# projectchrono/DEM-Engine

Measured on AMD Instinct MI355X. Metric: clump*steps/s, higher is better.
Workload: dtype f32 physics / f64 geometry

## Files before the change

dem-engine_amd/abi.py:

```python
import ctypes as C
import os

import numpy as np

_HERE = os.path.dirname(os.path.abspath(__file__))

NULL_MAPPING_PARTNER = 0xFFFFFFFF
FAMILY_MASK_ENTRIES = 32896
NUM_FAMILIES = 256
FAMILY_FIXED = 1
FAMILY_GHOST = 2
FAMILY_PRESCRIBED = 4
INTEGRATOR_FORWARD_EULER, INTEGRATOR_CENTERED_DIFFERENCE, INTEGRATOR_EXTENDED_TAYLOR = 0, 1, 2
FORCE_HERTZIAN, FORCE_HERTZIAN_FRICTIONLESS, FORCE_CUSTOM = 0, 1, 2
GHOST_BYTES = 56


ARITH_FAST, ARITH_EXACT = 1, 0


class DemeParams(C.Structure):
    _fields_ = [
        ("nvXp2", C.c_uint32), ("nvYp2", C.c_uint32), ("nvZp2", C.c_uint32),
        ("nbX", C.c_uint32), ("nbY", C.c_uint32), ("nbZ", C.c_uint32),
# ... 691 lines not shown


def _owner_state_request(owner_ids, columns):
    ids = np.ascontiguousarray(owner_ids, dtype=np.uint32).ravel()
    st, out = DemeOwnerState(), {}
    for name in STATE_DTYPES:
        setattr(st, name, None)
    for name in columns:
        out[name] = np.zeros(max(ids.size, 1), STATE_DTYPES[name])
        setattr(st, name, out[name].ctypes.data)
    st._keep = out
    return ids, st, {k: v[:ids.size] for k, v in out.items()}


def _owner_state_rows(owner_ids, arrays):
    ids = None if owner_ids is None else np.ascontiguousarray(owner_ids, dtype=np.uint32).ravel()
    st, keep = DemeOwnerState(), {}
    for name in STATE_DTYPES:
        a = arrays.get(name)
        if a is None:
            setattr(st, name, None)
            continue
        keep[name] = np.ascontiguousarray(a, dtype=STATE_DTYPES[name]).ravel()
        if ids is not None and keep[name].size != ids.size:
            raise DemeError(f"scatter_owner_state: column {name} has {keep[name].size} rows for {ids.size} ids")
        if not keep[name].size:
            keep[name] = np.zeros(1, STATE_DTYPES[name])
        setattr(st, name, keep[name].ctypes.data)
    st._keep = keep
    return ids, st


def exported_symbols():
    import re
    hdr = os.path.join(_HERE, "..", "include", "deme_hip.h")
    txt = open(hdr).read()
    return sorted(set(re.findall(r"\b(deme_[a-z_0-9]+)\s*\(", txt)))


def _ptr(a):
    return None if a is None else a.ctypes.data


def sort_tile_keys():
    return int(load_library().deme_sort_tile_keys())


def tri_loads_block_rows():
    return int(load_library().deme_tri_loads_block_rows())


def _inspect_tri_loads(self, fn, name, force_threshold, first, count):
    if count is None:
        if getattr(self, "n_tri", None) is None:
            raise ValueError(f"{name}: count is needed (this object has not seen the scene's triangle count)")
        count = self.n_tri - int(first)
    force = np.zeros((max(int(count), 0), 3), np.float64)
    contacts = np.zeros(max(int(count), 0), np.uint32)
    self._ck(fn(self.h, float(force_threshold), int(first), int(count), _ptr(force), _ptr(contacts)), name)
    return force, contacts


def sort_pairs_u32(keys, vals, begin_bit, end_bit, force_own=True, device=0):
    keys, vals = np.ascontiguousarray(keys, np.uint32), np.ascontiguousarray(vals, np.uint32)
    assert keys.shape == vals.shape and keys.ndim == 1
    ko, vo = np.empty_like(keys), np.empty_like(vals)
    rc = load_library().deme_sort_pairs_u32(device, _ptr(keys), _ptr(vals), keys.size, begin_bit, end_bit, int(bool(force_own)), _ptr(ko),
                                            _ptr(vo))
    if rc:
        raise DemeError(f"deme_sort_pairs_u32 failed with code {rc}")
    return ko, vo


def sort_keys_u64(keys, begin_bit, end_bit, force_own=True, device=0):
    keys = np.ascontiguousarray(keys, np.uint64)
    assert keys.ndim == 1
    ko = np.empty_like(keys)
    rc = load_library().deme_sort_keys_u64(device, _ptr(keys), keys.size, begin_bit, end_bit, int(bool(force_own)), _ptr(ko))
    if rc:
        raise DemeError(f"deme_sort_keys_u64 failed with code {rc}")
    return ko


def jit_probe(src, wildcard_names=(), prerequisites="", owner_wildcards=(), geo_wildcards=()):
    lib = load_library()

    def arr(ns):
        return (C.c_char_p * max(1, len(ns)))(*[s.encode() for s in ns])
    log = C.create_string_buffer(8192)
    rc = lib.deme_jit_probe_ex(src.encode(), arr(wildcard_names), len(wildcard_names), arr(owner_wildcards), len(owner_wildcards),
                               arr(geo_wildcards), len(geo_wildcards), prerequisites.encode(), log, len(log))
    return rc == 0, log.value.decode(errors="replace")


class Context:

    def __init__(self, device=0):
        self.lib = load_library()
        h = _P()
        rc = self.lib.deme_ctx_create(int(device), C.byref(h))
        if rc != 0 or not h:
            raise DemeError(f"deme_ctx_create failed (status {rc}): is a HIP device visible?")
        self.h = h
        self.n_owners = 0
        self.n_spheres = 0
        self.n_wildcards = 0

    @classmethod
    def borrowed(cls, handle):
        self = cls.__new__(cls)
        self.lib = load_library()
        self.h = handle
        self._borrowed = True
        v = (C.c_uint32 * 4)()
        self.lib.deme_scene_sizes.argtypes = [_P, C.POINTER(C.c_uint32)]
        self._ck(self.lib.deme_scene_sizes(self.h, v), "deme_scene_sizes")
        self.n_owners, self.n_spheres, self.n_wildcards = int(v[0]), int(v[2]), int(v[3])
        return self

    def refresh_sizes(self):
        v = (C.c_uint32 * 4)()
        self.lib.deme_scene_sizes.argtypes = [_P, C.POINTER(C.c_uint32)]
        self._ck(self.lib.deme_scene_sizes(self.h, v), "deme_scene_sizes")
        self.n_owners, self.n_spheres = int(v[0]), int(v[2])

    def close(self):
        if getattr(self, "h", None):
            if not getattr(self, "_borrowed", False):
                self.lib.deme_ctx_destroy(self.h)
            self.h = None

    def __del__(self):
        try:
            self.close()
        except Exception:
            pass

    def _ck(self, rc, what):
        if rc != 0:
            msg = self.lib.deme_last_error(self.h)
            raise DemeError(f"{what} failed (status {rc}): {msg.decode() if msg else ''}")

    def set_stream(self, stream_ptr):
        self._ck(self.lib.deme_ctx_set_stream(self.h, stream_ptr), "deme_ctx_set_stream")

    def sync(self):
        self._ck(self.lib.deme_sync(self.h), "deme_sync")

    def set_arith_mode(self, mode):
        m = {"fast": ARITH_FAST, "exact": ARITH_EXACT}.get(mode, mode)
        self._ck(self.lib.deme_set_arith_mode(self.h, int(m)), "deme_set_arith_mode")

    def arith_mode(self):
        return "fast" if self.lib.deme_get_arith_mode(self.h) == ARITH_FAST else "exact"

    def set_params(self, p):
        self.n_wildcards = int(p.nContactWildcards)
        self._ck(self.lib.deme_set_params(self.h, C.byref(p)), "deme_set_params")

    def upload_scene(self, sc):
        self.n_owners, self.n_spheres = int(sc.nOwners), int(sc.nSpheres)
        self.n_tri = int(sc.nTri)
        self._ck(self.lib.deme_upload_scene(self.h, C.byref(sc)), "deme_upload_scene")

    def upload_state(self, arrays):
        st, _ = make_state_struct(self.n_owners, arrays)
# ... 359 lines not shown
```

dem-engine_amd/csrc/deme_hip.hip:

```cpp
#include <algorithm>
#include <cmath>
#include <cstdarg>
#include <cstdio>
#include <cstdlib>
#include <chrono>
#include <cstring>
#include <condition_variable>
#include <functional>
#include <memory>
#include <mutex>
#include <dlfcn.h>
#include <map>
#include <string>
#include <thread>
#include <vector>

#include <hip/hip_runtime.h>
#include <rocprim/rocprim.hpp>
template <unsigned RB, unsigned IPT = 8>
using DemeRadixCfg = rocprim::radix_sort_config<rocprim::default_config, rocprim::default_config,
                                                rocprim::radix_sort_onesweep_config<rocprim::kernel_config<1024, IPT>, rocprim::kernel_config<1024, IPT>, RB,
                                                                                    rocprim::block_radix_rank_algorithm::match>,
                                                1024 * 1024>;
#include <array>
#include <iterator>
#include <limits>

#include "../../include/deme_hip.h"
#include "deme_device.h"
#include "deme_force.h"
#include "deme_force_fast.h"
#include "deme_jit.h"
#include "deme_kernels.h"
#include "deme_tile.h"
#include "deme_tile_step.h"
#include "deme_migrate.h"
#include "deme_mesh_kernels.h"
#include "deme_resize.h"
#include "deme_query.h"
#include "deme_contact_inspect.h"
#include "deme_tri_loads.h"
#include "deme_sort.h"

using namespace deme_dev;

namespace {

struct DevBuf {
    void* p = nullptr;
    size_t bytes = 0;
    template <typename T>
    T* as() const {
        return reinterpret_cast<T*>(p);
    }
};

struct ContactList {
    DevBuf mapping, ownerA, ownerB[2], bIdx[2], info, tInfo, rIdx, lPos, remVal, rankC, remKey[2], cDefer, blockMode, smFlag, smList;
    DevBuf aStart, bStart, heavy, fixedFlag, heavyList, rangeCtr, hList, hCount, tileMode, tileOrg, rStart, lOff, lCount, tileRem, tileBase,
        tileBig, bigList;
    uint64_t nListed = 0;
    int listKeys = 0;
    bool legacyLists = false;
    bool tileActive = false;
    bool fusedList = false;
    bool fusedChecked = false;
    bool hrPending = false, heavyOverflow = false;
    uint32_t nHeavy = 0, nHeavyFree = 0, nSA = 0, nSM = 0;
    uint32_t nBigTiles = 0, tileMaxHalo = 0, tileMaxList = 0, tileMaxHaloIn = 0;

    void invalidate() {
        nListed = 0, listKeys = 0;
        legacyLists = tileActive = fusedList = fusedChecked = hrPending = heavyOverflow = false;
        nHeavy = nHeavyFree = nSA = nSM = 0;
        nBigTiles = tileMaxHalo = tileMaxList = tileMaxHaloIn = 0;
    }
    std::array<DevBuf*, 35> buffers() {
        return {&mapping, &ownerA, &ownerB[0], &ownerB[1], &bIdx[0], &bIdx[1], &info, &tInfo, &rIdx, &lPos, &remVal, &rankC, &remKey[0],
                &remKey[1], &cDefer, &blockMode, &smFlag, &smList, &aStart, &bStart, &heavy, &fixedFlag, &heavyList, &rangeCtr, &hList,
                &hCount, &tileMode, &tileOrg, &rStart, &lOff, &lCount, &tileRem, &tileBase, &tileBig, &bigList};
    }
};

struct TimerSlot {
    std::vector<std::pair<hipEvent_t, hipEvent_t>> pending;
    double total_ms = 0;
    uint64_t launches = 0;
    uint64_t seen = 0;
};

}

struct deme_ctx {
    int device = 0;
    hipStream_t stream = nullptr;
    bool ownStream = true;
    std::string err;
    DemeParams hp{};
    bool haveParams = false, haveScene = false;
    DevParams dp{};
    uint32_t nOwners = 0, nOwnerClumps = 0, nSpheres = 0, nAnal = 0, nMat = 0, nComp = 0, nMassProps = 0;
    DevBuf owners, spheres, acc, comp, massProps, anal, matPair, E, nu, CoR, mu, Crr, famMasks, famExtra, famFlags;
    std::vector<uint8_t> hObjType;
    std::vector<float4> hComp;
    uint32_t nTemplateComps = 0;
    DevBuf rsMark, rsKeys[2], rsRuns, rsUKeys, rsIdx, rsOldR, rsUses, rsRemap;
    DevBuf qMark, qHits, qRecs, qCtr, qState;
    uint64_t qHostBytes = 0;
    DevBuf ciMask, ciCounts, ciPartial, ciOut;
    DevBuf tlTri[2], tlRow[2], tlTmp, tlPartial, tlForce, tlCount;
    std::map<std::string, int> regionBySource;
    DevBuf sphFam;
    DevBuf geo, binLo, binN, binPartial, incKeys[2], incVals[2], keysRaw, keysMid, keysSorted[2], wc[2], ctr,
        scanTmp, sortTmp, rec[4], stage;
    ContactList list[2];
    int cur = 0;
    DevBuf conA4, conA2, conB4, conB2, aSum, rec32;
    RangeCounters* hrPinned = nullptr;
    hipEvent_t hrEvent = nullptr;
    bool ctrFresh = false;
    bool conTile = false;
#define DEME_FUSED_AUTO_MAX_OWNERS 100000u
    int fusedEnable = 0;
    bool fusedPrevValid = false;
    uint64_t nFusedSteps = 0;
    DevBuf ownersNext, recContact, inCnt, inStart, tInfoIn, inContact, hCountIn;
    uint32_t tileMinContactsCustom = 320;
    uint64_t lastSegMax = 0;
    size_t keySegMin = (size_t)1 << 20;
    DevBuf persistKeys, binStat;
    DevBuf nextAcc;
    std::vector<AccRec> hNextAcc;
    bool nextAccPending = false;
    std::vector<uint64_t> hPersist;
    uint32_t nTri = 0;
    DevBuf tris, triWorld, triLo, triHi, triCounts, triOffsets, triKeys[2], triVals[2];
    size_t triCap = 0;
    uint64_t nTriInc = 0;
    deme_jit::MaterialTables mt;
    hipModule_t customMod = nullptr;
    hipFunction_t customFn[3] = {nullptr, nullptr, nullptr};
    hipFunction_t customTileFn[4] = {nullptr, nullptr, nullptr, nullptr};
    std::map<size_t, std::vector<char>> jitCache;
    bool conValid = false;
    int keysCur = 0, wcCur = 0;
    size_t incCap = 0, cntCap = 0;
    uint64_t nInc = 0, nContacts = 0, nPrev = 0, nWcStored = 0;
    uint64_t nActiveBins = 0;
    uint32_t maxInBin = 0;
    bool haveList = false, mapFresh = false;
    bool seeded = false;
    hipModule_t prescMod = nullptr;
    hipFunction_t prescFn = nullptr;
    DevBuf prescList, prescSlot, prescRec;
    DevBuf userWc[4][8];
    uint32_t nOwnerWc = 0, nGeoWc = 0;
    bool hasGhosts = false;
    uint32_t asyncLead = 0;
    DevBuf revSlot;
    const void* revAcc = nullptr;
    bool pairsOnce = false;
    PrescArgs laterPa{nullptr, nullptr};
    bool crossStale = false;
    char* pin = nullptr;
    int spinSync = 1;
    bool snapPending = false;
    DevBuf ownersSnap;
    hipStream_t detStream = nullptr;
    hipEvent_t evSnap = nullptr, evP1 = nullptr;
    uint64_t nAsyncDetections = 0;
    std::vector<uint32_t> hShared;
    DevBuf sharedIds, sharedBuf;
    bool tailFused = true;
    bool inGroupStep = false;
    hipStream_t haloStream = nullptr;
    hipEvent_t evStepDone = nullptr, evHaloDone = nullptr;
    bool overlapDetect = false;
    hipModule_t rulesMod = nullptr;
    DemeAdaptive ad{};
    hipEvent_t evDet0 = nullptr, evDet1 = nullptr, evWin0 = nullptr, evWin1 = nullptr;
    double binAccMs = 0, binPrevMs = -1, freqPrevMs = -1;
    float binRate = 0.f;
    uint32_t binObs = 0, freqObs = 0, nBinChanges = 0, nFreqChanges = 0;
    uint64_t winStartStep = 0;
    int freqDir = 1, binFlip = 1;
    bool winOpen = false;
    std::vector<hipModule_t> regionMod;
    std::vector<hipFunction_t> regionFn;
    DevBuf volumes;
    bool haveVolumes = false;
    hipFunction_t rulesFn = nullptr;
    bool rulesNeedAcc = false;
    uint32_t nPresc = 0;
    uint8_t hostFamFlags[DEME_NUM_FAMILIES] = {0};
    bool prescDirty = true;
    bool record = false;
    uint64_t nSteps = 0, nDetections = 0;
    uint32_t stepsSinceCD = 0;
    bool listStale = false;
    uint32_t lastStatus = 0;
    double timeElapsed = 0;
    int arith = DEME_ARITH_FAST;
    uint32_t xcdGroup = 0;
    bool permuted = false;
    int reorderEnable = 1;
    std::vector<uint32_t> hO2E, hE2O, hS2E, hE2S;
    DevBuf dO2E, dS2E;
    double orderSpread[2] = {0, 0};
    bool orderEligible = false;
    bool orderStructOK = false;
    bool geoStale = false;
    bool orderRenewDue = false;
    uint32_t orderBaseHalo = 0;
    uint64_t orderDetAt = 0, nOrderRenewals = 0;
    uint64_t listSerial = 0, viewSerial = ~0ull;
    std::vector<uint64_t> viewKeys;
    std::vector<uint32_t> viewPerm;
    int timing = 0;
    std::map<std::string, TimerSlot> timers;
    std::vector<hipEvent_t> eventPool;
};

namespace {

int fail(deme_ctx* c, int code, const char* fmt, ...) {
    char buf[1024];
    va_list ap;
    va_start(ap, fmt);
    vsnprintf(buf, sizeof(buf), fmt, ap);
    va_end(ap);
    if (c) {
        c->err = buf;
        c->lastStatus = (uint32_t)code;
    }
    return code;
}

inline uint64_t key_class_of_type(uint8_t type) {
    return type == DEME_SPHERE_SPHERE_CONTACT ? DEME_KEY_CLASS_SS : type == DEME_SPHERE_MESH_CONTACT ? DEME_KEY_CLASS_SM : DEME_KEY_CLASS_SA;
}

int records_refused(deme_ctx* c) {
    if (!c->record)
        return fail(c, DEME_ERR_INVALID, "contact recording is off (deme_set_record_contacts)");
    if (c->seeded)
        return fail(c, DEME_ERR_INVALID, "the list is a seed (deme_seed_contacts, or the engine's order was just renewed): its contacts have not been evaluated yet -- step or detect first");
    return DEME_OK;
}

#define HIPCK(call)                                                                                   \
    do {                                                                                              \
        hipError_t _e = (call);                                                                       \
        if (_e != hipSuccess)                                                                         \
            return fail(c, DEME_ERR_HIP, "%s failed: %s (%s:%d)", #call, hipGetErrorString(_e), __FILE__, __LINE__); \
    } while (0)

template <typename T>
static inline T* pin_at(deme_ctx* c, size_t off) {
    return reinterpret_cast<T*>(c->pin + off);
}
static hipError_t sync_readback(deme_ctx* c, hipStream_t st, bool spin) {
    if (c->spinSync && spin) {
        const auto t0 = std::chrono::steady_clock::now();
        for (int it = 0;; it++) {
            const hipError_t q = hipStreamQuery(st);
            if (q != hipErrorNotReady)
                return q;
            if ((it & 255) == 255 && std::chrono::steady_clock::now() - t0 > std::chrono::milliseconds(5))
                break;
        }
    }
    return hipStreamSynchronize(st);
}

int ensure(deme_ctx* c, DevBuf& b, size_t bytes, bool keep = false) {
    if (bytes <= b.bytes && b.p)
        return DEME_OK;
    size_t want = std::max<size_t>(bytes, 256);
    if (b.p)
        want = std::max(want, b.bytes + b.bytes / 4);
    void* np = nullptr;
    HIPCK(hipMalloc(&np, want));
    if (keep && b.p && b.bytes)
        HIPCK(hipMemcpyAsync(np, b.p, b.bytes, hipMemcpyDeviceToDevice, c->stream));
    if (b.p) {
        HIPCK(hipStreamSynchronize(c->stream));
        HIPCK(hipFree(b.p));
    }
    b.p = np;
    b.bytes = want;
    return DEME_OK;
}

template <typename T>
int upload(deme_ctx* c, DevBuf& b, const T* src, size_t n) {
    int rc = ensure(c, b, std::max<size_t>(n, 1) * sizeof(T));
    if (rc)
        return rc;
    if (n && src)
        HIPCK(hipMemcpyAsync(b.p, src, n * sizeof(T), hipMemcpyHostToDevice, c->stream));
    else if (n)
        HIPCK(hipMemsetAsync(b.p, 0, n * sizeof(T), c->stream));
    return DEME_OK;
}

template <class Call>
int with_temp(deme_ctx* c, DevBuf& tmp, Call&& call) {
    size_t bytes = 0;
    HIPCK(call(nullptr, bytes));
    if (int rc = ensure(c, tmp, bytes))
        return rc;
    bytes = tmp.bytes;
    HIPCK(call(tmp.p, bytes));
    return DEME_OK;
}

#ifndef DEME_SORT_ROCPRIM
#define DEME_SORT_ROCPRIM 0
#endif
constexpr size_t DEME_SORT_OWN_FROM_INCIDENCES = 82000;
constexpr size_t DEME_SORT_OWN_FROM_KEYS64 = 430000;
constexpr size_t DEME_SORT_OWN_FROM_RECORDS = 180000;
inline bool sort_takes_own(size_t n, size_t cap, size_t ownFrom) {
    return !DEME_SORT_ROCPRIM && n >= ownFrom && std::max(n, cap) <= deme_sort::MAX_N;
}
template <class RocCfg, bool HAS_V, typename K>
hipError_t deme_radix_sort(void* tmp, size_t& bytes, const K* keysIn, K* keysOut, const uint32_t* valsIn, uint32_t* valsOut, size_t n, size_t cap,
                           unsigned beginBit, unsigned endBit, size_t ownFrom, hipStream_t st) {
    if (sort_takes_own(n, cap, ownFrom))
        return deme_sort::radix_sort<K, HAS_V>(tmp, bytes, keysIn, keysOut, valsIn, valsOut, n, cap, beginBit, endBit, st);
    if constexpr (HAS_V)
        return rocprim::radix_sort_pairs<RocCfg>(tmp, bytes, keysIn, keysOut, valsIn, valsOut, n, beginBit, endBit, st);
    else
        return rocprim::radix_sort_keys<RocCfg>(tmp, bytes, keysIn, keysOut, n, beginBit, endBit, st);
}

inline unsigned grid_for(size_t n, unsigned block = 256) { return (unsigned)((n + block - 1) / block); }
inline unsigned bits_for(uint64_t n, unsigned cap) {
    unsigned b = 1;
    while (b < cap && (1ull << b) < n)
        b++;
    return b;
}

hipEvent_t get_event(deme_ctx* c) {
    if (!c->eventPool.empty()) {
        hipEvent_t e = c->eventPool.back();
        c->eventPool.pop_back();
        return e;
    }
    hipEvent_t e;
    hipEventCreate(&e);
    return e;
}
struct ScopedTimer {
    deme_ctx* c;
    TimerSlot* slot = nullptr;
    hipEvent_t a = nullptr, b = nullptr;
    hipStream_t st = nullptr;
    ScopedTimer(deme_ctx* ctx, const char* name, bool always = false, hipStream_t stream = nullptr) : c(ctx), st(stream ? stream : ctx->stream) {
        if (!c->timing)
            return;
        slot = &c->timers[name];
        if (!always && (slot->seen++ % (uint64_t)c->timing) != 0) {
            slot = nullptr;
            return;
        }
        if (slot->pending.size() >= 8192) {
            slot = nullptr;
            return;
        }
        a = get_event(c);
        b = get_event(c);
        hipEventRecord(a, st);
    }
    ~ScopedTimer() {
        if (slot) {
            hipEventRecord(b, st);
            slot->pending.emplace_back(a, b);
        }
    }
};
void drain_timers(deme_ctx* c) {
    for (auto& kv : c->timers) {
        for (auto& pr : kv.second.pending) {
            hipEventSynchronize(pr.second);
            float ms = 0;
            hipEventElapsedTime(&ms, pr.first, pr.second);
            kv.second.total_ms += ms;
            kv.second.launches++;
            c->eventPool.push_back(pr.first);
            c->eventPool.push_back(pr.second);
        }
        kv.second.pending.clear();
    }
}

void refresh_dev_params(deme_ctx* c) {
    DevParams& d = c->dp;
    const DemeParams& h = c->hp;
    d.nvXp2 = h.nvXp2, d.nvYp2 = h.nvYp2;
    d.nbX = h.nbX, d.nbY = h.nbY, d.nbZ = h.nbZ;
    d.mNbX = fast_div_magic(h.nbX), d.mNbXY = fast_div_magic(h.nbX * h.nbY);
    d.l = h.l, d.voxelSize = h.voxelSize, d.binSize = h.binSize;
    d.LBFX = h.LBFX, d.LBFY = h.LBFY, d.LBFZ = h.LBFZ;
    d.Gx = h.Gx, d.Gy = h.Gy, d.Gz = h.Gz;
    d.h = h.h;
    d.approxMaxVel = h.approxMaxVel, d.expSafetyMulti = h.expSafetyMulti, d.expSafetyAdder = h.expSafetyAdder;
    d.errOutVel = h.errOutVel;
    d.integrator = h.integrator, d.forceModel = h.forceModel, d.nW = h.nContactWildcards;
    d.nOwners = c->nOwners, d.nSpheres = c->nSpheres, d.nAnal = c->nAnal, d.nMat = c->nMat;
    d.errOutBinSphNum = h.errOutBinSphNum ? h.errOutBinSphNum : 32768u;
    d.comp = c->comp.as<float4>();
    d.massProps = c->massProps.as<float4>();
    d.anal = c->anal.as<AnalObj>();
    d.matPair = c->matPair.as<MatPair>();
    d.E = c->E.as<float>(), d.nu = c->nu.as<float>(), d.CoR = c->CoR.as<float>(), d.mu = c->mu.as<float>(),
    d.Crr = c->Crr.as<float>();
    d.familyMasks = c->famMasks.as<uint8_t>();
    d.familyExtra = c->famExtra.as<float>();
    d.familyFlags = c->famFlags.as<uint8_t>();
    d.tris = c->tris.p;
    d.nTri = c->nTri;
    d.s2e = c->permuted ? c->dS2E.as<uint32_t>() : nullptr;
    d.o2e = c->permuted ? c->dO2E.as<uint32_t>() : nullptr;
}

int check_ready(deme_ctx* c) {
    if (!c)
        return DEME_ERR_INVALID;
    if (!c->haveParams || !c->haveScene)
        return fail(c, DEME_ERR_INVALID, "deme_set_params and deme_upload_scene must be called first");
    if (hipSetDevice(c->device) != hipSuccess)
        return fail(c, DEME_ERR_HIP, "device %d cannot be selected", c->device);
    return DEME_OK;
}

void build_mat_pairs(const DemeScene* s, std::vector<MatPair>& out) {
    const uint32_t n = s->nMat;
    out.resize((size_t)n * n);
    for (uint32_t a = 0; a < n; a++)
        for (uint32_t b = 0; b < n; b++) {
            MatPair m{};
            const float Y1 = s->E[a], nu1 = s->nu[a], Y2 = s->E[b], nu2 = s->nu[b];
            const float invE = (1.0f - nu1 * nu1) / Y1 + (1.0f - nu2 * nu2) / Y2;
            m.E_cnt = 1.0f / invE;
            const float invG = 2.0f * (2.0f - nu1) * (1.0f + nu1) / Y1 + 2.0f * (2.0f - nu2) * (1.0f + nu2) / Y2;
            m.G_cnt = 1.0f / invG;
            m.CoR = s->CoR ? s->CoR[a * n + b] : 0.f;
            m.mu = s->mu ? s->mu[a * n + b] : 0.f;
            m.Crr = s->Crr ? s->Crr[a * n + b] : 0.f;
            const float loge = (float)((m.CoR < 1e-12) ? log(1e-12) : logf(m.CoR));
            m.beta = (float)(loge / sqrt(loge * loge + 9.869604401089358));
            out[(size_t)a * n + b] = m;
        }
}

int size_list_per_contact(deme_ctx* c, ContactList& L, size_t cap, bool hasGhosts, uint32_t nTri) {
    int rc = 0;
    rc |= ensure(c, L.mapping, cap * 4, true);
    rc |= ensure(c, L.ownerA, cap * 4);
    for (int k = 0; k < 2; k++) {
        rc |= ensure(c, L.ownerB[k], cap * 4);
        rc |= ensure(c, L.bIdx[k], cap * 4);
    }
    rc |= ensure(c, L.info, cap * 16);
    rc |= ensure(c, L.tInfo, cap * 8);
    rc |= ensure(c, L.rIdx, cap * 4);
    rc |= ensure(c, L.lPos, cap * 2);
    rc |= ensure(c, L.remVal, (cap + 1) * 4);
    rc |= ensure(c, L.rankC, (cap + 1) * 4);
    rc |= ensure(c, L.remKey[0], (cap + 1) * 4);
    rc |= ensure(c, L.remKey[1], (cap + 1) * 4);
    if (hasGhosts) {
        rc |= ensure(c, L.cDefer, cap);
        rc |= ensure(c, L.blockMode, (cap / DEME_FORCE_BLOCK + 2) * 4);
    }
    if (nTri) {
        rc |= ensure(c, L.smFlag, cap);
        rc |= ensure(c, L.smList, cap * 4);
    }
    return rc;
}
int size_list_per_owner(deme_ctx* c, ContactList& L, size_t nO) {
    if (ensure(c, L.aStart, (nO + 1) * 4) || ensure(c, L.bStart, (nO + 1) * 4) || ensure(c, L.heavy, nO + 1) || ensure(c, L.fixedFlag, nO + 1) ||
        ensure(c, L.heavyList, 4096 * 4) || ensure(c, L.rangeCtr, sizeof(RangeCounters)))
        return c->lastStatus;
    const size_t nTiles = (nO + DEME_TILE_NB - 1) / DEME_TILE_NB + 1;
    if (ensure(c, L.hList, nTiles * DEME_TILE_HMAX * 4) || ensure(c, L.hCount, nTiles * 4) || ensure(c, L.tileMode, nTiles * 4) ||
        ensure(c, L.tileOrg, nTiles * 24) || ensure(c, L.rStart, (nO + 1) * 4) || ensure(c, L.lOff, nTiles * (DEME_TILE_NB + 1) * 2) ||
        ensure(c, L.lCount, nTiles * 4) || ensure(c, L.tileRem, (nTiles + 1) * 4) || ensure(c, L.tileBase, (nTiles + 1) * 4) ||
        ensure(c, L.tileBig, nTiles * 4) || ensure(c, L.bigList, nTiles * 4))
        return c->lastStatus;
    return DEME_OK;
}

int grow_contact_arena(deme_ctx* c, size_t cap) {
    const uint32_t nW = std::max<uint32_t>(c->hp.nContactWildcards, 1);
    int rc = 0;
    rc |= ensure(c, c->keysRaw, cap * 8);
    rc |= ensure(c, c->keysSorted[0], cap * 8, true);
    rc |= ensure(c, c->keysSorted[1], cap * 8, true);
    rc |= ensure(c, c->wc[0], cap * 4 * nW, true);
    rc |= ensure(c, c->wc[1], cap * 4 * nW, true);
    if (c->record)
        for (int k = 0; k < 4; k++)
            rc |= ensure(c, c->rec[k], cap * 12);
    rc |= ensure(c, c->conA4, cap * 16);
    rc |= ensure(c, c->conA2, cap * 8);
    rc |= ensure(c, c->conB4, cap * 16);
    rc |= ensure(c, c->conB2, cap * 8);
    rc |= size_list_per_contact(c, c->list[c->cur], cap, c->hasGhosts, c->nTri);
    rc |= ensure(c, c->recContact, (cap + 1) * 4);
    rc |= ensure(c, c->tInfoIn, cap * 8);
    rc |= ensure(c, c->inContact, cap * 4);
    rc |= ensure(c, c->rec32, cap * 32);
    if (rc)
        return rc;
    c->cntCap = cap;
    return DEME_OK;
}

int grow_incidence_arena(deme_ctx* c, size_t cap) {
    int rc = 0;
    for (int k = 0; k < 2; k++) {
        rc |= ensure(c, c->incKeys[k], cap * 4);
        rc |= ensure(c, c->incVals[k], cap * 4);
    }
    if (rc)
        return rc;
    c->incCap = cap;
    return DEME_OK;
}

int status_to_error(deme_ctx* c, uint32_t st) {
    if (st & DEME_ST_NONFINITE)
        return fail(c, DEME_ERR_VELOCITY, "a non-finite owner velocity was found at time %.9g", c->timeElapsed);
    if (st & DEME_ST_VELOCITY)
        return fail(c, DEME_ERR_VELOCITY,
                    "system max velocity exceeded the error-out velocity %.7g at time %.9g (SetErrorOutVelocity)",
                    (double)c->hp.errOutVel, c->timeElapsed);
    return DEME_OK;
}

int do_margins(deme_ctx* c, uint32_t drift) {
    HIPCK(hipMemsetAsync(c->ctr.p, 0, sizeof(DetectBlock), c->stream));
    c->ctrFresh = true;
    if (c->nOwners)
    hipLaunchKernelGGL(k_margins, dim3(grid_for(c->nOwners)), dim3(256), 0, c->stream, c->dp, c->owners.as<OwnerRec>(),
                       drift, c->ctr.as<DetectCounters>());
    return DEME_OK;
}

int do_migrate(deme_ctx* c);
int detect_part1(deme_ctx* c, hipStream_t st, OwnerRec* ow, bool async, uint64_t* nCout) {
    const uint32_t nS = c->nSpheres;
    DetectCounters hc{};
    const bool countersFresh = c->ctrFresh;
    c->ctrFresh = false;
    bool statusSeen = false;

    DetectBlock* blk = c->ctr.as<DetectBlock>();
    for (int attempt = 0; attempt < 4; attempt++) {
        if (attempt > 0 || !countersFresh)
            HIPCK(hipMemsetAsync(c->ctr.p, 0, sizeof(DetectBlock), st));
        const bool segmented = c->keySegMin && c->cntCap >= c->keySegMin && c->cntCap >= DEME_KEY_SEGS * 64u;
        KeyArena ar;
        ar.keys = c->keysRaw.as<uint64_t>();
        ar.segMask = segmented ? DEME_KEY_SEGS - 1u : 0u;
        ar.segCap = segmented ? (uint64_t)c->cntCap / DEME_KEY_SEGS : (uint64_t)c->cntCap;
        ar.ctr = segmented ? blk->segCtr : &blk->c.nContactsRaw;
        if (nS) {
            c->geoStale = false;
            hipLaunchKernelGGL(k_sphere_prep, dim3(grid_for(nS)), dim3(256), 0, st, c->dp,
                               ow, c->spheres.as<SphereRec>(), c->geo.as<GeoRec>(),
                               c->binLo.as<uint4>(), c->binN.as<uint2>(), c->binPartial.as<uint32_t>(),
                               ar, c->ctr.as<DetectCounters>(), c->sphFam.as<uint16_t>());
            hipLaunchKernelGGL(k_scan_small, dim3(1), dim3(DEME_SCAN_T), 0, st, c->binPartial.as<uint32_t>(), c->binPartial.as<uint32_t>(),
                               grid_for(nS), &blk->c.nIncidence);
        }
        uint32_t P = 0;
        bool filled = false;
        auto fill_incidence = [&]() {
            hipLaunchKernelGGL(k_fill_incidence, dim3(grid_for(nS)), dim3(256), 0, st, c->dp,
                               c->binLo.as<uint4>(), c->binN.as<uint2>(), c->binPartial.as<uint32_t>(),
                               c->incKeys[0].as<uint32_t>(), c->incVals[0].as<uint32_t>(), (uint64_t)c->incCap);
            filled = true;
        };
        if (nS && c->incCap)
            fill_incidence();
        if (nS) {
            HIPCK(hipMemcpyAsync(pin_at<DetectCounters>(c, 1024), c->ctr.p, sizeof(hc), hipMemcpyDeviceToHost, st));
            HIPCK(sync_readback(c, st, !async));
            hc = *pin_at<DetectCounters>(c, 1024);
            if (!statusSeen) {
                statusSeen = true;
                if (int rc = status_to_error(c, hc.status & ~DEME_ST_INCIDENCE))
                    return rc;
            }
            if (hc.status & DEME_ST_INCIDENCE)
                return fail(c, DEME_ERR_OVERFLOW,
                            "a sphere touches more than %u bins (margin far larger than the bin size): the incidence list cannot be built",
                            DEME_MAX_BINS_PER_SPHERE);
            if (hc.nIncidence > 0xFFFFFFFFull)
                return fail(c, DEME_ERR_OVERFLOW, "%llu bin-sphere incidences do not fit the 32-bit list offsets (use larger bins)",
                            hc.nIncidence);
            P = (uint32_t)hc.nIncidence;
        }
        if (P > c->incCap) {
            if (int rc = grow_incidence_arena(c, (size_t)P + P / 4 + 1024))
                return rc;
            filled = false;
        }
        c->nInc = P;
        uint32_t nStats = 0;
        const unsigned bits = bits_for((uint64_t)c->hp.nbX * c->hp.nbY * c->hp.nbZ, 32);
        if (P) {
            if (!filled)
                fill_incidence();
            const bool twoPass = bits > 16 && bits <= 22;
            if (int rc = with_temp(c, c->sortTmp, [&](void* tmp, size_t& bytes) {
                    return twoPass ? deme_radix_sort<DemeRadixCfg<11, 16>, true>(tmp, bytes, c->incKeys[0].as<uint32_t>(), c->incKeys[1].as<uint32_t>(),
                                                                                 c->incVals[0].as<uint32_t>(), c->incVals[1].as<uint32_t>(), (size_t)P,
                                                                                 (size_t)c->incCap, 0, bits, DEME_SORT_OWN_FROM_INCIDENCES, st)
                                   : deme_radix_sort<DemeRadixCfg<8>, true>(tmp, bytes, c->incKeys[0].as<uint32_t>(), c->incKeys[1].as<uint32_t>(),
                                                                            c->incVals[0].as<uint32_t>(), c->incVals[1].as<uint32_t>(), (size_t)P,
                                                                            (size_t)c->incCap, 0, bits, DEME_SORT_OWN_FROM_INCIDENCES, st);
                }))
                return rc;
            const uint32_t nWin = (uint32_t)grid_for(P, SW_T);
            if (int rc = ensure(c, c->binStat, (size_t)nWin * sizeof(uint2)))
                return rc;
            static_assert(SW_WPB == 1, "k_sweep writes one statistics record per window");
            hipLaunchKernelGGL(k_sweep, dim3(nWin), dim3(SW_T), 0, st, c->dp,
                               c->incKeys[1].as<uint32_t>(), c->incVals[1].as<uint32_t>(), P, c->geo.as<GeoRec>(),
                               c->sphFam.as<uint16_t>(), ar, c->binStat.as<uint2>());
            if (segmented)
                nStats = nWin;
            else
                hipLaunchKernelGGL(k_bin_stats_final, dim3((nWin + 2047u) / 2048u), dim3(256), 0, st, c->binStat.as<uint2>(), nWin,
                                   c->ctr.as<DetectCounters>());
        }
        c->nTriInc = 0;
        if (c->nTri && P) {
            const uint32_t nT = c->nTri;
            hipLaunchKernelGGL(k_tri_prep, dim3(grid_for(nT)), dim3(256), 0, st, c->dp, nT, c->tris.as<TriRec>(),
                               ow, c->triWorld.as<TriWorld>(), c->triLo.as<int4>(),
                               c->triHi.as<int4>(), c->triCounts.as<uint32_t>());
            size_t tmp = c->scanTmp.bytes;
            HIPCK(rocprim::exclusive_scan(c->scanTmp.p, tmp, c->triCounts.as<uint32_t>(), c->triOffsets.as<uint32_t>(), 0u,
                                          (size_t)nT + 1, rocprim::plus<uint32_t>(), st));
            uint32_t TP = 0;
            HIPCK(hipMemcpyAsync(&TP, c->triOffsets.as<uint32_t>() + nT, 4, hipMemcpyDeviceToHost, st));
            HIPCK(hipStreamSynchronize(st));
            if (TP > c->triCap) {
                const size_t cap = (size_t)TP + TP / 4 + 1024;
                for (int k = 0; k < 2; k++)
                    if (ensure(c, c->triKeys[k], cap * 4) || ensure(c, c->triVals[k], cap * 4))
                        return c->lastStatus;
                c->triCap = cap;
            }
            c->nTriInc = TP;
            if (TP) {
                hipLaunchKernelGGL(k_tri_fill, dim3(grid_for(nT)), dim3(256), 0, st, c->dp, nT,
                                   c->triWorld.as<TriWorld>(), c->triLo.as<int4>(), c->triHi.as<int4>(),
                                   c->triOffsets.as<uint32_t>(), c->triKeys[0].as<uint32_t>(), c->triVals[0].as<uint32_t>(),
                                   (uint64_t)c->triCap);
                if (int rc = with_temp(c, c->sortTmp, [&](void* tmp, size_t& bytes) {
                        return rocprim::radix_sort_pairs(tmp, bytes, c->triKeys[0].as<uint32_t>(), c->triKeys[1].as<uint32_t>(),
                                                         c->triVals[0].as<uint32_t>(), c->triVals[1].as<uint32_t>(), (size_t)TP, 0, bits, st);
                    }))
                    return rc;
                hipLaunchKernelGGL(k_tri_sweep, dim3(grid_for(TP)), dim3(256), 0, st, c->dp, TP,
                                   c->triKeys[1].as<uint32_t>(), c->triVals[1].as<uint32_t>(), c->triWorld.as<TriWorld>(), P,
                                   c->incKeys[1].as<uint32_t>(), c->incVals[1].as<uint32_t>(), c->geo.as<GeoRec>(),
                                   c->sphFam.as<uint16_t>(), ar);
            }
        }
        const int nextEarly = c->keysCur ^ 1;
        uint32_t compactBlocks = 0;
        if (segmented) {
            compactBlocks = (uint32_t)std::min<uint64_t>(grid_for(std::max<uint64_t>(c->lastSegMax + c->lastSegMax / 8 + 1024, 1)), grid_for(ar.segCap));
            hipLaunchKernelGGL(k_compact_keys, dim3(compactBlocks, DEME_KEY_SEGS), dim3(256), 0, st, c->keysRaw.as<uint64_t>(), ar.segCap,
                               blk, 0u, c->keysSorted[nextEarly].as<uint64_t>(), c->binStat.as<uint2>(), nStats);
        }
        const DetectHead* hh = pin_at<DetectHead>(c, 1024);
        HIPCK(hipMemcpyAsync(pin_at<DetectHead>(c, 1024), c->ctr.p, segmented ? sizeof(DetectHead) : sizeof(DetectCounters), hipMemcpyDeviceToHost, st));
        HIPCK(sync_readback(c, st, !async));
        hc = hh->c;
        if (!statusSeen) {
            statusSeen = true;
            if (int rc = status_to_error(c, hc.status & ~DEME_ST_INCIDENCE))
                return rc;
        }
        unsigned long long segMax = 0;
        if (segmented) {
            hc.nContactsRaw = 0;
            for (uint32_t g = 0; g < DEME_KEY_SEGS; g++) {
                hc.nContactsRaw += hh->segCount[g];
                segMax = std::max(segMax, hh->segCount[g]);
            }
        }
        if (hc.nContactsRaw > c->cntCap || segMax > ar.segCap) {
            if (async)
                HIPCK(hipStreamSynchronize(c->stream));
            const size_t want = std::max<size_t>(hc.nContactsRaw, (size_t)segMax * DEME_KEY_SEGS);
            if (int rc = grow_contact_arena(c, want + want / 4 + 1024))
                return rc;
            continue;
        }
        c->nActiveBins = hc.nActiveBins;
        c->maxInBin = hc.maxInBin ? hc.maxInBin : (P ? 1u : 0u);
        if (c->maxInBin > c->dp.errOutBinSphNum)
            return fail(c, DEME_ERR_BIN_TOO_FULL,
                        "a bin contains %u sphere components, exceeding the allowance %u (SetMaxSphereInBin)", c->maxInBin,
                        c->dp.errOutBinSphNum);
        uint64_t nC = hc.nContactsRaw;
        const size_t nPersist = c->hPersist.size();
        if (nPersist) {
            if (nC + nPersist > c->cntCap) {
                if (async)
                HIPCK(hipStreamSynchronize(c->stream));
            if (int rc = grow_contact_arena(c, (size_t)nC + nPersist + nC / 4 + 1024))
                    return rc;
                continue;
            }
            nC += nPersist;
        }
        const int next = c->keysCur ^ 1;
        uint64_t* rawKeys = c->keysRaw.as<uint64_t>();
        if (segmented) {
            c->lastSegMax = segMax;
            if (grid_for(segMax) > compactBlocks)
                hipLaunchKernelGGL(k_compact_keys, dim3((unsigned)grid_for(segMax) - compactBlocks, DEME_KEY_SEGS), dim3(256), 0, st,
                                   c->keysRaw.as<uint64_t>(), ar.segCap, blk, compactBlocks, c->keysSorted[next].as<uint64_t>(),
                                   (const uint2*)nullptr, 0u);
            if (hc.nContactsRaw)
                rawKeys = c->keysSorted[next].as<uint64_t>();
        }
        if (nPersist)
            HIPCK(hipMemcpyAsync(rawKeys + hc.nContactsRaw, c->persistKeys.p, nPersist * 8, hipMemcpyDeviceToDevice, st));
        if (nC) {
            const unsigned bitsA = bits_for(c->dp.nSpheres, 31);
            if (int rc = ensure(c, c->keysMid, (size_t)c->cntCap * 8))
                return rc;
            uint64_t* mid = c->keysMid.as<uint64_t>();
            if (int rc = with_temp(c, c->sortTmp, [&](void* tmp, size_t& bytes) {
                    return deme_radix_sort<DemeRadixCfg<8>, false>(tmp, bytes, rawKeys, mid, nullptr, nullptr, (size_t)nC, (size_t)c->cntCap, 31,
                                                                   33 + bitsA, DEME_SORT_OWN_FROM_KEYS64, st);
                }))
                return rc;
            hipLaunchKernelGGL(k_segment_rank_sort, dim3(grid_for(nC)), dim3(256), 0, st, (uint32_t)nC, mid,
                               c->keysSorted[next].as<uint64_t>());
            if (nPersist) {
                unsigned long long* cnt = &blk->c.nContactsRaw;
                if (int rc = with_temp(c, c->scanTmp, [&](void* tmp, size_t& bytes) {
                        return rocprim::unique(tmp, bytes, c->keysSorted[next].as<uint64_t>(), c->keysRaw.as<uint64_t>(), cnt, (size_t)nC,
                                               rocprim::equal_to<uint64_t>(), st);
                    }))
                    return rc;
                unsigned long long nU = 0;
                HIPCK(hipMemcpyAsync(&nU, cnt, 8, hipMemcpyDeviceToHost, st));
                HIPCK(hipStreamSynchronize(st));
                nC = nU;
                HIPCK(hipMemcpyAsync(c->keysSorted[next].p, c->keysRaw.p, (size_t)nC * 8, hipMemcpyDeviceToDevice, st));
            }
        }
        *nCout = nC;
        return DEME_OK;
    }
    return fail(c, DEME_ERR_OVERFLOW, "contact arena kept overflowing");
}

int build_legacy_lists(deme_ctx* c, ContactList& L, const OwnerRec* ow, hipStream_t st) {
    const uint64_t nC = L.nListed;
    if (nC) {
        const unsigned obits = bits_for(c->nOwners, 32);
        if (int rc = with_temp(c, c->sortTmp, [&](void* tmp, size_t& bytes) {
                return rocprim::radix_sort_pairs(tmp, bytes, L.ownerB[0].as<uint32_t>(), L.ownerB[1].as<uint32_t>(), L.bIdx[0].as<uint32_t>(),
                                                 L.bIdx[1].as<uint32_t>(), (size_t)nC, 0, obits, st);
            }))
            return rc;
    }
    if (c->hasGhosts) {
        if (int rc = size_list_per_contact(c, L, c->cntCap, true, c->nTri))
            return rc;
        HIPCK(hipMemsetAsync(L.blockMode.p, 0, L.blockMode.bytes, st));
    }
    if (nC)
        hipLaunchKernelGGL(k_run_starts, dim3(grid_for(nC)), dim3(256), 0, st, (uint32_t)nC, L.ownerB[1].as<uint32_t>(),
                           c->nOwners, L.bStart.as<uint32_t>());
    else
        HIPCK(hipMemsetAsync(L.bStart.p, 0, ((size_t)c->nOwners + 1) * 4, st));
    HIPCK(hipMemsetAsync(&L.rangeCtr.as<RangeCounters>()->nHeavy, 0, 2 * sizeof(unsigned int), st));
    hipLaunchKernelGGL(k_owner_ranges, dim3(grid_for((size_t)c->nOwners + 1)), dim3(256), 0, st, c->dp, (uint32_t)nC,
                       L.ownerA.as<uint32_t>(), L.ownerB[1].as<uint32_t>(), ow, L.aStart.as<uint32_t>(),
                       L.bStart.as<uint32_t>(), L.heavy.as<uint8_t>(), L.fixedFlag.as<uint8_t>(), L.heavyList.as<uint32_t>(),
                       (uint32_t)(L.heavyList.bytes / 4), L.rangeCtr.as<RangeCounters>(), L.info.as<uint4>(),
                       c->hasGhosts ? L.cDefer.as<uint8_t>() : (uint8_t*)nullptr, L.blockMode.as<uint32_t>());
    L.legacyLists = true;
    return DEME_OK;
}
int read_legacy_counts(deme_ctx* c, ContactList& L, hipStream_t st, RangeCounters& hr) {
    HIPCK(hipMemcpyAsync(&hr, L.rangeCtr.p, sizeof(hr), hipMemcpyDeviceToHost, st));
    HIPCK(hipStreamSynchronize(st));
    if (hr.nHeavy > L.heavyList.bytes / 4)
        return fail(c, DEME_ERR_OVERFLOW, "%u owners exceed the heavy-owner list", hr.nHeavy);
    L.nHeavy = hr.nHeavy, L.nHeavyFree = hr.nHeavyFree;
    return DEME_OK;
}

void resolve_heavy_counts(deme_ctx* c, ContactList& L);
int ensure_legacy_lists(deme_ctx* c) {
    ContactList& L = c->list[c->cur];
    if (L.legacyLists || !c->haveList)
        return DEME_OK;
    resolve_heavy_counts(c, L);
    if (int rc = build_legacy_lists(c, L, c->owners.as<OwnerRec>(), c->stream))
        return rc;
    RangeCounters hr{};
    return read_legacy_counts(c, L, c->stream, hr);
}

bool tile_eligible(const deme_ctx* c, uint64_t nC) {
    const uint32_t nTiles = (c->nOwners + DEME_TILE_NB - 1) / DEME_TILE_NB;
    if (!nC || c->arith != DEME_ARITH_FAST || !c->hShared.empty())
        return false;
    if (c->hp.forceModel == DEME_FORCE_CUSTOM && !(c->customTileFn[0] && nC >= (uint64_t)c->tileMinContactsCustom * nTiles))
        return false;
    static_assert(DEME_TILE_T < 2 * 17 * 17, "a tile's tables may hold more than 16 materials: tInfo has 4-bit material fields");
    const uint64_t pieces = (uint64_t)c->nComp + 2ull * c->nMat * c->nMat + 4ull * c->nAnal;
    return pieces <= DEME_TILE_T && c->nMassProps <= DEME_TILE_T && c->nAnal <= 65535 && c->nComp <= 65535 &&
           tile_table_bytes(c->nComp, c->nMat, c->nAnal, c->nMassProps, c->dp.familyTrivial) <= DEME_TILE_TABLE_MAX;
}

int detect_part2(deme_ctx* c, ContactList& L, const OwnerRec* ow, hipStream_t st, uint64_t nC) {
    const int next = c->keysCur ^ 1;
    L.invalidate();
    const bool tileEligible = tile_eligible(c, nC);
    const uint32_t nTiles = (c->nOwners + DEME_TILE_NB - 1) / DEME_TILE_NB;
    if (nC) {
        const uint64_t nPrev = c->haveList ? c->nContacts : 0;
        hipLaunchKernelGGL(k_history, dim3(grid_for(nC)), dim3(256), 0, st, (uint32_t)nC, c->keysSorted[next].as<uint64_t>(),
                           (uint32_t)nPrev, c->keysSorted[c->keysCur].as<uint64_t>(), L.mapping.as<uint32_t>(),
                           L.rangeCtr.as<uint32_t>(), (uint32_t)(sizeof(RangeCounters) / 4), L.tileRem.as<uint32_t>(),
                           tileEligible ? nTiles + 1 : 0u);
    } else {
        HIPCK(hipMemsetAsync(L.rangeCtr.p, 0, sizeof(RangeCounters), st));
    }
    if (nC) {
        hipLaunchKernelGGL(k_contact_owners, dim3(grid_for(nC)), dim3(256), 0, st, c->dp, (uint32_t)nC,
                           c->keysSorted[next].as<uint64_t>(), c->spheres.as<SphereRec>(), L.ownerA.as<uint32_t>(),
                           L.ownerB[0].as<uint32_t>(), L.bIdx[0].as<uint32_t>(), L.info.as<uint4>(),
                           c->nTri ? L.smFlag.as<uint8_t>() : (uint8_t*)nullptr,
                           tileEligible ? L.tileRem.as<uint32_t>() : (uint32_t*)nullptr, (uint32_t)DEME_TILE_NB);
        if (c->nTri) {
            unsigned int* cnt = &L.rangeCtr.as<RangeCounters>()->nSM;
            if (int rc = with_temp(c, c->scanTmp, [&](void* tmp, size_t& bytes) {
                    return rocprim::select(tmp, bytes, rocprim::counting_iterator<uint32_t>(0), L.smFlag.as<uint8_t>(), L.smList.as<uint32_t>(), cnt,
                                           (size_t)nC, st);
                }))
                return rc;
        }
        hipLaunchKernelGGL(k_run_starts, dim3(grid_for(nC)), dim3(256), 0, st, (uint32_t)nC, L.ownerA.as<uint32_t>(), c->nOwners,
                           L.aStart.as<uint32_t>());
    } else {
        HIPCK(hipMemsetAsync(L.aStart.p, 0, ((size_t)c->nOwners + 1) * 4, st));
    }
    L.nListed = nC, L.listKeys = next;
    bool tiled = false;
    RangeCounters hr{};
    if (tileEligible) {
        hipLaunchKernelGGL(k_scan_small, dim3(1), dim3(DEME_SCAN_T), 0, st, L.tileRem.as<uint32_t>(), L.tileBase.as<uint32_t>(), nTiles + 1,
                           &L.rangeCtr.as<RangeCounters>()->nRemote);
        hipLaunchKernelGGL(k_tile_build, dim3(nTiles), dim3(256), 0, st, c->dp, c->nOwners, L.info.as<uint4>(),
                           L.ownerB[0].as<uint32_t>(), L.aStart.as<uint32_t>(), ow, L.tileBase.as<uint32_t>(), L.tInfo.as<uint2>(),
                           L.hList.as<uint32_t>(), L.hCount.as<uint32_t>(),
                           c->hasGhosts ? L.tileMode.as<uint32_t>() : (uint32_t*)nullptr, L.lOff.as<uint16_t>(),
                           L.lPos.as<uint16_t>(), L.lCount.as<uint32_t>(), L.rankC.as<uint32_t>(), L.remKey[0].as<uint32_t>(),
                           L.remVal.as<uint32_t>(), L.tileOrg.as<int64_t>(), L.rangeCtr.as<RangeCounters>(), nTiles,
                           L.tileBig.as<uint32_t>(), L.bigList.as<uint32_t>(), c->recContact.as<uint32_t>());
        hipLaunchKernelGGL(k_tile_stats, dim3((nTiles + 1023u) / 1024u), dim3(256), 0, st, nTiles, L.hCount.as<uint32_t>(),
                           L.lCount.as<uint32_t>(), L.rangeCtr.as<RangeCounters>());
        uint32_t nR = 0;
        HIPCK(hipMemcpyAsync(pin_at<RangeCounters>(c, 128), L.rangeCtr.p, sizeof(hr), hipMemcpyDeviceToHost, st));
        HIPCK(sync_readback(c, st, true));
        hr = *pin_at<RangeCounters>(c, 128);
        nR = (uint32_t)hr.nRemote + hr.nExtra;
        L.nBigTiles = hr.nBig;
        const unsigned obits = bits_for(c->nOwners, 32);
        if (nR) {
            if (int rc = with_temp(c, c->sortTmp, [&](void* tmp, size_t& bytes) {
                    return deme_radix_sort<DemeRadixCfg<10>, true>(tmp, bytes, L.remKey[0].as<uint32_t>(), L.remKey[1].as<uint32_t>(),
                                                                   L.remVal.as<uint32_t>(), L.rIdx.as<uint32_t>(), (size_t)nR, (size_t)c->cntCap, 0, obits,
                                                                   DEME_SORT_OWN_FROM_RECORDS, st);
                }))
                return rc;
            hipLaunchKernelGGL(k_run_starts, dim3(grid_for(nR)), dim3(256), 0, st, nR, L.remKey[1].as<uint32_t>(), c->nOwners,
                               L.rStart.as<uint32_t>());
        } else {
            HIPCK(hipMemsetAsync(L.rStart.p, 0, ((size_t)c->nOwners + 1) * 4, st));
        }
        hipLaunchKernelGGL(k_owner_ranges_tile, dim3(grid_for(c->nOwners)), dim3(256), 0, st, c->dp, ow, L.aStart.as<uint32_t>(),
                           L.lOff.as<uint16_t>(), L.rStart.as<uint32_t>(), L.heavy.as<uint8_t>(), L.fixedFlag.as<uint8_t>(),
                           L.heavyList.as<uint32_t>(), (uint32_t)(L.heavyList.bytes / 4), L.rangeCtr.as<RangeCounters>());
        tiled = true;
        static const int fusedEnv = getenv("DEME_FUSED") ? atoi(getenv("DEME_FUSED")) : -1;
        const int fusedMode = fusedEnv < 0 ? c->fusedEnable : fusedEnv;
        if ((fusedMode == 2 ? c->nOwners <= DEME_FUSED_AUTO_MAX_OWNERS : fusedMode != 0) && hr.nBig == 0 && c->hp.forceModel != DEME_FORCE_CUSTOM && !c->record && c->nTri == 0 &&
            !c->hasGhosts && !c->prescFn && !c->rulesFn && c->hShared.empty() && c->asyncLead == 0 &&
            !c->ad.autoBinSize && !c->ad.autoUpdateFreq) {
            hipLaunchKernelGGL(k_in_count, dim3(grid_for((size_t)c->nOwners + 1)), dim3(256), 0, st, c->dp, ow,
                               L.rStart.as<uint32_t>(), c->inCnt.as<uint32_t>());
            if (int rc = with_temp(c, c->scanTmp, [&](void* tmp, size_t& bytes) {
                    return rocprim::exclusive_scan(tmp, bytes, c->inCnt.as<uint32_t>(), c->inStart.as<uint32_t>(), 0u, (size_t)c->nOwners + 1,
                                                   rocprim::plus<uint32_t>(), st);
                }))
                return rc;
            hipLaunchKernelGGL(k_tile_incoming, dim3(nTiles), dim3(256), 0, st, c->dp, c->nOwners, L.info.as<uint4>(),
                               L.rStart.as<uint32_t>(), L.rIdx.as<uint32_t>(), c->recContact.as<uint32_t>(), c->inStart.as<uint32_t>(),
                               L.hList.as<uint32_t>(), L.hCount.as<uint32_t>(), c->hCountIn.as<uint32_t>(), c->tInfoIn.as<uint2>(),
                               c->inContact.as<uint32_t>(), L.rangeCtr.as<RangeCounters>());
            L.fusedList = true;
        }
    }
    if (tiled) {
        if (!c->hrPinned) {
            HIPCK(hipHostMalloc((void**)&c->hrPinned, sizeof(RangeCounters), hipHostMallocDefault));
            HIPCK(hipEventCreateWithFlags(&c->hrEvent, hipEventDisableTiming));
        }
        HIPCK(hipMemcpyAsync(c->hrPinned, L.rangeCtr.p, sizeof(RangeCounters), hipMemcpyDeviceToHost, st));
        HIPCK(hipEventRecord(c->hrEvent, st));
        L.hrPending = true;
    } else {
        if (int rc = build_legacy_lists(c, L, ow, st))
            return rc;
        if (int rc = read_legacy_counts(c, L, st, hr))
            return rc;
    }
    L.tileActive = tiled;
    L.tileMaxHalo = hr.tileMaxHalo, L.tileMaxList = hr.tileMaxList;
    L.nSA = hr.nSA;
    L.nSM = hr.nSM;
    c->fusedPrevValid = false;
    if (tiled && c->orderEligible) {
        const uint32_t fit = std::max(1u, nTiles - std::min(nTiles, hr.nBig));
        const uint32_t mean16 = (uint32_t)(16ull * hr.tileHaloSum / fit);
        if (!c->orderBaseHalo) {
            c->orderBaseHalo = std::max(mean16, 16u);
            c->orderDetAt = c->nDetections;
        } else if (c->nDetections - c->orderDetAt >= 20 && nTiles > 4 &&
                   (hr.nBig > std::max(4u, nTiles / 64u) || mean16 > c->orderBaseHalo + c->orderBaseHalo / 2)) {
            c->orderRenewDue = true;
        }
    }
    c->conValid = false;
    c->nPrev = c->haveList ? c->nContacts : 0;
    c->nContacts = nC;
    c->keysCur = next;
    c->listSerial++;
    c->haveList = true;
    c->seeded = false;
    c->mapFresh = true;
    c->nDetections++;
    return DEME_OK;
}


int do_detect(deme_ctx* c) {
    if (c->mapFresh)
        if (int rc = do_migrate(c))
            return rc;
    ScopedTimer tm(c, "detect", true);
    uint64_t nC = 0;
    if (int rc = detect_part1(c, c->stream, c->owners.as<OwnerRec>(), false, &nC))
        return rc;
    return detect_part2(c, c->list[c->cur], c->owners.as<OwnerRec>(), c->stream, nC);
}

int do_migrate(deme_ctx* c) {
    ContactList& L = c->list[c->cur];
    const uint32_t nW = c->hp.nContactWildcards;
// ... 364 lines not shown
            PrescRec* rec = c->prescRec.as<PrescRec>();
            uint32_t n = c->nPresc;
            float t = (float)c->timeElapsed;
            void* args[] = {&c->dp, &ow, &list, &n, &rec, &t};
            HIPCK(hipModuleLaunchKernel(c->prescFn, grid_for(n), 1, 1, 256, 1, 1, 0, c->stream, args, nullptr));
            pa.rec = rec;
            pa.slot = c->prescSlot.as<uint32_t>();
        }
    }
    if (from == AccFrom::Contributions) {
        if (L.heavyOverflow)
            return c->lastStatus;
        GatherArgs ga = gather_args(c);
        ga.revPhase = who == Owners::NotWaiting ? 1u : 0u;
        if (c->nOwners)
        hipLaunchKernelGGL(k_integrate<true>, dim3(grid_for(c->nOwners)), dim3(256), 0, c->stream, c->dp,
                           c->owners.as<OwnerRec>(), c->acc.as<AccRec>(), ga, pa);
    } else {
        if (c->nOwners)
        hipLaunchKernelGGL(k_integrate<false>, dim3(grid_for(c->nOwners)), dim3(256), 0, c->stream, c->dp,
                           c->owners.as<OwnerRec>(), c->acc.as<AccRec>(), gather_args(c), pa);
    }
    c->laterPa = pa;
    if (who == Owners::NotWaiting)
        return DEME_OK;
    return clear_next_acc(c);
}
int launch_integrate_later(deme_ctx* c, const uint32_t* ids, uint32_t n) {
    if (n) {
        ScopedTimer tm(c, "integrate_later");
        hipLaunchKernelGGL(k_integrate_list, dim3(grid_for(n)), dim3(256), 0, c->stream, c->dp, c->owners.as<OwnerRec>(),
                           c->acc.as<AccRec>(), gather_args(c), c->laterPa, ids, n);
    }
    return clear_next_acc(c);
}

void launch_full_reduction(deme_ctx* c) {
    if (c->nOwners)
    hipLaunchKernelGGL(k_gather_acc, dim3(grid_for(c->nOwners)), dim3(256), 0, c->stream, c->dp, gather_args(c),
                       c->owners.as<OwnerRec>(), c->acc.as<AccRec>());
    launch_reduce_heavy(c, false);
}

}

#include "deme_order.inc"

extern "C" {

const char* deme_version(void) { return "deme_hip 0.1 (gfx950)"; }

int deme_ctx_create(int device, deme_ctx** out) {
    if (!out)
        return DEME_ERR_INVALID;
    *out = nullptr;
    int n = 0;
    if (hipGetDeviceCount(&n) != hipSuccess || n <= 0 || device >= n)
        return DEME_ERR_HIP;
    if (hipSetDevice(device) != hipSuccess)
        return DEME_ERR_HIP;
    deme_ctx* c = new deme_ctx();
    c->device = device;
    if (hipStreamCreateWithFlags(&c->stream, hipStreamNonBlocking) != hipSuccess) {
        delete c;
        return DEME_ERR_HIP;
    }
    if (ensure(c, c->ctr, sizeof(DetectBlock)) || ensure(c, c->scanTmp, 1 << 20)) {
        delete c;
        return DEME_ERR_HIP;
    }
    hipMemsetAsync(c->ctr.p, 0, sizeof(DetectBlock), c->stream);
    if (hipHostMalloc((void**)&c->pin, 16384, hipHostMallocDefault) != hipSuccess) {
        deme_ctx_destroy(c);
        return DEME_ERR_HIP;
    }
    if (const char* e = getenv("DEME_ARITH"))
        c->arith = (strcmp(e, "exact") == 0) ? DEME_ARITH_EXACT : DEME_ARITH_FAST;
    if (const char* e = getenv("DEME_XCD_GROUP"))
        c->xcdGroup = (uint32_t)std::max(0, atoi(e));
    if (const char* e = getenv("DEME_SPIN_SYNC"))
        c->spinSync = atoi(e);
    if (const char* e = getenv("DEME_KEY_SEG_MIN"))
        c->keySegMin = (size_t)std::max(0ll, atoll(e));
    *out = c;
    return DEME_OK;
}

void deme_ctx_destroy(deme_ctx* c) {
    if (!c)
        return;
    hipSetDevice(c->device);
    hipStreamSynchronize(c->stream);
    drain_timers(c);
    for (auto e : c->eventPool)
        hipEventDestroy(e);
    for (hipModule_t m : {c->customMod, c->prescMod, c->rulesMod})
        if (m)
            (void)hipModuleUnload(m);
    for (hipModule_t m : c->regionMod)
        if (m)
            (void)hipModuleUnload(m);
    for (hipEvent_t e : {c->evDet0, c->evDet1, c->evWin0, c->evWin1})
        if (e)
            hipEventDestroy(e);
    if (c->haloStream) {
        hipStreamSynchronize(c->haloStream);
        hipEventDestroy(c->evStepDone);
        hipEventDestroy(c->evHaloDone);
        hipStreamDestroy(c->haloStream);
    }
    if (c->pin)
        hipHostFree(c->pin);
    for (ContactList& l : c->list)
        for (DevBuf* b : l.buffers())
            if (b->p)
                hipFree(b->p);
    if (c->hrPinned) {
        hipHostFree(c->hrPinned);
        hipEventDestroy(c->hrEvent);
    }
    if (c->detStream) {
        hipStreamSynchronize(c->detStream);
        hipEventDestroy(c->evSnap);
        hipEventDestroy(c->evP1);
        hipStreamDestroy(c->detStream);
    }
    DevBuf* all[] = {&c->hCountIn, &c->ownersNext, &c->recContact, &c->inCnt, &c->inStart, &c->tInfoIn, &c->inContact,
                     &c->sphFam, &c->dO2E, &c->dS2E, &c->rec32, &c->revSlot, &c->nextAcc, &c->binStat, &c->volumes,
                     &c->persistKeys, &c->owners, &c->spheres, &c->acc, &c->conA4, &c->conA2, &c->conB4, &c->conB2, &c->aSum,
                     &c->prescList, &c->prescSlot, &c->prescRec, &c->tris, &c->triWorld, &c->triLo, &c->triHi, &c->triCounts,
                     &c->triOffsets, &c->triKeys[0], &c->triKeys[1], &c->triVals[0], &c->triVals[1], &c->comp, &c->massProps,
                     &c->anal, &c->matPair, &c->E, &c->nu, &c->CoR, &c->mu, &c->Crr, &c->famMasks, &c->famExtra, &c->famFlags,
                     &c->geo, &c->binLo, &c->binN, &c->binPartial, &c->incKeys[0], &c->incKeys[1], &c->incVals[0],
                     &c->incVals[1], &c->keysRaw, &c->keysSorted[0], &c->keysSorted[1], &c->wc[0], &c->wc[1], &c->ctr,
                     &c->scanTmp, &c->sortTmp, &c->rec[0], &c->rec[1], &c->rec[2], &c->rec[3], &c->stage, &c->sharedIds,
                     &c->sharedBuf, &c->keysMid, &c->ownersSnap, &c->rsMark, &c->rsKeys[0], &c->rsKeys[1], &c->rsRuns,
                     &c->rsUKeys, &c->rsIdx, &c->rsOldR, &c->rsUses, &c->rsRemap, &c->qMark, &c->qHits, &c->qRecs, &c->qCtr, &c->qState,
                     &c->ciMask, &c->ciCounts, &c->ciPartial, &c->ciOut, &c->tlTri[0], &c->tlTri[1], &c->tlRow[0], &c->tlRow[1],
                     &c->tlTmp, &c->tlPartial, &c->tlForce, &c->tlCount};
    for (DevBuf* b : all)
        if (b->p)
            hipFree(b->p);
    for (auto& kind : c->userWc)
        for (auto& b : kind)
            if (b.p)
                hipFree(b.p);
    if (c->ownStream && c->stream)
        hipStreamDestroy(c->stream);
    delete c;
}

const char* deme_last_error(const deme_ctx* c) { return c ? c->err.c_str() : "null context"; }

int deme_ctx_set_stream(deme_ctx* c, void* s) {
    if (!c)
        return DEME_ERR_INVALID;
    hipSetDevice(c->device);
    HIPCK(hipStreamSynchronize(c->stream));
    if (s) {
        if (c->ownStream)
            hipStreamDestroy(c->stream);
        c->stream = (hipStream_t)s;
        c->ownStream = false;
    } else if (!c->ownStream) {
        HIPCK(hipStreamCreateWithFlags(&c->stream, hipStreamNonBlocking));
        c->ownStream = true;
    }
    return DEME_OK;
}

int deme_set_arith_mode(deme_ctx* c, int mode) {
    if (!c || (mode != DEME_ARITH_FAST && mode != DEME_ARITH_EXACT))
        return DEME_ERR_INVALID;
    hipSetDevice(c->device);
    if (mode != c->arith) {
        HIPCK(hipStreamSynchronize(c->stream));
        c->arith = mode;
        c->conValid = false;
        if (mode == DEME_ARITH_EXACT) {
            c->orderEligible = false, c->orderRenewDue = false;
            if (c->permuted && c->haveScene)
                if (int rc = order_restore(c))
                    return rc;
        } else if (c->haveScene && c->orderStructOK) {
            c->orderEligible = true;
            c->orderRenewDue = true;
        }
    }
    return DEME_OK;
}
int deme_get_arith_mode(const deme_ctx* c) { return c ? c->arith : -1; }

int deme_force_kernel_name(const deme_ctx* c, char* name, size_t cap, uint32_t* tileMaxHalo, uint32_t* tileMaxList) {
    if (!c || !name || !cap)
        return DEME_ERR_INVALID;
// ... 2913 lines not shown
    if (int rc = check_ready(c))
        return rc;
    if (int rc = contact_inspect_refused(c, "deme_inspect_contacts", out, region, thr))
        return rc;
    ContactSums* res = nullptr;
    if (int rc = contact_inspect_launch(c, region, thr, false, &res))
        return rc;
    DemeContactSums h;
    HIPCK(hipMemcpyAsync(&h, res, sizeof h, hipMemcpyDeviceToHost, c->stream));
    HIPCK(hipStreamSynchronize(c->stream));
    c->qHostBytes += sizeof h;
    *out = h;
    return DEME_OK;
}

int deme_inspect_contact_counts(deme_ctx* c, int region, float thr, uint32_t* perOwner, size_t cap) {
    if (int rc = check_ready(c))
        return rc;
    if (int rc = contact_inspect_refused(c, "deme_inspect_contact_counts", perOwner, region, thr))
        return rc;
    const size_t nO = c->nOwners;
    if (cap < nO)
        return fail(c, DEME_ERR_INVALID, "buffer too small: need %zu", nO);
    if (!nO)
        return DEME_OK;
    if (ensure(c, c->ciOut, nO * 4))
        return c->lastStatus;
    if (int rc = contact_inspect_launch(c, region, thr, true, nullptr))
        return rc;
    if (nO)
    hipLaunchKernelGGL(k_contact_counts_out, dim3(grid_for(nO)), dim3(256), 0, c->stream, (uint32_t)nO, c->ciCounts.as<uint32_t>(), c->dp.o2e,
                       (const uint32_t*)nullptr, c->ciOut.as<uint32_t>(), (uint32_t)nO);
    std::vector<uint32_t> h(nO);
    HIPCK(hipMemcpyAsync(h.data(), c->ciOut.p, nO * 4, hipMemcpyDeviceToHost, c->stream));
    HIPCK(hipStreamSynchronize(c->stream));
    c->qHostBytes += 4ull * nO;
    memcpy(perOwner, h.data(), nO * 4);
    return DEME_OK;
}

namespace {
int tri_loads_args_refused(char (&msg)[320], const char* who, float thr, uint32_t firstTri, uint32_t nTris, uint32_t nTri, const void* force,
                           const void* contacts) {
    msg[0] = 0;
    if (!std::isfinite(thr) || thr < 0.f)
        snprintf(msg, sizeof msg, "%s: the force threshold is %g; it must be finite and >= 0", who, (double)thr);
    else if ((uint64_t)firstTri + nTris > nTri)
        snprintf(msg, sizeof msg, "%s: triangles [%u, %llu) were asked for; the scene has %u", who, firstTri,
                 (unsigned long long)firstTri + nTris, nTri);
    else if (nTris && !force && !contacts)
        snprintf(msg, sizeof msg, "%s: null output (force and contacts)", who);
    return msg[0] ? DEME_ERR_INVALID : DEME_OK;
}
int tri_loads_launch(deme_ctx* c, float thr) {
    const size_t n = c->haveList ? (size_t)c->nContacts : 0, nT = c->nTri;
    const unsigned grid = grid_for(std::max<size_t>(n, 1), TRI_LOADS_BLOCK_ROWS);
    if (ensure(c, c->tlForce, nT * 24) || ensure(c, c->tlCount, nT * 4))
        return c->lastStatus;
    HIPCK(hipMemsetAsync(c->tlForce.p, 0, nT * 24, c->stream));
    HIPCK(hipMemsetAsync(c->tlCount.p, 0, nT * 4, c->stream));
    if (!n)
        return DEME_OK;
    for (int k = 0; k < 2; k++)
        if (ensure(c, c->tlTri[k], n * 4) || ensure(c, c->tlRow[k], n * 4))
            return c->lastStatus;
    if (ensure(c, c->tlPartial, (size_t)grid * 2 * sizeof(TriPartial)))
        return c->lastStatus;
    TriSelectArgs a{};
    a.n = (uint32_t)n, a.keys = c->keysSorted[c->keysCur].as<uint64_t>();
    a.spheres = c->spheres.as<SphereRec>(), a.owners = c->owners.as<OwnerRec>();
    a.nSpheres = c->nSpheres, a.nOwners = c->nOwners, a.nTri = c->nTri;
    a.force = c->rec[0].as<float>(), a.thr2 = (double)thr * (double)thr;
    a.tri = c->tlTri[0].as<uint32_t>(), a.row = c->tlRow[0].as<uint32_t>();
    {
        ScopedTimer t(c, "tri_loads_select", true);
        hipLaunchKernelGGL(k_tri_select, dim3(grid_for(n)), dim3(256), 0, c->stream, a);
    }
    const unsigned bits = bits_for((uint64_t)nT + 1, 32);
    {
        ScopedTimer t(c, "tri_loads_sort", true);
        if (int rc = with_temp(c, c->tlTmp, [&](void* tmp, size_t& bytes) {
                return deme_radix_sort<DemeRadixCfg<8>, true>(tmp, bytes, c->tlTri[0].as<uint32_t>(), c->tlTri[1].as<uint32_t>(),
                                                              c->tlRow[0].as<uint32_t>(), c->tlRow[1].as<uint32_t>(), n, n, 0, bits,
                                                              DEME_SORT_OWN_FROM_RECORDS, c->stream);
            }))
            return rc;
    }
    ScopedTimer t(c, "tri_loads_sums", true);
    hipLaunchKernelGGL(k_tri_seg_sums, dim3(grid), dim3(256), 0, c->stream, (uint32_t)n, (uint32_t)nT, c->tlTri[1].as<uint32_t>(),
                       c->tlRow[1].as<uint32_t>(), c->rec[0].as<float>(), c->tlForce.as<double>(), c->tlCount.as<uint32_t>(),
                       c->tlPartial.as<TriPartial>());
    hipLaunchKernelGGL(k_tri_seg_final, dim3(1), dim3(256), 0, c->stream, 2u * grid, (uint32_t)nT, c->tlPartial.as<TriPartial>(),
                       c->tlForce.as<double>(), c->tlCount.as<uint32_t>());
    HIPCK(hipGetLastError());
    return DEME_OK;
}
int tri_loads_fetch(deme_ctx* c, uint32_t firstTri, uint32_t nTris, double* force, uint32_t* contacts) {
    if (force)
        HIPCK(hipMemcpyAsync(force, c->tlForce.as<double>() + 3 * (size_t)firstTri, (size_t)nTris * 24, hipMemcpyDeviceToHost, c->stream));
    if (contacts)
        HIPCK(hipMemcpyAsync(contacts, c->tlCount.as<uint32_t>() + firstTri, (size_t)nTris * 4, hipMemcpyDeviceToHost, c->stream));
    HIPCK(hipStreamSynchronize(c->stream));
    return DEME_OK;
}
}

unsigned deme_tri_loads_block_rows(void) { return TRI_LOADS_BLOCK_ROWS; }

int deme_inspect_tri_loads(deme_ctx* c, float thr, uint32_t firstTri, uint32_t nTris, double* force, uint32_t* contacts) {
    if (int rc = check_ready(c))
        return rc;
    char msg[320];
    if (int rc = tri_loads_args_refused(msg, "deme_inspect_tri_loads", thr, firstTri, nTris, c->nTri, force, contacts))
        return fail(c, rc, "%s", msg);
    if (!nTris)
        return DEME_OK;
    if (records_refused(c))
        return fail(c, DEME_ERR_INVALID, "deme_inspect_tri_loads: %s", std::string(c->err).c_str());
    if (int rc = tri_loads_launch(c, thr))
        return rc;
    std::vector<double> hf(force ? (size_t)nTris * 3 : 0);
    std::vector<uint32_t> hn(contacts ? nTris : 0);
    if (int rc = tri_loads_fetch(c, firstTri, nTris, force ? hf.data() : nullptr, contacts ? hn.data() : nullptr))
        return rc;
    c->qHostBytes += (uint64_t)nTris * ((force ? 24 : 0) + (contacts ? 4 : 0));
    if (force)
        memcpy(force, hf.data(), hf.size() * 8);
    if (contacts)
        memcpy(contacts, hn.data(), hn.size() * 4);
    return DEME_OK;
}

namespace {
inline void owner_state_row(const DemeOwnerState* out, size_t at, const OwnerRec& r) {
#define DEME_COL(abi, T, Rec, f) if (out->abi) out->abi[at] = r.f;
    DEME_OWNER_COLS(DEME_COL, DEME_COL_NONE, DEME_COL_NONE)
#undef DEME_COL
    if (out->familyID) out->familyID[at] = (uint8_t)r.family;
}
}

int deme_query_owner_state(deme_ctx* c, const uint32_t* ownerIds, size_t n, DemeOwnerState* out) {
    if (int rc = check_ready(c))
        return rc;
    char msg[320];
    if (int rc = owner_ids_refused(msg, "deme_query_owner_state", out, "state", ownerIds, n, c->nOwners, out,
                                   "need the reduction a full download launches (deme_download_owner_state)", true))
        return fail(c, rc, "%s", msg);
    if (!n)
        return DEME_OK;
    std::vector<uint32_t> slots(n);
    for (size_t i = 0; i < n; i++)
        slots[i] = c->permuted ? c->hE2O[ownerIds[i]] : ownerIds[i];
    if (ensure(c, c->stage, n * 4) || ensure(c, c->qState, n * sizeof(OwnerRec)))
        return c->lastStatus;
    HIPCK(hipMemcpyAsync(c->stage.p, slots.data(), n * 4, hipMemcpyHostToDevice, c->stream));
    hipLaunchKernelGGL(k_query_owner_state, dim3(grid_for(n)), dim3(256), 0, c->stream, (uint32_t)n, c->owners.as<OwnerRec>(),
                       c->stage.as<uint32_t>(), (const uint32_t*)nullptr, SlabBooksDev{}, 0u, 0u, (const uint8_t*)nullptr,
                       c->qState.as<OwnerRec>(), (uint32_t)n, (uint32_t*)nullptr);
    std::vector<OwnerRec> h(n);
    HIPCK(hipMemcpyAsync(h.data(), c->qState.p, n * sizeof(OwnerRec), hipMemcpyDeviceToHost, c->stream));
    HIPCK(hipStreamSynchronize(c->stream));
    c->qHostBytes += (uint64_t)n * sizeof(OwnerRec);
    for (size_t i = 0; i < n; i++)
        owner_state_row(out, i, h[i]);
    return DEME_OK;
}
// ... 20 lines not shown
    HIPCK(hipMemcpyAsync(c->stage.p, keys.data(), n * 4, hipMemcpyHostToDevice, c->stream));
    HIPCK(hipMemcpyAsync(c->qState.p, patch.data(), n * sizeof(OwnerRec), hipMemcpyHostToDevice, c->stream));
    const uint32_t threads = byGid ? c->nOwners : (uint32_t)n;
    if (threads)
        hipLaunchKernelGGL(k_scatter_owner_state, dim3(grid_for(threads)), dim3(256), 0, c->stream, threads, c->owners.as<OwnerRec>(), c->nOwners,
                           c->stage.as<uint32_t>(), (uint32_t)n, c->qState.as<OwnerRec>(), mask, byGid ? c->dp.o2e : (const uint32_t*)nullptr,
                           byGid ? ownerGid : (const uint32_t*)nullptr);
    HIPCK(hipStreamSynchronize(c->stream));
    return DEME_OK;
}
}

int deme_scatter_owner_state(deme_ctx* c, const uint32_t* ownerIds, size_t n, const DemeOwnerState* in) {
    if (int rc = check_ready(c))
        return rc;
    char msg[320];
    std::vector<std::pair<uint32_t, uint32_t>> sorted;
    if (int rc = owner_ids_refused(msg, "deme_scatter_owner_state", in, "state", ownerIds, n, c->nOwners, in,
                                   "columns are not written by owner id (deme_upload_owner_state hands the accumulators to the caller)", true, &sorted))
        return fail(c, rc, "%s", msg);
    const uint32_t mask = owner_state_mask(in);
    if (!n || !mask)
        return DEME_OK;
    std::vector<uint32_t> slots(n);
    std::vector<OwnerRec> patch(n);
    for (size_t i = 0; i < n; i++) {
        slots[i] = c->permuted ? c->hE2O[ownerIds[i]] : ownerIds[i];
        patch[i] = owner_state_patch(in, i);
    }
    if (int rc = launch_owner_scatter(c, in, slots, patch, mask, false, nullptr))
        return rc;
    c->qHostBytes += (uint64_t)n * (4 + sizeof(OwnerRec));
    return DEME_OK;
}

namespace {
struct SortScratch {
    std::vector<void*> held;
    ~SortScratch() {
        for (void* p : held)
            (void)hipFree(p);
    }
    template <typename T>
    T* room(size_t n) {
        void* p = nullptr;
        if (hipMalloc(&p, std::max<size_t>(n, 1) * sizeof(T)) != hipSuccess)
            return nullptr;
        held.push_back(p);
        return reinterpret_cast<T*>(p);
    }
};
template <class RocCfg, bool HAS_V, typename K>
int sort_host_arrays(int device, const K* keys, const uint32_t* vals, size_t n, unsigned beginBit, unsigned endBit, size_t ownFrom, K* keysOut,
                     uint32_t* valsOut) {
    if (endBit < beginBit || endBit > 8 * sizeof(K) || (n && (!keys || !keysOut || (HAS_V && (!vals || !valsOut)))))
        return DEME_ERR_INVALID;
    if (!ownFrom && (DEME_SORT_ROCPRIM || n > deme_sort::MAX_N))
        return DEME_ERR_INVALID;
    if (!n)
        return DEME_OK;
    if (hipSetDevice(device) != hipSuccess)
        return DEME_ERR_HIP;
    SortScratch s;
    K *dIn = s.room<K>(n), *dOut = s.room<K>(n);
    uint32_t *vIn = HAS_V ? s.room<uint32_t>(n) : nullptr, *vOut = HAS_V ? s.room<uint32_t>(n) : nullptr;
    if (!dIn || !dOut || (HAS_V && (!vIn || !vOut)))
        return DEME_ERR_HIP;
    size_t bytes = 0;
    if (deme_radix_sort<RocCfg, HAS_V>(nullptr, bytes, dIn, dOut, vIn, vOut, n, n, beginBit, endBit, ownFrom, nullptr) != hipSuccess)
        return DEME_ERR_HIP;
    void* tmp = s.room<char>(bytes);
    if (!tmp)
        return DEME_ERR_HIP;
    bool ok = hipMemcpy(dIn, keys, n * sizeof(K), hipMemcpyHostToDevice) == hipSuccess;
    if (HAS_V)
        ok = ok && hipMemcpy(vIn, vals, n * 4, hipMemcpyHostToDevice) == hipSuccess;
    ok = ok && deme_radix_sort<RocCfg, HAS_V>(tmp, bytes, dIn, dOut, vIn, vOut, n, n, beginBit, endBit, ownFrom, nullptr) == hipSuccess;
    ok = ok && hipDeviceSynchronize() == hipSuccess;
    ok = ok && hipMemcpy(keysOut, dOut, n * sizeof(K), hipMemcpyDeviceToHost) == hipSuccess;
    if (HAS_V)
        ok = ok && hipMemcpy(valsOut, vOut, n * 4, hipMemcpyDeviceToHost) == hipSuccess;
    return ok ? DEME_OK : DEME_ERR_HIP;
}
}

unsigned deme_sort_tile_keys(void) { return deme_sort::TILE; }

int deme_sort_pairs_u32(int device, const uint32_t* keys, const uint32_t* vals, size_t n, unsigned beginBit, unsigned endBit, int forceOwn,
                        uint32_t* keysOut, uint32_t* valsOut) {
    const unsigned bits = endBit >= beginBit ? endBit - beginBit : 0;
    if (bits <= 20)
        return sort_host_arrays<DemeRadixCfg<10>, true>(device, keys, vals, n, beginBit, endBit, forceOwn ? 0 : DEME_SORT_OWN_FROM_RECORDS, keysOut,
                                                        valsOut);
    if (bits <= 22)
        return sort_host_arrays<DemeRadixCfg<11, 16>, true>(device, keys, vals, n, beginBit, endBit, forceOwn ? 0 : DEME_SORT_OWN_FROM_INCIDENCES,
                                                            keysOut, valsOut);
    return sort_host_arrays<DemeRadixCfg<8>, true>(device, keys, vals, n, beginBit, endBit, forceOwn ? 0 : DEME_SORT_OWN_FROM_INCIDENCES, keysOut,
                                                   valsOut);
}

int deme_sort_keys_u64(int device, const uint64_t* keys, size_t n, unsigned beginBit, unsigned endBit, int forceOwn, uint64_t* keysOut) {
    return sort_host_arrays<DemeRadixCfg<8>, false>(device, keys, nullptr, n, beginBit, endBit, forceOwn ? 0 : DEME_SORT_OWN_FROM_KEYS64, keysOut,
                                                    nullptr);
}

#include "deme_decomp.inc"
```

dem-engine_amd/csrc/deme_kernels.h:

```cpp
#pragma once
#include "deme_device.h"
#include "deme_owner_cols.h"

namespace deme_dev {

#define DEME_NULL_BINID_DEV 0xFFFFFFFFu
#define DEME_ST_VELOCITY 1u
#define DEME_ST_NONFINITE 2u
#define DEME_ST_INCIDENCE 4u
#define DEME_MAX_BINS_PER_SPHERE 0xFFFFFFu

struct DetectCounters {
    unsigned long long nContactsRaw;
    unsigned int nActiveBins;
    unsigned int maxInBin;
    unsigned int status;
    unsigned int pad0;
    unsigned long long nIncidence;
    unsigned int pad[8];
};

#define DEME_KEY_SEGS 64u
#define DEME_KEY_SEG_STRIDE 16u
struct DetectBlock {
    DetectCounters c;
    unsigned long long segCount[DEME_KEY_SEGS];
    unsigned long long segCtr[DEME_KEY_SEGS * DEME_KEY_SEG_STRIDE];
};
struct DetectHead {
    DetectCounters c;
    unsigned long long segCount[DEME_KEY_SEGS];
};
struct KeyArena {
    uint64_t* keys;
    unsigned long long* ctr;
    uint64_t segCap;
    uint32_t segMask;
};
__device__ inline uint32_t arena_seg(const KeyArena& a) {
    return blockIdx.x & a.segMask;
}
__device__ inline unsigned long long arena_reserve(const KeyArena& a, uint32_t seg, unsigned long long n) {
    return atomicAdd(&a.ctr[seg * DEME_KEY_SEG_STRIDE], n);
}
__device__ inline void arena_store(const KeyArena& a, uint32_t seg, unsigned long long slot, uint64_t key) {
    if (slot < a.segCap)
        a.keys[(uint64_t)seg * a.segCap + slot] = key;
}
__device__ void bin_stats_block(const uint2* __restrict__ perBlock, uint32_t nBlocks, uint32_t block, DetectCounters* ctr);
__global__ __launch_bounds__(256) void k_compact_keys(const uint64_t* __restrict__ in, uint64_t segCap, DetectBlock* blk, uint32_t xOff,
                                                      uint64_t* __restrict__ out, const uint2* __restrict__ stats, uint32_t nStats) {
    __shared__ unsigned long long sStart, sCount;
    const uint32_t seg = blockIdx.y;
    if (threadIdx.x < 64) {
        static_assert(DEME_KEY_SEGS == 64, "one lane per segment");
        const unsigned long long raw = blk->segCtr[threadIdx.x * DEME_KEY_SEG_STRIDE];
        if (stats && seg == 0 && blockIdx.x == 0)
            blk->segCount[threadIdx.x] = raw;
        const unsigned long long cnt = min(raw, (unsigned long long)segCap);
        unsigned long long inc = cnt;
        for (int d = 1; d < 64; d <<= 1) {
            const unsigned long long u = __shfl_up(inc, d);
            if ((int)threadIdx.x >= d)
                inc += u;
        }
        if (threadIdx.x == seg)
            sStart = inc - cnt, sCount = cnt;
    }
    __syncthreads();
    const uint64_t i = ((uint64_t)xOff + blockIdx.x) * blockDim.x + threadIdx.x;
    if (i < sCount)
        out[sStart + i] = in[(uint64_t)seg * segCap + i];
    if (stats && seg == 0)
        for (uint32_t b = blockIdx.x; b * 2048u < nStats; b += gridDim.x)
            bin_stats_block(stats, nStats, b, &blk->c);
}

__global__ __launch_bounds__(256) void k_margins(const DevParams p, OwnerRec* owners, uint32_t drift,
                                                 DetectCounters* ctr) {
    const uint32_t o = blockIdx.x * blockDim.x + threadIdx.x;
    if (o >= p.nOwners)
        return;
    OwnerRec* r = owners + o;
    const double vx = r->vx, vy = r->vy, vz = r->vz;
    float absv = (float)sqrt(vx * vx + vy * vy + vz * vz);
    if (!isfinite(absv))
        atomicOr(&ctr->status, DEME_ST_NONFINITE);
    else if (absv > p.errOutVel)
        atomicOr(&ctr->status, DEME_ST_VELOCITY);
    if (absv > p.approxMaxVel)
        absv = p.approxMaxVel;
    const float extra = p.familyTrivial ? 0.f : p.familyExtra[fam_of(r->family)];
    r->margin = (float)((double)(absv * p.expSafetyMulti + p.expSafetyAdder) * (double)p.h * (double)drift + (double)extra);
}

__global__ __launch_bounds__(256) void k_set_margins(uint32_t n, OwnerRec* owners, const float* m, const uint32_t* __restrict__ o2e) {
    const uint32_t o = blockIdx.x * blockDim.x + threadIdx.x;
    if (o < n)
        owners[o].margin = m[o2e ? o2e[o] : o];
}

struct ObjWorld {
    double x, y, z;
    float dx, dy, dz;
    float size1, nsign, margin;
    uint32_t type, family;
};

__global__ __launch_bounds__(256) void k_sphere_prep(const DevParams p, const OwnerRec* __restrict__ owners,
                                                     const SphereRec* __restrict__ spheres, GeoRec* __restrict__ geo,
                                                     uint4* __restrict__ binLo, uint2* __restrict__ binN,
                                                     uint32_t* __restrict__ partial, const KeyArena ar, DetectCounters* ctr,
                                                     uint16_t* __restrict__ sphFam) {
    __shared__ ObjWorld sObj[64];
    __shared__ uint32_t sWaveSum[4];
    const uint32_t s = blockIdx.x * blockDim.x + threadIdx.x;
    const bool valid = s < p.nSpheres;
    d3 pos{0, 0, 0};
    double rBin = 0;
    uint32_t fam = 0, myCount = 0;
    bool ghostOnce = false;
    if (valid) {
        const SphereRec sr = load_sphere(spheres, s);
        const OwnerRec o = load_owner(owners, sr.owner);
        const float4 c = p.comp[sr.comp];
        const d3 op = decode_pos(o.voxelID, o.locX, o.locY, o.locZ, p);
        const f3 rel = rot_apply(rot_coeffs(o.qw, o.qx, o.qy, o.qz), mk3(c.x, c.y, c.z));
        pos = {op.x + (double)rel.x, op.y + (double)rel.y, op.z + (double)rel.z};
        rBin = (double)c.w;
        rBin += o.margin;
        float rSweep = c.w;
        rSweep += o.margin;
        fam = fam_of(o.family);
        ghostOnce = ghost_of(o.family) && (p.hasGhosts & 2u);
        GeoRec g;
        g.x = pos.x, g.y = pos.y, g.z = pos.z, g.r = rSweep, g.owner = p.o2e ? p.o2e[sr.owner] : sr.owner;
        geo[s] = g;
        if (!(p.familyTrivial && !p.hasGhosts))
            sphFam[s] = (uint16_t)o.family;
        uint32_t lx, hx, ly, hy, lz, hz;
        bin_range(pos.x, rBin, p.binSize, p.nbX, lx, hx);
        bin_range(pos.y, rBin, p.binSize, p.nbY, ly, hy);
        bin_range(pos.z, rBin, p.binSize, p.nbZ, lz, hz);
        const uint32_t nx = hx - lx + 1, ny = hy - ly + 1, nz = hz - lz + 1;
        binLo[s] = make_uint4(lx, ly, lz, nx);
        binN[s] = make_uint2(ny, nz);
        const uint64_t n64 = (uint64_t)nx * ny * nz;
        if (n64 > DEME_MAX_BINS_PER_SPHERE)
            atomicOr(&ctr->status, DEME_ST_INCIDENCE);
        myCount = (n64 > DEME_MAX_BINS_PER_SPHERE) ? 0u : (uint32_t)n64;
    }
    {
        uint32_t sum = myCount;
        for (int off = 32; off > 0; off >>= 1)
            sum += (uint32_t)__shfl_xor((int)sum, off);
        if ((threadIdx.x & 63u) == 0)
            sWaveSum[threadIdx.x >> 6] = sum;
        __syncthreads();
        if (threadIdx.x == 0)
            partial[blockIdx.x] = sWaveSum[0] + sWaveSum[1] + sWaveSum[2] + sWaveSum[3];
    }

    for (uint32_t ob0 = 0; ob0 < p.nAnal; ob0 += 64) {
        __syncthreads();
        if (threadIdx.x < 64 && ob0 + threadIdx.x < p.nAnal) {
            const AnalObj ob = p.anal[ob0 + threadIdx.x];
            const OwnerRec o = load_owner(owners, ob.owner);
            const d3 op = decode_pos(o.voxelID, o.locX, o.locY, o.locZ, p);
            const RotM m = rot_coeffs(o.qw, o.qx, o.qy, o.qz);
            const f3 rp = rot_apply(m, mk3(ob.relx, ob.rely, ob.relz));
            const f3 rd = rot_apply(m, mk3(ob.rotx, ob.roty, ob.rotz));
            ObjWorld w;
            w.x = op.x + (double)rp.x, w.y = op.y + (double)rp.y, w.z = op.z + (double)rp.z;
            w.dx = rd.x, w.dy = rd.y, w.dz = rd.z;
            w.size1 = ob.size1, w.nsign = ob.normal, w.margin = o.margin;
            w.type = ob.type, w.family = fam_of(o.family);
            sObj[threadIdx.x] = w;
        }
        __syncthreads();
        {
            const uint32_t nHere = min(64u, p.nAnal - ob0);
            const uint32_t lane = threadIdx.x & 63u;
            for (uint32_t k = 0; k < nHere; k++) {
                const ObjWorld w = sObj[k];
                bool hit = valid && !ghostOnce;
                float thres = 0.f;
                if (hit && !p.familyTrivial) {
                    if (p.familyMasks[mask_pair(fam, w.family)] != 0)
                        hit = false;
                    const float ea = p.familyExtra[fam], eb = p.familyExtra[w.family];
                    thres = (ea < eb) ? ea : eb;
                }
                if (hit) {
                    d3 cp;
                    f3 nr;
                    double depth;
                    const uint32_t t = sphere_entity(pos, (float)rBin, w.type, {w.x, w.y, w.z}, mk3(w.dx, w.dy, w.dz),
                                                     w.size1, w.nsign, w.margin, cp, nr, depth);
                    hit = t && depth > (double)thres;
                }
                const unsigned long long m = __ballot(hit);
                if (m) {
                    const int leader = __ffsll((long long)m) - 1;
                    unsigned long long slot0 = 0;
                    if ((int)lane == leader)
                        slot0 = arena_reserve(ar, arena_seg(ar), (unsigned long long)__popcll(m));
                    slot0 = __shfl(slot0, leader);
                    const unsigned long long slot = slot0 + (unsigned long long)__popcll(m & ((1ull << lane) - 1ull));
                    if (hit)
                        arena_store(ar, arena_seg(ar), slot, make_key(DEME_KEY_CLASS_SA, s, ob0 + k));
                }
            }
        }
    }
}

#define DEME_SCAN_T 1024u
#define DEME_SCAN_IPT 4u
__global__ __launch_bounds__(DEME_SCAN_T) void k_scan_small(const uint32_t* in, uint32_t* out, uint32_t n, unsigned long long* totalOut) {
    __shared__ unsigned long long sWave[DEME_SCAN_T / 64];
    __shared__ unsigned long long sCarry;
    const uint32_t lane = threadIdx.x & 63u, w = threadIdx.x >> 6;
    if (threadIdx.x == 0)
        sCarry = 0;
    __syncthreads();
    for (uint32_t base = 0; base < n; base += DEME_SCAN_T * DEME_SCAN_IPT) {
        const uint32_t first = base + threadIdx.x * DEME_SCAN_IPT;
        uint32_t v[DEME_SCAN_IPT];
        unsigned long long sum = 0;
#pragma unroll
        for (uint32_t i = 0; i < DEME_SCAN_IPT; i++) {
            v[i] = first + i < n ? in[first + i] : 0u;
            sum += v[i];
        }
        unsigned long long inc = sum;
        for (int d = 1; d < 64; d <<= 1) {
            const unsigned long long u = __shfl_up(inc, d);
            if ((int)lane >= d)
                inc += u;
        }
        if (lane == 63)
            sWave[w] = inc;
        __syncthreads();
        unsigned long long run = sCarry + inc - sum, total = 0;
        for (uint32_t j = 0; j < DEME_SCAN_T / 64; j++) {
            const unsigned long long t = sWave[j];
            run += j < w ? t : 0ull;
            total += t;
        }
#pragma unroll
        for (uint32_t i = 0; i < DEME_SCAN_IPT; i++) {
            if (first + i < n)
                out[first + i] = (uint32_t)run;
            run += v[i];
        }
        __syncthreads();
        if (threadIdx.x == 0)
            sCarry += total;
        __syncthreads();
    }
    if (threadIdx.x == 0)
        *totalOut = sCarry;
}

__global__ __launch_bounds__(256) void k_fill_incidence(const DevParams p, const uint4* __restrict__ binLo,
                                                        const uint2* __restrict__ binN,
                                                        const uint32_t* __restrict__ partialPrefix,
                                                        uint32_t* __restrict__ keys, uint32_t* __restrict__ vals,
                                                        uint64_t cap) {
    __shared__ uint32_t sWaveSum[4];
    const uint32_t s = blockIdx.x * blockDim.x + threadIdx.x;
    const bool valid = s < p.nSpheres;
    const uint4 lo = valid ? binLo[s] : make_uint4(0u, 0u, 0u, 0u);
    const uint2 n = valid ? binN[s] : make_uint2(0u, 0u);
    const uint64_t n64 = (uint64_t)lo.w * n.x * n.y;
    const uint32_t cnt = n64 > DEME_MAX_BINS_PER_SPHERE ? 0u : (uint32_t)n64;
    const uint32_t lane = threadIdx.x & 63u, w = threadIdx.x >> 6;
    uint32_t inc = cnt;
    for (int d = 1; d < 64; d <<= 1) {
        const uint32_t u = (uint32_t)__shfl_up((int)inc, d);
        if ((int)lane >= d)
            inc += u;
    }
    if (lane == 63)
        sWaveSum[w] = inc;
    __syncthreads();
    uint32_t before = partialPrefix[blockIdx.x] + inc - cnt;
    for (uint32_t j = 0; j < 3; j++)
        before += j < w ? sWaveSum[j] : 0u;
    if (!cnt)
        return;
    uint64_t off = before;
    for (uint32_t k = lo.z; k < lo.z + n.y; k++)
        for (uint32_t j = lo.y; j < lo.y + n.x; j++)
            for (uint32_t i = lo.x; i < lo.x + lo.w; i++) {
                if (off < cap) {
                    keys[off] = i + j * p.nbX + k * p.nbX * p.nbY;
                    vals[off] = s;
                }
                off++;
            }
}

#ifndef SW_T
#define SW_T 256
#endif
#ifndef SW_WPB
#define SW_WPB 1
#endif
#define SW_W (2 * SW_T)
#define SW_OUT 256
#define SW_FLUSH 128

struct SweepLDS {
    float4 f[SW_W];
    uint32_t owner[SW_W], sph[SW_W], bin[SW_W];
    uint16_t fam[SW_W];
    uint32_t queue[SW_T / 64][128];
    uint64_t out[SW_OUT];
    unsigned long long gBase;
    unsigned long long headMask[SW_W / 64];
    uint32_t nOut;
    uint32_t start, endIdx, giant;
    uint32_t pop;
    uint32_t nBins, nextBin;
    uint16_t binStart[SW_W + 2];
};

__device__ inline bool pair_near(double ax, double ay, double az, float ar, uint32_t ao, double bx, double by, double bz, float br,
                                 uint32_t bo) {
    if (ao == bo)
        return false;
    const double rA = (double)ar, rB = (double)br;
    const double d2 = (ax - bx) * (ax - bx) + (ay - by) * (ay - by) + (az - bz) * (az - bz);
    return !(d2 > (rA + rB) * (rA + rB));
}

__device__ inline float sweep_radius(float x, float y, float z, float r) {
    const float mag = fabsf(x) + fabsf(y) + fabsf(z) + r;
    return (r + 0.5e-6f + 4e-7f * mag) * 1.00001f;
}
__device__ inline bool pair_near_f(float4 a, uint32_t ao, float4 b, uint32_t bo) {
    const float dx = a.x - b.x, dy = a.y - b.y, dz = a.z - b.z;
    const float rs = a.w + b.w;
    return (ao != bo) & (dx * dx + dy * dy + dz * dz <= rs * rs);
// ... 278 lines not shown
                    float mr = 0;
                    uint32_t mo = 0, mf = 0, ms = 0;
                    if (valid) {
                        ms = sphIds[jb];
                        const GeoRec g = geo[ms];
                        mx = g.x, my = g.y, mz = g.z, mr = g.r, mo = g.owner;
                        mf = (p.familyTrivial && !p.hasGhosts) ? 0u : sphFam[ms];
                    }
                    for (uint32_t i = 0; i < na; i++) {
                        const bool act = valid && (ta + i < jb);
                        bool hit = false;
                        uint64_t key = 0;
                        if (act) {
                            const GeoRec ga = geo[L.sph[i]];
                            const bool entryFirst = L.owner[i] <= mo;
                            const double ax = entryFirst ? ga.x : mx, ay = entryFirst ? ga.y : my, az = entryFirst ? ga.z : mz;
                            const double bx = entryFirst ? mx : ga.x, by = entryFirst ? my : ga.y, bz = entryFirst ? mz : ga.z;
                            const float ar_ = entryFirst ? ga.r : mr, br_ = entryFirst ? mr : ga.r;
                            const uint32_t ao = entryFirst ? L.owner[i] : mo, bo = entryFirst ? mo : L.owner[i];
                            const uint32_t af = entryFirst ? (uint32_t)L.fam[i] : mf, bf = entryFirst ? mf : (uint32_t)L.fam[i];
                            hit = pair_test(p, ax, ay, az, ar_, ao, af, bx, by, bz, br_, bo, bf, gbin);
                            if (hit)
                                key = entryFirst ? make_key(DEME_KEY_CLASS_SS, L.sph[i], ms) : make_key(DEME_KEY_CLASS_SS, ms, L.sph[i]);
                        }
                        sweep_emit(L, hit, key, lane, ar);
                    }
                    __syncthreads();
                    if (L.nOut >= SW_FLUSH)
                        sweep_flush(L, t, ar);
                }
            }
        }
        __syncthreads();
        if (t == 0) {
            uint32_t heads = (giantStart < SW_W) ? 1u : 0u;
            for (uint32_t ch = 0; ch < SW_W / 64; ch++)
                heads += (uint32_t)__popcll(L.headMask[ch]);
            winStats[win] = make_uint2(heads, max(L.pop, giantPop));
        }
        if (L.nOut >= SW_FLUSH)
            sweep_flush(L, t, ar);
    }
    __syncthreads();
    sweep_flush(L, t, ar);
}

__device__ void bin_stats_block(const uint2* __restrict__ perBlock, uint32_t nBlocks, uint32_t block, DetectCounters* ctr) {
    __shared__ uint32_t sHeads[4], sPop[4];
    uint32_t heads = 0, pop = 0;
    {
        const uint32_t i0 = block * 2048u;
        uint2 v[8];
#pragma unroll
        for (uint32_t k = 0; k < 8; k++) {
            const uint32_t i = i0 + k * 256u + threadIdx.x;
            v[k] = (i < nBlocks) ? perBlock[i] : make_uint2(0u, 0u);
        }
#pragma unroll
        for (uint32_t k = 0; k < 8; k++) {
            heads += v[k].x;
            pop = max(pop, v[k].y);
        }
    }
    for (int off = 32; off > 0; off >>= 1) {
        heads += (uint32_t)__shfl_xor((int)heads, off);
        pop = max(pop, (uint32_t)__shfl_xor((int)pop, off));
    }
    if ((threadIdx.x & 63u) == 0) {
        sHeads[threadIdx.x >> 6] = heads;
        sPop[threadIdx.x >> 6] = pop;
    }
    __syncthreads();
    if (threadIdx.x == 0) {
        atomicAdd(&ctr->nActiveBins, sHeads[0] + sHeads[1] + sHeads[2] + sHeads[3]);
        const uint32_t m = max(max(sPop[0], sPop[1]), max(sPop[2], sPop[3]));
        if (m > 1)
            atomicMax(&ctr->maxInBin, m);
    }
    __syncthreads();
}
__global__ __launch_bounds__(256) void k_bin_stats_final(const uint2* __restrict__ perBlock, uint32_t nBlocks, DetectCounters* ctr) {
    bin_stats_block(perBlock, nBlocks, blockIdx.x, ctr);
}

__global__ __launch_bounds__(256) void k_segment_rank_sort(uint32_t n, const uint64_t* __restrict__ in, uint64_t* __restrict__ out) {
    const uint32_t i = blockIdx.x * blockDim.x + threadIdx.x;
    if (i >= n)
        return;
    const uint64_t k = in[i], seg = k >> 31;
    uint32_t s = i, rank = 0;
    while (s > 0) {
        const uint64_t q = in[s - 1];
        if ((q >> 31) != seg)
            break;
        rank += (q <= k) ? 1u : 0u;
        s--;
    }
    for (uint32_t j = i + 1; j < n; j++) {
        const uint64_t q = in[j];
        if ((q >> 31) != seg)
            break;
        rank += (q < k) ? 1u : 0u;
    }
    out[s + rank] = k;
}

__global__ __launch_bounds__(256) void k_history(uint32_t nNew, const uint64_t* __restrict__ newKeys, uint32_t nPrev,
                                                 const uint64_t* __restrict__ prevKeys, uint32_t* __restrict__ mapping,
                                                 uint32_t* __restrict__ zeroA, uint32_t nZeroA, uint32_t* __restrict__ zeroB,
                                                 uint32_t nZeroB) {
    const uint32_t c = blockIdx.x * blockDim.x + threadIdx.x;
    for (uint32_t i = c; i < nZeroA; i += gridDim.x * blockDim.x)
        zeroA[i] = 0u;
    for (uint32_t i = c; i < nZeroB; i += gridDim.x * blockDim.x)
        zeroB[i] = 0u;
    if (c >= nNew)
        return;
    const uint64_t k = newKeys[c];
    uint32_t lo = 0, hi = nPrev;
    if (nPrev) {
        uint32_t g = (uint32_t)(((uint64_t)c * nPrev) / nNew);
        g = min(g, nPrev - 1);
        if (prevKeys[g] < k) {
            lo = g + 1;
            uint32_t step = 8;
            while (lo < nPrev) {
                const uint32_t j = (lo + step < nPrev) ? lo + step : nPrev - 1;
                if (prevKeys[j] < k) {
                    lo = j + 1;
                    step <<= 2;
                } else {
                    hi = j;
                    break;
                }
            }
        } else {
            hi = g;
            uint32_t step = 8;
            while (hi > 0) {
                const uint32_t j = (hi > step) ? hi - step : 0;
                if (prevKeys[j] < k) {
                    lo = j + 1;
                    break;
                }
                hi = j;
                step <<= 2;
            }
        }
    }
    while (lo < hi) {
        const uint32_t mid = lo + ((hi - lo) >> 1);
        if (prevKeys[mid] < k)
            lo = mid + 1;
        else
            hi = mid;
    }
    mapping[c] = (lo < nPrev && prevKeys[lo] == k) ? lo : 0xFFFFFFFFu;
}

__global__ __launch_bounds__(256) void k_migrate(uint32_t nNew, uint32_t nW, const uint32_t* __restrict__ mapping,
                                                 uint32_t nPrevStored, const float* __restrict__ oldW,
                                                 float* __restrict__ newW) {
    const uint32_t c = blockIdx.x * blockDim.x + threadIdx.x;
    if (c >= nNew)
        return;
    const uint32_t m = mapping[c];
    const bool have = (m != 0xFFFFFFFFu) && (m < nPrevStored);
    if (nW == 4) {
// ... 272 lines not shown
        const SphereRec sa = load_sphere(spheres, key_a(k));
        const uint32_t cls = key_class(k);
        uint32_t ob = 0, w = key_b(k);
        if (cls == DEME_KEY_CLASS_SS) {
            const SphereRec sb = load_sphere(spheres, key_b(k));
            ob = sb.owner;
            w = (uint32_t)sb.comp | ((uint32_t)sb.mat << 16);
        } else if (cls == DEME_KEY_CLASS_SA) {
            ob = p.anal[key_b(k)].owner;
        } else {
            ob = reinterpret_cast<const uint32_t*>(p.tris)[12 * (size_t)key_b(k) + 9];
        }
        ownerA[c] = sa.owner;
        ownerB[c] = ob;
        idx[c] = c;
        info[c] = make_uint4(sa.owner | (cls << 30), ob, (uint32_t)sa.comp | ((uint32_t)sa.mat << 16), w);
        if (smFlag)
            smFlag[c] = (cls == DEME_KEY_CLASS_SM) ? 1 : 0;
        if (tileRem) {
            tA = sa.owner / tileNB;
            remote = tA != ob / tileNB;
        }
    }
    if (tileRem) {
        unsigned long long todo = __ballot(remote);
        while (todo) {
            const int first = __ffsll((long long)todo) - 1;
            const uint32_t t0 = (uint32_t)__shfl((int)tA, first);
            const unsigned long long m = __ballot(remote && tA == t0);
            if ((int)(threadIdx.x & 63u) == first)
                atomicAdd(&tileRem[t0], (uint32_t)__popcll(m));
            todo &= ~m;
        }
    }
}

__global__ __launch_bounds__(256) void k_persist_flags(const DevParams p, uint32_t nC, const uint64_t* __restrict__ keys,
                                                       const SphereRec* __restrict__ spheres,
                                                       const OwnerRec* __restrict__ owners, int mode, uint32_t N1, uint32_t N2,
                                                       uint8_t* __restrict__ flag) {
    const uint32_t c = blockIdx.x * blockDim.x + threadIdx.x;
    if (c >= nC)
        return;
    const uint64_t k = keys[c];
    const uint32_t oa = load_sphere(spheres, key_a(k)).owner, cls = key_class(k);
    uint32_t ob;
    if (cls == DEME_KEY_CLASS_SS)
        ob = load_sphere(spheres, key_b(k)).owner;
    else if (cls == DEME_KEY_CLASS_SA)
        ob = p.anal[key_b(k)].owner;
    else
        ob = reinterpret_cast<const uint32_t*>(p.tris)[12 * (size_t)key_b(k) + 9];
    const uint32_t fA = fam_of(owners[oa].family), fB = fam_of(owners[ob].family);
    const bool q = mode == 0 || (mode == 1 && (fA == N1 || fB == N1)) || (mode == 2 && fA == N1 && fB == N1) ||
                   (mode == 3 && ((fA == N1 && fB == N2) || (fA == N2 && fB == N1)));
    flag[c] = q ? 1 : 0;
}

__device__ inline uint32_t lower_bound_u32(const uint32_t* a, uint32_t n, uint32_t v) {
    uint32_t lo = 0, hi = n;
    while (lo < hi) {
        const uint32_t mid = lo + ((hi - lo) >> 1);
        if (a[mid] < v)
            lo = mid + 1;
        else
            hi = mid;
    }
    return lo;
}

#define DEME_HEAVY_THRESHOLD 256u
struct RangeCounters {
    unsigned int nHeavy;
    unsigned int nHeavyFree;
    unsigned int nSA, nSM;
    unsigned int tileOverflow;
    unsigned int tileMaxHalo, tileMaxList;
    unsigned int nBig;
    unsigned int nExtra;
    unsigned int tileHaloSum;
    unsigned int nBigIn;
    unsigned int tileMaxHaloIn;
    unsigned long long nRemote;
    unsigned int pad[2];
};

__global__ __launch_bounds__(256) void k_run_starts(uint32_t n, const uint32_t* __restrict__ owner, uint32_t nOwners,
                                                    uint32_t* __restrict__ start) {
    const uint32_t i = blockIdx.x * blockDim.x + threadIdx.x;
    if (i >= n)
        return;
    const uint32_t cur = owner[i];
    const uint32_t first = (i == 0) ? 0u : owner[i - 1] + 1u;
    for (uint32_t o = first; o <= cur && o <= nOwners; o++)
        start[o] = i;
    if (i == n - 1)
        for (uint32_t o = cur + 1; o <= nOwners; o++)
            start[o] = n;
}

__global__ __launch_bounds__(256) void k_owner_ranges(const DevParams p, uint32_t nC, const uint32_t* __restrict__ ownerA,
                                                      const uint32_t* __restrict__ ownerBSorted,
                                                      const OwnerRec* __restrict__ owners, uint32_t* __restrict__ aStart,
                                                      uint32_t* __restrict__ bStart, uint8_t* __restrict__ heavy,
                                                      uint8_t* __restrict__ fixedFlag, uint32_t* __restrict__ heavyList,
                                                      uint32_t heavyCap, RangeCounters* rc,
                                                      const uint4* __restrict__ info, uint8_t* __restrict__ cDefer,
                                                      uint32_t* __restrict__ blockMode) {
    const uint32_t o = blockIdx.x * blockDim.x + threadIdx.x;
    if (o > p.nOwners)
        return;
    if (o == p.nOwners)
        return;
    const uint32_t a0 = aStart[o], a1 = aStart[o + 1];
    const uint32_t b0 = bStart[o], b1 = bStart[o + 1];
    const uint32_t fw = owners[o].family;
    const bool isFixed = (p.familyFlags[fam_of(fw)] & 1u) != 0 || ghost_of(fw);
    fixedFlag[o] = isFixed ? 1 : 0;
    if (cDefer) {
        bool d = ghost_of(fw);
        for (uint32_t c = a0; c < a1 && !d; c++)
            d = ghost_of(owners[info[c].y].family);
        for (uint32_t c = a0; c < a1; c++) {
            cDefer[c] = d ? 1 : 0;
            if (c == a0 || (c % DEME_FORCE_BLOCK) == 0)
                atomicOr(&blockMode[c / DEME_FORCE_BLOCK], d ? 2u : 1u);
        }
    }
    const bool hv = (a1 - a0) + (b1 - b0) > DEME_HEAVY_THRESHOLD || shared_of(fw);
    heavy[o] = hv ? 1 : 0;
    if (hv) {
        const unsigned int slot = atomicAdd(&rc->nHeavy, 1u);
        if (slot < heavyCap)
            heavyList[slot] = o;
        if (!isFixed)
            atomicAdd(&rc->nHeavyFree, 1u);
    }
}

struct PrescArgs {
    const PrescRec* rec;
    const uint32_t* slot;
};

#define DEME_INT_STAGE (64 * 5)
__device__ inline void lds_wave_fence() {
    __builtin_amdgcn_fence(__ATOMIC_RELEASE, "wavefront");
    __builtin_amdgcn_wave_barrier();
    __builtin_amdgcn_fence(__ATOMIC_ACQUIRE, "wavefront");
}
__device__ inline OwnerRec coop_load_owner(const OwnerRec* owners, uint32_t nOwners, uint32_t waveBase, uint4* stage) {
    const uint32_t lane = threadIdx.x & 63u;
    const uint4* src = reinterpret_cast<const uint4*>(owners) + (size_t)waveBase * 4;
    const uint32_t lim = (nOwners > waveBase ? min(64u, nOwners - waveBase) : 0u) * 4u;
    uint4 v[4];
#pragma unroll
    for (uint32_t k = 0; k < 4; k++) {
        const uint32_t e = k * 64u + lane;
        v[k] = (e < lim) ? src[e] : make_uint4(0, 0, 0, 0);
    }
#pragma unroll
    for (uint32_t k = 0; k < 4; k++) {
        const uint32_t e = k * 64u + lane;
        stage[(e >> 2) * 5u + (e & 3u)] = v[k];
    }
    lds_wave_fence();
    OwnerRec r;
    uint4* q = reinterpret_cast<uint4*>(&r);
    const uint4* mine = stage + lane * 5u;
    q[0] = mine[0], q[1] = mine[1], q[2] = mine[2], q[3] = mine[3];
    return r;
}
// ... 390 lines not shown
```

dem-engine_amd/csrc/deme_sort.h:

```cpp
#pragma once
#include <cstdint>
#include <hip/hip_runtime.h>
#include <rocprim/block/block_scan.hpp>

namespace deme_sort {

#ifndef DEME_SORT_THREADS
#define DEME_SORT_THREADS 512
#endif
#ifndef DEME_SORT_KPT
#define DEME_SORT_KPT 8
#endif
constexpr unsigned THREADS = DEME_SORT_THREADS, WAVE = 64, WAVES = THREADS / WAVE;
constexpr unsigned SCAN_THREADS = 256;
constexpr unsigned RB = 8, RADIX = 1u << RB;
constexpr unsigned KPT = DEME_SORT_KPT;
constexpr unsigned TILE = THREADS * KPT;
constexpr unsigned SCAN_IPT = 16;
constexpr size_t MAX_N = (size_t)1 << 31;
static_assert(THREADS >= RADIX && THREADS % WAVE == 0, "one thread per digit in the histogram steps");
static_assert(WAVE == 64, "ballots are 64 lanes wide");

using BlockScan = rocprim::block_scan<uint32_t, THREADS>;
using RowScan = rocprim::block_scan<uint32_t, SCAN_THREADS>;

template <typename K>
__device__ inline unsigned digit_of(K k, unsigned shift, unsigned mask) {
    return (unsigned)(k >> shift) & mask;
}

template <typename K>
__global__ __launch_bounds__(THREADS) void k_count(const K* __restrict__ keys, uint32_t n, uint32_t nTiles, unsigned shift, unsigned nbits,
                                                   uint32_t* __restrict__ table) {
    constexpr unsigned COPIES = 4;
    __shared__ uint32_t hist[COPIES * RADIX];
    const unsigned tid = threadIdx.x, tile = blockIdx.x, mask = (1u << nbits) - 1u;
    for (unsigned d = tid; d < COPIES * RADIX; d += THREADS)
        hist[d] = 0;
    __syncthreads();
    const uint32_t base = tile * TILE + tid;
    K k[KPT];
#pragma unroll
    for (unsigned i = 0; i < KPT; i++)
        k[i] = base + i * THREADS < n ? keys[base + i * THREADS] : K(0);
#pragma unroll
    for (unsigned i = 0; i < KPT; i++)
        if (base + i * THREADS < n)
            atomicAdd(&hist[digit_of(k[i], shift, mask) * COPIES + tid % COPIES], 1u);
    __syncthreads();
    if (tid <= mask) {
        uint32_t c = 0;
#pragma unroll
        for (unsigned j = 0; j < COPIES; j++)
            c += hist[tid * COPIES + j];
        table[(size_t)tid * nTiles + tile] = c;
    }
}

__global__ __launch_bounds__(SCAN_THREADS) void k_scan_rows(uint32_t* __restrict__ table, uint32_t nTiles, uint32_t* __restrict__ totals) {
    __shared__ typename RowScan::storage_type scanSt;
    uint32_t* row = table + (size_t)blockIdx.x * nTiles;
    uint32_t carry = 0;
    for (uint32_t base = 0; base < nTiles; base += SCAN_THREADS * SCAN_IPT) {
        const uint32_t first = base + threadIdx.x * SCAN_IPT;
        uint32_t v[SCAN_IPT], sum = 0;
#pragma unroll
        for (unsigned i = 0; i < SCAN_IPT; i++) {
            v[i] = first + i < nTiles ? row[first + i] : 0u;
            sum += v[i];
        }
        uint32_t excl, total;
        RowScan().exclusive_scan(sum, excl, 0u, total, scanSt);
        __syncthreads();
        uint32_t run = carry + excl;
#pragma unroll
        for (unsigned i = 0; i < SCAN_IPT; i++) {
            if (first + i < nTiles)
                row[first + i] = run;
            run += v[i];
        }
        carry += total;
    }
    if (threadIdx.x == 0)
        totals[blockIdx.x] = carry;
}

template <typename K, bool HAS_V>
__global__ __launch_bounds__(THREADS) void k_scatter(const K* __restrict__ keys, const uint32_t* __restrict__ vals, uint32_t n, uint32_t nTiles,
                                                     unsigned shift, unsigned nbits, const uint32_t* __restrict__ table,
                                                     const uint32_t* __restrict__ totals, K* __restrict__ keysOut, uint32_t* __restrict__ valsOut) {
    __shared__ typename BlockScan::storage_type scanSt;
    __shared__ K sKeys[TILE];
    __shared__ uint32_t sVals[HAS_V ? TILE : 1];
    __shared__ uint32_t wcnt[WAVES * RADIX];
    __shared__ uint32_t gbase[RADIX];
    const unsigned tid = threadIdx.x, lane = tid % WAVE, w = tid / WAVE, tile = blockIdx.x, mask = (1u << nbits) - 1u;
    const uint32_t tile0 = tile * TILE, nValid = n - tile0 < TILE ? n - tile0 : TILE;
    for (unsigned d = tid; d < WAVES * RADIX; d += THREADS)
        wcnt[d] = 0;
    K k[KPT];
    uint32_t v[KPT], rank[KPT];
#pragma unroll
    for (unsigned i = 0; i < KPT; i++) {
        const uint32_t at = w * (WAVE * KPT) + i * WAVE + lane;
        k[i] = at < nValid ? keys[tile0 + at] : ~K(0);
        if (HAS_V)
            v[i] = at < nValid ? vals[tile0 + at] : 0u;
    }
    __syncthreads();
    uint32_t* wc = wcnt + w * RADIX;
#pragma unroll
    for (unsigned i = 0; i < KPT; i++) {
        const unsigned d = digit_of(k[i], shift, mask);
        unsigned long long same = ~0ull;
#pragma unroll
        for (unsigned b = 0; b < RB; b++) {
            const bool bit = (d >> b) & 1u;
            const unsigned long long bal = __ballot(bit);
            same &= bit ? bal : ~bal;
        }
        const uint32_t before = __hip_atomic_load(wc + d, __ATOMIC_RELAXED, __HIP_MEMORY_SCOPE_WAVEFRONT);
        if ((same >> lane) == 1ull)
            __hip_atomic_fetch_add(wc + d, (uint32_t)__popcll(same), __ATOMIC_RELAXED, __HIP_MEMORY_SCOPE_WAVEFRONT);
        rank[i] = before + (uint32_t)__popcll(same & ((1ull << lane) - 1ull));
    }
    __syncthreads();
    const unsigned dt = tid % RADIX;
    uint32_t pre[WAVES], c = 0;
#pragma unroll
    for (unsigned j = 0; j < WAVES; j++) {
        pre[j] = c;
        c += tid < RADIX ? wcnt[j * RADIX + dt] : 0u;
    }
    uint32_t dstart, dbase;
    BlockScan().exclusive_scan(c, dstart, 0u, scanSt);
    __syncthreads();
    BlockScan().exclusive_scan(tid <= mask ? totals[tid] : 0u, dbase, 0u, scanSt);
    if (tid < RADIX) {
#pragma unroll
        for (unsigned j = 0; j < WAVES; j++)
            wcnt[j * RADIX + dt] = dstart + pre[j];
    }
    if (tid <= mask)
        gbase[tid] = dbase + table[(size_t)tid * nTiles + tile] - dstart;
    __syncthreads();
#pragma unroll
    for (unsigned i = 0; i < KPT; i++) {
        const uint32_t p = wcnt[w * RADIX + digit_of(k[i], shift, mask)] + rank[i];
        sKeys[p] = k[i];
        if (HAS_V)
            sVals[p] = v[i];
    }
    __syncthreads();
#pragma unroll
    for (unsigned i = 0; i < KPT; i++) {
        const uint32_t p = i * THREADS + tid;
        if (p < nValid) {
            const K key = sKeys[p];
            const uint32_t o = gbase[digit_of(key, shift, mask)] + p;
            if (o < n) {
                keysOut[o] = key;
                if (HAS_V)
                    valsOut[o] = sVals[p];
            }
        }
    }
}

inline size_t align256(size_t b) { return (b + 255) & ~(size_t)255; }
inline unsigned passes_for(unsigned beginBit, unsigned endBit) { return (endBit - beginBit + RB - 1) / RB; }

template <typename K, bool HAS_V>
hipError_t radix_sort(void* tmp, size_t& bytes, const K* keysIn, K* keysOut, const uint32_t* valsIn, uint32_t* valsOut, size_t n, size_t cap,
                      unsigned beginBit, unsigned endBit, hipStream_t st) {
    const size_t room = n > cap ? n : cap, tilesRoom = (room + TILE - 1) / TILE;
    const size_t tableB = align256((tilesRoom + 1) * RADIX * 4), keysB = align256(room * sizeof(K)), valsB = HAS_V ? align256(room * 4) : 0;
    if (!tmp) {
        bytes = tableB + keysB + valsB;
        return hipSuccess;
    }
    if (bytes < tableB + keysB + valsB || room > MAX_N || endBit < beginBit || endBit > 8 * sizeof(K))
        return hipErrorInvalidValue;
    if (!n)
        return hipSuccess;
    const unsigned passes = passes_for(beginBit, endBit);
    if (!passes) {
        hipError_t e = hipMemcpyAsync(keysOut, keysIn, n * sizeof(K), hipMemcpyDeviceToDevice, st);
        if (e == hipSuccess && HAS_V)
            e = hipMemcpyAsync(valsOut, valsIn, n * 4, hipMemcpyDeviceToDevice, st);
        return e;
    }
    uint32_t* table = reinterpret_cast<uint32_t*>(tmp);
    uint32_t* totals = table + tilesRoom * RADIX;
    K* keysAlt = reinterpret_cast<K*>(reinterpret_cast<char*>(tmp) + tableB);
    uint32_t* valsAlt = reinterpret_cast<uint32_t*>(reinterpret_cast<char*>(tmp) + tableB + keysB);
    const uint32_t nTiles = (uint32_t)((n + TILE - 1) / TILE);
    const K* kSrc = keysIn;
    const uint32_t* vSrc = valsIn;
    for (unsigned p = 0; p < passes; p++) {
        const unsigned shift = beginBit + p * RB, nbits = endBit - shift < RB ? endBit - shift : RB;
        const bool toOut = (passes - 1 - p) % 2 == 0;
        K* kDst = toOut ? keysOut : keysAlt;
        uint32_t* vDst = toOut ? valsOut : valsAlt;
        hipLaunchKernelGGL(k_count<K>, dim3(nTiles), dim3(THREADS), 0, st, kSrc, (uint32_t)n, nTiles, shift, nbits, table);
        hipLaunchKernelGGL(k_scan_rows, dim3(1u << nbits), dim3(SCAN_THREADS), 0, st, table, nTiles, totals);
        hipLaunchKernelGGL((k_scatter<K, HAS_V>), dim3(nTiles), dim3(THREADS), 0, st, kSrc, vSrc, (uint32_t)n, nTiles, shift, nbits, table,
                           totals, kDst, vDst);
        kSrc = kDst, vSrc = vDst;
    }
    return hipGetLastError();
}

}
```

dem-engine_amd/csrc/deme_tile.h:

```cpp
#pragma once
#include "deme_force_fast.h"

#ifndef DEME_TILE_NB
#define DEME_TILE_NB 128
#endif
#ifndef DEME_TILE_HMAX
#define DEME_TILE_HMAX 192
#endif
#ifndef DEME_TILE_T
#define DEME_TILE_T 256
#endif
#define DEME_TILE_HP2 256
#define DEME_TILE_LREG 4
#define DEME_TILE_LMAX (DEME_TILE_LREG * DEME_TILE_T)
static_assert(DEME_TILE_T >= 2 * DEME_TILE_NB, "one pulling thread per owner and side");
static_assert(DEME_TILE_NB + DEME_TILE_HMAX <= 2 * DEME_TILE_T, "a thread stages at most two owner records");
static_assert(DEME_TILE_LMAX == DEME_TILE_LREG * DEME_TILE_T, "list entries per thread");
#define DEME_TILE_HASH 1024u
#ifndef DEME_TILE_REC
#define DEME_TILE_REC 6
#endif
#define DEME_TILE_REC_USER 5
#ifndef DEME_JIT_NW
#define DEME_JIT_NW 1
// ... 647 lines not shown
                __attribute__((aligned(16))) uint4 sa[DEME_TILE_REC], sb[DEME_TILE_REC];
                const OwnerRec ra = load_owner(a.owners, oa), rb = load_owner(a.owners, ob);
                tile_stage<MODEL>(p, p.massProps[ra.inertiaOff].x, ra, u0x, u0y, u0z, sa);
                tile_stage<MODEL>(p, p.massProps[rb.inertiaOff].x, rb, u0x, u0y, u0z, sb);
                const TileOwner A = tile_read<MODEL>(sa, 0u, 0u), B = tile_read<MODEL>(sb, 0u, 0u);
                if (MODEL == 2) {
                    constexpr int NWU = DEME_JIT_NW;
                    float uw[NWU];
#pragma unroll
                    for (int k = 0; k < NWU; k++)
                        uw[k] = DEME_JIT_HAS_WC ? a.wc[(size_t)c * NWU + k] : 0.f;
                    TileUser U;
                    U.ox = (double)u0x * p.l + (double)p.LBFX, U.oy = (double)u0y * p.l + (double)p.LBFY, U.oz = (double)u0z * p.l + (double)p.LBFZ;
                    U.ownerA = oa, U.ownerB = ob;
                    U.c = c, U.keys = a.keys, U.ownerWc = a.ownerWc, U.geoWcSph = a.geoWcSph, U.geoWcAnal = a.geoWcAnal, U.time = a.timeElapsed;
                    tile_contact<MODEL>(p, T, ci, A, B, h, force, tA, tB, uw, &U);
                    if (DEME_JIT_HAS_WC) {
#pragma unroll
                        for (int k = 0; k < NWU; k++)
                            a.wc[(size_t)c * NWU + k] = uw[k];
                    }
                } else if (REC) {
                    TileRecOut ro;
                    tile_contact<MODEL>(p, T, ci, A, B, h, force, tA, tB, nullptr, nullptr, &ro);
                    float* r = a.rec[0] + 3ull * c;
                    r[0] = force.x, r[1] = force.y, r[2] = force.z;
                    r = a.rec[1] + 3ull * c;
                    r[0] = ro.torqueOnly.x, r[1] = ro.torqueOnly.y, r[2] = ro.torqueOnly.z;
                    r = a.rec[2] + 3ull * c;
                    r[0] = ro.locA.x, r[1] = ro.locA.y, r[2] = ro.locA.z;
                    r = a.rec[3] + 3ull * c;
                    r[0] = ro.locB.x, r[1] = ro.locB.y, r[2] = ro.locB.z;
                } else {
                    tile_contact<MODEL>(p, T, ci, A, B, h, force, tA, tB);
                }
                if (MODEL == 0)
                    stream_store(wc4 + c, h);
            }
            recA4[tid] = make_float4(force.x, force.y, force.z, tA.x);
            recA2[tid] = make_float2(tA.y, tA.z);
            const uint32_t k = a.rankC[c];
            float2* const r24 = reinterpret_cast<float2*>(a.rec32) + 3 * (size_t)k;
            stream_store(r24, make_float2(-force.x, -force.y));
            stream_store(r24 + 1, make_float2(-force.z, tB.x));
            stream_store(r24 + 2, make_float2(tB.y, tB.z));
        }
        __syncthreads();
        if (sideA) {
            const uint32_t e = min(phi, rlo + DEME_TILE_T);
            while (plo < e) {
                float4 v4[4];
                float2 v2[4];
#pragma unroll
                for (int k = 0; k < 4; k++) {
                    const uint32_t i = (plo + k < e) ? plo + k - rlo : (uint32_t)DEME_TILE_T;
                    v4[k] = recA4[i], v2[k] = recA2[i];
                }
#pragma unroll
                for (int k = 0; k < 4; k++) {
                    s01 += v2f{v4[k].x, v4[k].y};
                    s23 += v2f{v4[k].z, v4[k].w};
                    s45 += v2f{v2[k].x, v2[k].y};
                }
                plo = min(plo + 4u, e);
            }
        }
        __syncthreads();
    }
    if (sideA) {
        float2* const t24 = reinterpret_cast<float2*>(a.tSum) + 3 * (size_t)(o0 + tid);
        t24[0] = make_float2(s01.x, s01.y), t24[1] = make_float2(s23.x, s23.y), t24[2] = make_float2(s45.x, s45.y);
    }
}

#ifndef DEME_JIT
__global__ __launch_bounds__(256) void k_tile_build(const DevParams p, uint32_t nOwners, const uint4* __restrict__ info,
                                                    const uint32_t* __restrict__ ownerBList,
                                                    const uint32_t* __restrict__ aStart, const OwnerRec* __restrict__ owners,
                                                    const uint32_t* __restrict__ tileBase, uint2* __restrict__ tInfo,
                                                    uint32_t* __restrict__ hList, uint32_t* __restrict__ hCount,
                                                    uint32_t* __restrict__ tileMode, uint16_t* __restrict__ lOff,
                                                    uint16_t* __restrict__ lPos, uint32_t* __restrict__ lCount,
                                                    uint32_t* __restrict__ rankC, uint32_t* __restrict__ remKey,
                                                    uint32_t* __restrict__ remVal, int64_t* __restrict__ org, RangeCounters* rc,
                                                    uint32_t nTiles, uint32_t* __restrict__ tileBig, uint32_t* __restrict__ bigList,
                                                    uint32_t* __restrict__ recContact) {
    __shared__ uint32_t table[DEME_TILE_HASH];
    __shared__ uint16_t slotTab[DEME_TILE_HASH];
    __shared__ uint32_t list[DEME_TILE_HP2];
    __shared__ uint32_t cnt[DEME_TILE_NB], off[DEME_TILE_NB + 1], wsum[4];
    __shared__ uint16_t lp[DEME_TILE_LMAX];
    __shared__ uint32_t nU, nL, anyGhost;
    const uint32_t t = blockIdx.x, tid = threadIdx.x, lane = tid & 63u, wave = tid >> 6;
    const uint32_t o0 = t * DEME_TILE_NB, o1 = min(o0 + (uint32_t)DEME_TILE_NB, nOwners);
    const uint32_t c0 = aStart[o0], c1 = aStart[o1];
    for (uint32_t i = tid; i < DEME_TILE_HASH; i += 256)
        table[i] = 0xFFFFFFFFu;
    for (uint32_t i = tid; i < DEME_TILE_HP2; i += 256)
        list[i] = 0xFFFFFFFFu;
    if (tid < DEME_TILE_NB)
        cnt[tid] = 0;
    if (tid == 0)
        nU = 0, nL = 0, anyGhost = 0;
    __syncthreads();
    for (uint32_t c = c0 + tid; c < c1; c += 256) {
        const uint32_t ob = ownerBList[c];
        if (ob >= o0 && ob < o1) {
            atomicAdd(&cnt[ob - o0], 1u);
            continue;
        }
        uint32_t h = (ob * 2654435761u) >> 22;
        while (*(volatile uint32_t*)&nU <= DEME_TILE_HMAX) {
            const uint32_t old = atomicCAS(&table[h], 0xFFFFFFFFu, ob);
            if (old == 0xFFFFFFFFu) {
                const uint32_t slot = atomicAdd(&nU, 1u);
                slotTab[h] = (uint16_t)slot;
                if (slot < DEME_TILE_HP2)
                    list[slot] = ob;
                break;
            }
            if (old == ob)
                break;
            h = (h + 1u) & (DEME_TILE_HASH - 1u);
        }
    }
    __syncthreads();
    {
        static_assert(DEME_TILE_NB <= 256, "the builder has one thread per owner of the tile");
        uint32_t v = (tid < DEME_TILE_NB) ? cnt[tid] : 0u, inc = v;
        for (int d = 1; d < 64; d <<= 1) {
            const uint32_t u = (uint32_t)__shfl_up((int)inc, d);
            if ((int)lane >= d)
                inc += u;
        }
        if (lane == 63u)
            wsum[wave] = inc;
        __syncthreads();
        if (tid < DEME_TILE_NB) {
            uint32_t base = 0;
            for (uint32_t w = 0; w < wave; w++)
                base += wsum[w];
            off[tid] = base + inc - v;
            if (tid == DEME_TILE_NB - 1u)
                off[DEME_TILE_NB] = base + inc;
        }
        __syncthreads();
    }
    const uint32_t n = nU, nLoc = off[DEME_TILE_NB];
    if (n > DEME_TILE_HMAX || c1 - c0 > DEME_TILE_CMAX || nLoc > DEME_TILE_LMAX) {
        __shared__ uint32_t extraBase, bigGhost;
        if (tid == 0) {
            tileBig[t] = 1u;
            bigList[atomicAdd(&rc->nBig, 1u)] = t;
            extraBase = tileBase[nTiles] + atomicAdd(&rc->nExtra, nLoc);
            bigGhost = 0;
            hCount[t] = 0;
            lCount[t] = 0;
            int64_t ux, uy, uz;
            pos_units(load_owner(owners, o0), p, ux, uy, uz);
            org[3 * (size_t)t] = ux, org[3 * (size_t)t + 1] = uy, org[3 * (size_t)t + 2] = uz;
        }
        for (uint32_t i = tid; i <= DEME_TILE_NB; i += 256)
            lOff[(size_t)t * (DEME_TILE_NB + 1) + i] = 0;
        __syncthreads();
        uint32_t runR = tileBase[t], runL = extraBase;
        bool g = false;
        for (uint32_t cb = c0; cb < c1; cb += 256) {
            const uint32_t c = cb + tid;
            bool remote = false, local = false;
            uint32_t ob = 0;
            if (c < c1) {
                ob = ownerBList[c];
                local = ob >= o0 && ob < o1;
                remote = !local;
                if (tileMode)
                    g = g || ghost_of(owners[ob].family) || ghost_of(owners[info[c].x & 0x3FFFFFFFu].family);
            }
            const unsigned long long mr = __ballot(remote), ml = __ballot(local);
            if (lane == 0)
                wsum[wave] = (uint32_t)__popcll(mr) | ((uint32_t)__popcll(ml) << 16);
            __syncthreads();
            uint32_t beforeR = 0, beforeL = 0, totR = 0, totL = 0;
            for (uint32_t w = 0; w < 4; w++) {
                const uint32_t v = wsum[w];
                beforeR += (w < wave) ? (v & 0xFFFFu) : 0u, beforeL += (w < wave) ? (v >> 16) : 0u;
                totR += v & 0xFFFFu, totL += v >> 16;
            }
            if (c < c1) {
                const unsigned long long below = (1ull << lane) - 1ull;
                const uint32_t r = remote ? runR + beforeR + (uint32_t)__popcll(mr & below) : runL + beforeL + (uint32_t)__popcll(ml & below);
                rankC[c] = r;
                remKey[r] = ob, remVal[r] = r, recContact[r] = c;
            }
            runR += totR, runL += totL;
            __syncthreads();
        }
        if (tileMode) {
            if (g)
                bigGhost = 1;
            __syncthreads();
            if (tid == 0)
                tileMode[t] = bigGhost ? 2u : 1u;
        }
        return;
    }
    if (tid == 0)
        tileBig[t] = 0u;
    if (tid < DEME_TILE_NB)
        cnt[tid] = 0;
    __syncthreads();
    for (uint32_t i = tid; i < n; i += 256)
        hList[(size_t)t * DEME_TILE_HMAX + i] = list[i];
    if (tid == 0) {
        hCount[t] = n;
        lCount[t] = nLoc;
        int64_t ux, uy, uz;
        pos_units(load_owner(owners, o0), p, ux, uy, uz);
        org[3 * (size_t)t] = ux, org[3 * (size_t)t + 1] = uy, org[3 * (size_t)t + 2] = uz;
    }
    if (tileMode) {
        bool g = false;
        for (uint32_t i = tid; i < (o1 - o0) + n; i += 256)
            g = g || ghost_of(owners[i < o1 - o0 ? o0 + i : list[i - (o1 - o0)]].family);
        if (g)
            anyGhost = 1;
        __syncthreads();
        if (tid == 0)
            tileMode[t] = anyGhost ? 2u : 1u;
    }
    uint32_t run = tileBase[t];
    for (uint32_t cb = c0; cb < c1; cb += 256) {
        const uint32_t c = cb + tid;
        bool remote = false;
        uint32_t ob = 0;
        if (c < c1) {
            const uint4 ci = info[c];
            const uint32_t oa = ci.x & 0x3FFFFFFFu, cls = ci.x >> 30;
            ob = ci.y;
            uint32_t slotB;
            if (ob >= o0 && ob < o1) {
                slotB = ob - o0;
                lp[off[slotB] + atomicAdd(&cnt[slotB], 1u)] = (uint16_t)(c - c0);
            } else {
                uint32_t h = (ob * 2654435761u) >> 22;
                while (table[h] != ob)
                    h = (h + 1u) & (DEME_TILE_HASH - 1u);
                slotB = DEME_TILE_NB + slotTab[h];
                remote = true;
            }
            const uint32_t matA = ci.z >> 16, compA = ci.z & 0xFFFFu;
            const uint32_t matB = (cls == DEME_KEY_CLASS_SS) ? (ci.w >> 16) : 0u;
            const uint32_t wB = (cls == DEME_KEY_CLASS_SS) ? (ci.w & 0xFFFFu) : ci.w;
            tInfo[c] = make_uint2(tile_info_x(oa - o0, slotB, cls, remote ? 1u : 0u, matA, matB), compA | (wB << 16));
        }
        const unsigned long long m = __ballot(remote);
        if (lane == 0)
            wsum[wave] = (uint32_t)__popcll(m);
        __syncthreads();
        uint32_t before = 0, total = 0;
        for (uint32_t w = 0; w < 4; w++) {
            const uint32_t v = wsum[w];
            before += (w < wave) ? v : 0u;
            total += v;
        }
        const uint32_t r = run + before + (uint32_t)__popcll(m & ((1ull << lane) - 1ull));
        if (c < c1) {
            rankC[c] = r;
            if (remote)
                remKey[r] = ob, remVal[r] = r, recContact[r] = c;
        }
        run += total;
        __syncthreads();
    }
    if (tid < DEME_TILE_NB) {
        const uint32_t b = off[tid], e = off[tid + 1];
        for (uint32_t i = b + 1; i < e; i++) {
            const uint16_t v = lp[i];
            uint32_t j = i;
            while (j > b && lp[j - 1] > v) {
                lp[j] = lp[j - 1];
                j--;
            }
            lp[j] = v;
        }
    }
    __syncthreads();
    for (uint32_t i = tid; i < nLoc; i += 256)
        lPos[c0 + i] = lp[i];
    for (uint32_t i = tid; i <= DEME_TILE_NB; i += 256)
        lOff[(size_t)t * (DEME_TILE_NB + 1) + i] = (uint16_t)off[i];
}

__global__ __launch_bounds__(256) void k_tile_stats(uint32_t nTiles, const uint32_t* __restrict__ hCount,
                                                    const uint32_t* __restrict__ lCount, RangeCounters* rc) {
    __shared__ uint32_t mh[4], ml[4], sh[4];
    uint32_t a = 0, b = 0, sum = 0;
    for (uint32_t k = 0; k < 4; k++) {
        const uint32_t t = (blockIdx.x * 4u + k) * 256u + threadIdx.x;
        if (t < nTiles)
            a = max(a, hCount[t]), b = max(b, lCount[t]), sum += hCount[t];
    }
    for (int o = 32; o > 0; o >>= 1) {
        a = max(a, (uint32_t)__shfl_xor((int)a, o));
        b = max(b, (uint32_t)__shfl_xor((int)b, o));
        sum += (uint32_t)__shfl_xor((int)sum, o);
    }
    if ((threadIdx.x & 63u) == 0)
        mh[threadIdx.x >> 6] = a, ml[threadIdx.x >> 6] = b, sh[threadIdx.x >> 6] = sum;
    __syncthreads();
    if (threadIdx.x == 0) {
        atomicAdd(&rc->tileHaloSum, sh[0] + sh[1] + sh[2] + sh[3]);
        atomicMax(&rc->tileMaxHalo, max(max(mh[0], mh[1]), max(mh[2], mh[3])));
        atomicMax(&rc->tileMaxList, max(max(ml[0], ml[1]), max(ml[2], ml[3])));
    }
}

__global__ __launch_bounds__(256) void k_owner_ranges_tile(const DevParams p, const OwnerRec* __restrict__ owners,
                                                           const uint32_t* __restrict__ aStart, const uint16_t* __restrict__ lOff,
                                                           const uint32_t* __restrict__ rStart, uint8_t* __restrict__ heavy,
                                                           uint8_t* __restrict__ fixedFlag, uint32_t* __restrict__ heavyList,
                                                           uint32_t heavyCap, RangeCounters* rc) {
    const uint32_t o = blockIdx.x * blockDim.x + threadIdx.x;
    if (o >= p.nOwners)
        return;
    const uint32_t t = o / DEME_TILE_NB, k = o - t * DEME_TILE_NB;
    const uint16_t* lo = lOff + (size_t)t * (DEME_TILE_NB + 1);
    const uint32_t nA = aStart[o + 1] - aStart[o], nB = (uint32_t)(lo[k + 1] - lo[k]) + (rStart[o + 1] - rStart[o]);
    const uint32_t fw = owners[o].family;
    const bool isFixed = (p.familyFlags[fam_of(fw)] & 1u) != 0 || ghost_of(fw);
    fixedFlag[o] = isFixed ? 1 : 0;
    const bool hv = nA + nB > DEME_HEAVY_THRESHOLD || shared_of(fw);
    heavy[o] = hv ? 1 : 0;
    if (hv) {
        const unsigned int slot = atomicAdd(&rc->nHeavy, 1u);
        if (slot < heavyCap)
            heavyList[slot] = o;
        if (!isFixed)
            atomicAdd(&rc->nHeavyFree, 1u);
    }
}

#endif

}

#pragma clang fp contract(off)
```

include/deme_hip.h:

```cpp
#ifndef DEME_HIP_H
#define DEME_HIP_H

#include <stddef.h>
#include <stdint.h>

#ifdef __cplusplus
extern "C" {
#endif

#define DEME_NOT_A_CONTACT 0
#define DEME_SPHERE_SPHERE_CONTACT 1
#define DEME_SPHERE_MESH_CONTACT 2
#define DEME_SPHERE_PLANE_CONTACT 11
#define DEME_SPHERE_CYL_CONTACT 13

#define DEME_ANAL_OBJ_TYPE_PLANE 0
#define DEME_ANAL_OBJ_TYPE_PLATE 1
#define DEME_ANAL_OBJ_TYPE_CYL_INF 2

#define DEME_NULL_MAPPING_PARTNER 0xFFFFFFFFu
#define DEME_NULL_BINID 0xFFFFFFFFu
#define DEME_NUM_FAMILIES 256
#define DEME_FAMILY_MASK_ENTRIES 32896
#define DEME_MAX_WILDCARD_NUM 16
// ... 78 lines not shown
    uint64_t* voxelID;
    uint16_t *locX, *locY, *locZ;
    float *oriQw, *oriQx, *oriQy, *oriQz;
    float *vX, *vY, *vZ;
    float *omgBarX, *omgBarY, *omgBarZ;
    float *aX, *aY, *aZ;
    float *alphaX, *alphaY, *alphaZ;
    uint8_t* familyID;
} DemeOwnerState;

typedef struct DemeCounts {
    uint64_t nContacts;
    uint64_t nPrevContacts;
    uint64_t nBinSphereTouches;
    uint64_t nActiveBins;
    uint64_t nSteps;
    uint64_t nDetections;
    uint32_t maxSpheresInBin;
    uint32_t lastStatus;
} DemeCounts;

typedef struct deme_ctx deme_ctx;

int deme_ctx_create(int device, deme_ctx** out);
void deme_ctx_destroy(deme_ctx* ctx);
const char* deme_last_error(const deme_ctx* ctx);
const char* deme_version(void);
int deme_ctx_set_stream(deme_ctx* ctx, void* hip_stream);
int deme_sync(deme_ctx* ctx);

#define DEME_ARITH_FAST 1
#define DEME_ARITH_EXACT 0
int deme_set_arith_mode(deme_ctx* ctx, int mode);
int deme_get_arith_mode(const deme_ctx* ctx);
int deme_tile_stats(const deme_ctx* ctx, uint32_t out[4]);
int deme_heavy_owners(deme_ctx* ctx, uint32_t out[2]);
int deme_set_tile_policy(deme_ctx* ctx, uint32_t minContactsPerTileCustom);
int deme_force_kernel_name(const deme_ctx* ctx, char* name, size_t cap, uint32_t* tileMaxHalo, uint32_t* tileMaxList);
int deme_set_fused_step(deme_ctx* ctx, int on);

int deme_get_order(const deme_ctx* ctx, int* reordered, double spread[2]);
int deme_set_reorder(deme_ctx* ctx, int enable);
int deme_renew_order(deme_ctx* ctx);
int deme_order_renewals(const deme_ctx* ctx, uint64_t* n);
int deme_order_probe(const DemeParams* p, size_t nClumps, const uint64_t* voxelID, const uint16_t* locX, const uint16_t* locY,
                     const uint16_t* locZ, uint32_t* order, double spread[2]);

int deme_set_params(deme_ctx* ctx, const DemeParams* p);
int deme_upload_scene(deme_ctx* ctx, const DemeScene* s);
int deme_upload_owner_state(deme_ctx* ctx, const DemeOwnerState* st);
int deme_download_owner_state(deme_ctx* ctx, DemeOwnerState* st);
int deme_update_tri_nodes(deme_ctx* ctx, const float* n1, const float* n2, const float* n3);

int deme_compute_margins(deme_ctx* ctx, uint32_t drift);
int deme_set_margins(deme_ctx* ctx, const float* marginSize);

int deme_detect_contacts(deme_ctx* ctx);
int deme_migrate_history(deme_ctx* ctx);
int deme_calc_forces(deme_ctx* ctx);
int deme_integrate(deme_ctx* ctx);
int deme_step(deme_ctx* ctx, uint32_t nsteps);
int deme_set_async_detection(deme_ctx* ctx, uint32_t leadSteps);

int deme_get_counts(deme_ctx* ctx, DemeCounts* out);

int deme_download_bin_incidence(deme_ctx* ctx, uint32_t* binIDs, uint32_t* sphereIDs, size_t cap);
int deme_download_contacts(deme_ctx* ctx, uint32_t* idA, uint32_t* idB, uint8_t* type, uint32_t* mapping, size_t cap);
int deme_download_contact_wildcard(deme_ctx* ctx, uint32_t w, float* out, size_t cap);
int deme_upload_contact_wildcard(deme_ctx* ctx, uint32_t w, const float* in, size_t n);
int deme_seed_contacts(deme_ctx* ctx, const uint32_t* idA, const uint32_t* idB, const uint8_t* type, const float* wildcards,
                       size_t n);
int deme_set_record_contacts(deme_ctx* ctx, int enable);
int deme_download_contact_records(deme_ctx* ctx, float* force, float* torqueOnly, float* cpA, float* cpB, size_t cap);
int deme_query_owner_contacts(deme_ctx* ctx, const uint32_t* ownerIds, size_t nOwners, int withRecords, uint32_t* idA, uint32_t* idB,
                              uint8_t* type, uint32_t* ownerA, uint32_t* ownerB, uint8_t* side, float* force, float* torqueOnly,
                              float* cpA, float* cpB, size_t cap, size_t* nOut);
int deme_query_host_bytes(const deme_ctx* ctx, uint64_t* bytes);
int deme_query_owner_state(deme_ctx* ctx, const uint32_t* ownerIds, size_t n, DemeOwnerState* out);
int deme_scatter_owner_state(deme_ctx* ctx, const uint32_t* ownerIds, size_t n, const DemeOwnerState* in);
int deme_sort_pairs_u32(int device, const uint32_t* keys, const uint32_t* vals, size_t n, unsigned beginBit, unsigned endBit, int forceOwn,
                        uint32_t* keysOut, uint32_t* valsOut);
int deme_sort_keys_u64(int device, const uint64_t* keys, size_t n, unsigned beginBit, unsigned endBit, int forceOwn, uint64_t* keysOut);
unsigned deme_sort_tile_keys(void);
int deme_download_sphere_geometry(deme_ctx* ctx, double* X, double* Y, double* Z, float* R, size_t cap);

int deme_change_owner_sizes(deme_ctx* ctx, const uint32_t* ownerIds, const float* factors, size_t n);
int deme_num_components(const deme_ctx* ctx, uint32_t* n);
int deme_download_components(deme_ctx* ctx, float* relX, float* relY, float* relZ, float* radius, size_t cap);
int deme_download_sphere_components(deme_ctx* ctx, uint16_t* comp, size_t cap);
int deme_set_template_components(deme_ctx* ctx, uint32_t n);

int deme_compile_force_model(deme_ctx* ctx, const char* src, size_t len, const char* const* wildcardNames,
                             uint32_t nWildcards, const char* prerequisites);

int deme_compile_prescriptions(deme_ctx* ctx, const char* velCases, const char* posCases, const char* accCases);

int deme_compile_family_rules(deme_ctx* ctx, const char* rules);
int deme_change_family(deme_ctx* ctx, uint32_t from, uint32_t to);

typedef struct DemeAdaptive {
    uint32_t autoBinSize;
    uint32_t binObserveSteps;
    float binMaxRate;
    float binAcc;
    float binUpperSafety;
    float binLowerSafety;
    uint32_t autoUpdateFreq;
    uint32_t maxUpdateFreq;
    uint32_t freqObserveDetections;
} DemeAdaptive;
int deme_set_adaptive(deme_ctx* ctx, const DemeAdaptive* a);
int deme_get_adaptive_state(deme_ctx* ctx, double* binSize, uint32_t* cdUpdateFreq, uint32_t* nBinChanges, uint32_t* nFreqChanges);

int deme_add_owner_acc(deme_ctx* ctx, uint32_t owner, uint32_t n, const float* acc, const float* angAcc);

int deme_mark_persistent_contacts(deme_ctx* ctx, int mode, uint32_t N1, uint32_t N2, int mark);
int deme_num_persistent_contacts(deme_ctx* ctx, size_t* n);
int deme_download_persistent_contacts(deme_ctx* ctx, uint32_t* idA, uint32_t* idB, uint8_t* type, size_t cap);
int deme_upload_persistent_contacts(deme_ctx* ctx, const uint32_t* idA, const uint32_t* idB, const uint8_t* type, size_t n);

int deme_compile_force_model_ex(deme_ctx* ctx, const char* src, size_t len, const char* const* contactWildcards, uint32_t nContactWc,
                                const char* const* ownerWildcards, uint32_t nOwnerWc, const char* const* geoWildcards,
                                uint32_t nGeoWc, const char* prerequisites);
int deme_upload_wildcard_array(deme_ctx* ctx, uint32_t kind, uint32_t index, const float* in, size_t n);
int deme_download_wildcard_array(deme_ctx* ctx, uint32_t kind, uint32_t index, float* out, size_t cap);

int deme_set_family_material(deme_ctx* ctx, uint32_t family, uint32_t material, int kind);
int deme_device_memory(deme_ctx* ctx, size_t* usedBytes, size_t* totalBytes);

int deme_jit_probe(const char* src, const char* const* wildcardNames, uint32_t nWildcards, const char* prerequisites,
                   char* log, size_t logCap);
int deme_jit_probe_ex(const char* src, const char* const* wildcardNames, uint32_t nWildcards, const char* const* ownerNames,
                      uint32_t nOwnerWc, const char* const* geoNames, uint32_t nGeoWc, const char* prerequisites, char* log,
                      size_t logCap);

#define DEME_INSPECT_CLUMP_MAX_Z 0
#define DEME_INSPECT_CLUMP_MIN_Z 1
#define DEME_INSPECT_CLUMP_MAX_ABSV 2
#define DEME_INSPECT_CLUMP_MASS 3
#define DEME_INSPECT_MAX_ABSV 4
#define DEME_INSPECT_CLUMP_KINETIC_ENERGY 5
#define DEME_INSPECT_ABSV 6
#define DEME_INSPECT_CLUMP_VOLUME 7
int deme_inspect(deme_ctx* ctx, uint32_t quantity, float* out);
int deme_inspect_values(deme_ctx* ctx, uint32_t quantity, float* out, size_t cap);
int deme_compile_region(deme_ctx* ctx, const char* code, int* regionId);
int deme_inspect_region(deme_ctx* ctx, uint32_t quantity, int regionId, float* out);
int deme_upload_volumes(deme_ctx* ctx, const float* volumes, size_t n);
typedef struct DemeContactSums {
    double virial[9];
    uint64_t sides;
    uint64_t clumps;
} DemeContactSums;
int deme_inspect_contacts(deme_ctx* ctx, int regionId, float forceThreshold, DemeContactSums* out);
int deme_inspect_contact_counts(deme_ctx* ctx, int regionId, float forceThreshold, uint32_t* perOwner, size_t cap);
int deme_inspect_tri_loads(deme_ctx* ctx, float forceThreshold, uint32_t firstTri, uint32_t nTris, double* force ,
                           uint32_t* contacts );
unsigned deme_tri_loads_block_rows(void);

int deme_kernel_time_ms(deme_ctx* ctx, const char* name, double* avg_ms, uint64_t* launches);
int deme_kernel_time_reset(deme_ctx* ctx);
int deme_set_timing(deme_ctx* ctx, int enable);

#define DEME_GHOST_BYTES 56
int deme_halo_pack(deme_ctx* ctx, const uint32_t* d_ownerIDs, uint32_t n, void* d_buf);
int deme_halo_unpack(deme_ctx* ctx, const uint32_t* d_ownerIDs, uint32_t n, const void* d_buf);
// ... 104 lines not shown
```

Baseline: 6.503 billion.

## Launch radix sorts before host readback using device-side lengths

Incidence and contact-key radix sorts are now enqueued before the host waits on the counter readback. They use an upper bound estimated from the previous step's length, and the real length is read from a device counter inside the sort kernels. Readback sync moves to an event recorded before the sort, so the host can inspect counts while the sort runs; if the bound is exceeded, the normal sort path runs again. The explicit remVal index array is also dropped in favour of a counting iterator or implicit iota. This adds idle-tile launches for the bounded grid and extra complexity in the fallback paths.

```diff
diff --git a/dem-engine_amd/abi.py b/dem-engine_amd/abi.py
--- a/dem-engine_amd/abi.py
+++ b/dem-engine_amd/abi.py
@@ -797,6 +797,32 @@
     return ko
 
 
+def sort_pairs_u32_devlen(keys, vals, length, begin_bit, end_bit, fill=0xFFFFFFFF, device=0):
+    keys = np.ascontiguousarray(keys, np.uint32)
+    vals = None if vals is None else np.ascontiguousarray(vals, np.uint32)
+    assert keys.ndim == 1 and (vals is None or vals.shape == keys.shape)
+    ko, vo = np.full_like(keys, fill), np.full_like(keys, fill)
+    fn = load_library().deme_sort_pairs_u32_devlen
+    fn.argtypes, fn.restype = [C.c_int, _P, _P, C.c_size_t, C.c_uint32, C.c_uint, C.c_uint, _P, _P], C.c_int
+    rc = fn(device, _ptr(keys), _ptr(vals), keys.size, int(length), begin_bit, end_bit, _ptr(ko),
+                                                   _ptr(vo))
+    if rc:
+        raise DemeError(f"deme_sort_pairs_u32_devlen failed with code {rc}")
+    return ko, vo
+
+
+def sort_keys_u64_devlen(keys, length, begin_bit, end_bit, fill=0xFFFFFFFFFFFFFFFF, device=0):
+    keys = np.ascontiguousarray(keys, np.uint64)
+    assert keys.ndim == 1
+    ko = np.full_like(keys, fill)
+    fn = load_library().deme_sort_keys_u64_devlen
+    fn.argtypes, fn.restype = [C.c_int, _P, C.c_size_t, C.c_uint32, C.c_uint, C.c_uint, _P], C.c_int
+    rc = fn(device, _ptr(keys), keys.size, int(length), begin_bit, end_bit, _ptr(ko))
+    if rc:
+        raise DemeError(f"deme_sort_keys_u64_devlen failed with code {rc}")
+    return ko
+
+
 def jit_probe(src, wildcard_names=(), prerequisites="", owner_wildcards=(), geo_wildcards=()):
     lib = load_library()
 
diff --git a/dem-engine_amd/csrc/deme_hip.hip b/dem-engine_amd/csrc/deme_hip.hip
--- a/dem-engine_amd/csrc/deme_hip.hip
+++ b/dem-engine_amd/csrc/deme_hip.hip
@@ -56,7 +56,7 @@
 };
 
 struct ContactList {
-    DevBuf mapping, ownerA, ownerB[2], bIdx[2], info, tInfo, rIdx, lPos, remVal, rankC, remKey[2], cDefer, blockMode, smFlag, smList;
+    DevBuf mapping, ownerA, ownerB[2], bIdx[2], info, tInfo, rIdx, lPos, rankC, remKey[2], cDefer, blockMode, smFlag, smList;
     DevBuf aStart, bStart, heavy, fixedFlag, heavyList, rangeCtr, hList, hCount, tileMode, tileOrg, rStart, lOff, lCount, tileRem, tileBase,
         tileBig, bigList;
     uint64_t nListed = 0;
@@ -76,7 +76,7 @@
         nBigTiles = tileMaxHalo = tileMaxList = tileMaxHaloIn = 0;
     }
     std::array<DevBuf*, 35> buffers() {
-        return {&mapping, &ownerA, &ownerB[0], &ownerB[1], &bIdx[0], &bIdx[1], &info, &tInfo, &rIdx, &lPos, &remVal, &rankC, &remKey[0],
+        return {&mapping, &ownerA, &ownerB[0], &ownerB[1], &bIdx[0], &bIdx[1], &info, &tInfo, &rIdx, &lPos, &rankC, &remKey[0],
                 &remKey[1], &cDefer, &blockMode, &smFlag, &smList, &aStart, &bStart, &heavy, &fixedFlag, &heavyList, &rangeCtr, &hList,
                 &hCount, &tileMode, &tileOrg, &rStart, &lOff, &lCount, &tileRem, &tileBase, &tileBig, &bigList};
     }
@@ -126,7 +126,11 @@
     uint64_t nFusedSteps = 0;
     DevBuf ownersNext, recContact, inCnt, inStart, tInfoIn, inContact, hCountIn;
     uint32_t tileMinContactsCustom = 320;
+    int sortAhead = 1;
+    size_t ownFromInc = 0, ownFromKeys = 0, ownFromRecs = 0;
+    uint64_t lastIncLen = 0, lastKeyLen = 0, lastRecLen = 0;
     uint64_t lastSegMax = 0;
+    hipEvent_t evReadback = nullptr;
     size_t keySegMin = (size_t)1 << 20;
     DevBuf persistKeys, binStat;
     DevBuf nextAcc;
@@ -259,18 +263,21 @@
 static inline T* pin_at(deme_ctx* c, size_t off) {
     return reinterpret_cast<T*>(c->pin + off);
 }
-static hipError_t sync_readback(deme_ctx* c, hipStream_t st, bool spin) {
+static hipError_t mark_readback(deme_ctx* c, hipStream_t st) {
+    return hipEventRecord(c->evReadback, st);
+}
+static hipError_t sync_readback(deme_ctx* c, bool spin) {
     if (c->spinSync && spin) {
         const auto t0 = std::chrono::steady_clock::now();
         for (int it = 0;; it++) {
-            const hipError_t q = hipStreamQuery(st);
+            const hipError_t q = hipEventQuery(c->evReadback);
             if (q != hipErrorNotReady)
                 return q;
             if ((it & 255) == 255 && std::chrono::steady_clock::now() - t0 > std::chrono::milliseconds(5))
                 break;
         }
     }
-    return hipStreamSynchronize(st);
+    return hipEventSynchronize(c->evReadback);
 }
 
 int ensure(deme_ctx* c, DevBuf& b, size_t bytes, bool keep = false) {
@@ -329,10 +336,19 @@
                            unsigned beginBit, unsigned endBit, size_t ownFrom, hipStream_t st) {
     if (sort_takes_own(n, cap, ownFrom))
         return deme_sort::radix_sort<K, HAS_V>(tmp, bytes, keysIn, keysOut, valsIn, valsOut, n, cap, beginBit, endBit, st);
-    if constexpr (HAS_V)
+    if constexpr (HAS_V) {
+        if (!valsIn)
+            return rocprim::radix_sort_pairs<RocCfg>(tmp, bytes, keysIn, keysOut, rocprim::counting_iterator<uint32_t>(0), valsOut, n, beginBit,
+                                                     endBit, st);
         return rocprim::radix_sort_pairs<RocCfg>(tmp, bytes, keysIn, keysOut, valsIn, valsOut, n, beginBit, endBit, st);
-    else
+    } else
         return rocprim::radix_sort_keys<RocCfg>(tmp, bytes, keysIn, keysOut, n, beginBit, endBit, st);
+}
+inline bool sort_goes_ahead(const deme_ctx* c, uint64_t lastLen, size_t ownFrom, size_t bound) {
+    return c->sortAhead && !DEME_SORT_ROCPRIM && lastLen >= ownFrom && lastLen > 0 && bound > 0 && bound <= deme_sort::MAX_N;
+}
+inline size_t ahead_bound(uint64_t lastLen, size_t cap) {
+    return (size_t)std::min<uint64_t>(cap, lastLen + lastLen / 4 + 1024);
 }
 
 inline unsigned grid_for(size_t n, unsigned block = 256) { return (unsigned)((n + block - 1) / block); }
@@ -468,7 +484,6 @@
     rc |= ensure(c, L.tInfo, cap * 8);
     rc |= ensure(c, L.rIdx, cap * 4);
     rc |= ensure(c, L.lPos, cap * 2);
-    rc |= ensure(c, L.remVal, (cap + 1) * 4);
     rc |= ensure(c, L.rankC, (cap + 1) * 4);
     rc |= ensure(c, L.remKey[0], (cap + 1) * 4);
     rc |= ensure(c, L.remKey[1], (cap + 1) * 4);
@@ -577,10 +592,11 @@
                                c->binLo.as<uint4>(), c->binN.as<uint2>(), c->binPartial.as<uint32_t>(),
                                ar, c->ctr.as<DetectCounters>(), c->sphFam.as<uint16_t>());
             hipLaunchKernelGGL(k_scan_small, dim3(1), dim3(DEME_SCAN_T), 0, st, c->binPartial.as<uint32_t>(), c->binPartial.as<uint32_t>(),
-                               grid_for(nS), &blk->c.nIncidence);
+                               grid_for(nS), &blk->c.nIncidence, &blk->nIncSort, (unsigned long long)c->incCap);
         }
         uint32_t P = 0;
-        bool filled = false;
+        bool filled = false, incSorted = false;
+        const unsigned bits = bits_for((uint64_t)c->hp.nbX * c->hp.nbY * c->hp.nbZ, 32);
         auto fill_incidence = [&]() {
             hipLaunchKernelGGL(k_fill_incidence, dim3(grid_for(nS)), dim3(256), 0, st, c->dp,
                                c->binLo.as<uint4>(), c->binN.as<uint2>(), c->binPartial.as<uint32_t>(),
@@ -590,8 +606,23 @@
         if (nS && c->incCap)
             fill_incidence();
         if (nS) {
+            const bool ahead = filled && sort_goes_ahead(c, c->lastIncLen, c->ownFromInc, c->incCap);
+            const size_t incBound = ahead_bound(c->lastIncLen, c->incCap);
+            size_t aheadBytes = 0;
+            if (ahead) {
+                HIPCK((deme_sort::radix_sort<uint32_t, true>(nullptr, aheadBytes, nullptr, nullptr, nullptr, nullptr, incBound, c->incCap, 0, bits, st)));
+                if (int rc = ensure(c, c->sortTmp, aheadBytes))
+                    return rc;
+            }
             HIPCK(hipMemcpyAsync(pin_at<DetectCounters>(c, 1024), c->ctr.p, sizeof(hc), hipMemcpyDeviceToHost, st));
-            HIPCK(sync_readback(c, st, !async));
+            HIPCK(mark_readback(c, st));
+            if (ahead) {
+                aheadBytes = c->sortTmp.bytes;
+                HIPCK((deme_sort::radix_sort<uint32_t, true>(c->sortTmp.p, aheadBytes, c->incKeys[0].as<uint32_t>(), c->incKeys[1].as<uint32_t>(),
+                                                             c->incVals[0].as<uint32_t>(), c->incVals[1].as<uint32_t>(), incBound, c->incCap, 0,
+                                                             bits, st, &blk->nIncSort)));
+            }
+            HIPCK(sync_readback(c, !async));
             hc = *pin_at<DetectCounters>(c, 1024);
             if (!statusSeen) {
                 statusSeen = true;
@@ -606,26 +637,28 @@
                 return fail(c, DEME_ERR_OVERFLOW, "%llu bin-sphere incidences do not fit the 32-bit list offsets (use larger bins)",
                             hc.nIncidence);
             P = (uint32_t)hc.nIncidence;
+            incSorted = ahead && P <= incBound;
         }
         if (P > c->incCap) {
+            HIPCK(hipStreamSynchronize(st));
             if (int rc = grow_incidence_arena(c, (size_t)P + P / 4 + 1024))
                 return rc;
-            filled = false;
-        }
-        c->nInc = P;
+            filled = incSorted = false;
+        }
+        c->nInc = c->lastIncLen = P;
         uint32_t nStats = 0;
-        const unsigned bits = bits_for((uint64_t)c->hp.nbX * c->hp.nbY * c->hp.nbZ, 32);
         if (P) {
             if (!filled)
                 fill_incidence();
             const bool twoPass = bits > 16 && bits <= 22;
+            if (!incSorted)
             if (int rc = with_temp(c, c->sortTmp, [&](void* tmp, size_t& bytes) {
                     return twoPass ? deme_radix_sort<DemeRadixCfg<11, 16>, true>(tmp, bytes, c->incKeys[0].as<uint32_t>(), c->incKeys[1].as<uint32_t>(),
                                                                                  c->incVals[0].as<uint32_t>(), c->incVals[1].as<uint32_t>(), (size_t)P,
-                                                                                 (size_t)c->incCap, 0, bits, DEME_SORT_OWN_FROM_INCIDENCES, st)
+                                                                                 (size_t)c->incCap, 0, bits, c->ownFromInc, st)
                                    : deme_radix_sort<DemeRadixCfg<8>, true>(tmp, bytes, c->incKeys[0].as<uint32_t>(), c->incKeys[1].as<uint32_t>(),
                                                                             c->incVals[0].as<uint32_t>(), c->incVals[1].as<uint32_t>(), (size_t)P,
-                                                                            (size_t)c->incCap, 0, bits, DEME_SORT_OWN_FROM_INCIDENCES, st);
+                                                                            (size_t)c->incCap, 0, bits, c->ownFromInc, st);
                 }))
                 return rc;
             const uint32_t nWin = (uint32_t)grid_for(P, SW_T);
@@ -677,16 +710,36 @@
                                    c->sphFam.as<uint16_t>(), ar);
             }
         }
-        const int nextEarly = c->keysCur ^ 1;
+        const int next = c->keysCur ^ 1;
         uint32_t compactBlocks = 0;
         if (segmented) {
             compactBlocks = (uint32_t)std::min<uint64_t>(grid_for(std::max<uint64_t>(c->lastSegMax + c->lastSegMax / 8 + 1024, 1)), grid_for(ar.segCap));
             hipLaunchKernelGGL(k_compact_keys, dim3(compactBlocks, DEME_KEY_SEGS), dim3(256), 0, st, c->keysRaw.as<uint64_t>(), ar.segCap,
-                               blk, 0u, c->keysSorted[nextEarly].as<uint64_t>(), c->binStat.as<uint2>(), nStats);
+                               blk, 0u, c->keysSorted[next].as<uint64_t>(), c->binStat.as<uint2>(), nStats);
+        }
+        const unsigned bitsA = bits_for(c->dp.nSpheres, 31);
+        const bool keysAhead = c->hPersist.empty() && sort_goes_ahead(c, c->lastKeyLen, c->ownFromKeys, c->cntCap);
+        const size_t keyBound = ahead_bound(c->lastKeyLen, c->cntCap);
+        if (keysAhead) {
+            size_t bytes = 0;
+            HIPCK((deme_sort::radix_sort<uint64_t, false>(nullptr, bytes, nullptr, nullptr, nullptr, nullptr, keyBound, c->cntCap, 31, 33 + bitsA, st)));
+            if (ensure(c, c->keysMid, (size_t)c->cntCap * 8) || ensure(c, c->sortTmp, bytes))
+                return c->lastStatus;
+            if (!segmented)
+                hipLaunchKernelGGL(k_key_length, dim3(1), dim3(1), 0, st, blk, (unsigned long long)c->cntCap);
         }
         const DetectHead* hh = pin_at<DetectHead>(c, 1024);
         HIPCK(hipMemcpyAsync(pin_at<DetectHead>(c, 1024), c->ctr.p, segmented ? sizeof(DetectHead) : sizeof(DetectCounters), hipMemcpyDeviceToHost, st));
-        HIPCK(sync_readback(c, st, !async));
+        HIPCK(mark_readback(c, st));
+        if (keysAhead) {
+            size_t bytes = c->sortTmp.bytes;
+            HIPCK((deme_sort::radix_sort<uint64_t, false>(c->sortTmp.p, bytes, segmented ? c->keysSorted[next].as<uint64_t>() : c->keysRaw.as<uint64_t>(),
+                                                          c->keysMid.as<uint64_t>(), nullptr, nullptr, keyBound, c->cntCap, 31, 33 + bitsA, st,
+                                                          &blk->nKeySort)));
+            hipLaunchKernelGGL(k_segment_rank_sort, dim3(grid_for(keyBound)), dim3(256), 0, st, (uint32_t)keyBound, &blk->nKeySort,
+                               c->keysMid.as<uint64_t>(), c->keysSorted[next].as<uint64_t>());
+        }
+        HIPCK(sync_readback(c, !async));
         hc = hh->c;
         if (!statusSeen) {
             statusSeen = true;
@@ -704,6 +757,8 @@
         if (hc.nContactsRaw > c->cntCap || segMax > ar.segCap) {
             if (async)
                 HIPCK(hipStreamSynchronize(c->stream));
+            if (keysAhead)
+                HIPCK(hipStreamSynchronize(st));
             const size_t want = std::max<size_t>(hc.nContactsRaw, (size_t)segMax * DEME_KEY_SEGS);
             if (int rc = grow_contact_arena(c, want + want / 4 + 1024))
                 return rc;
@@ -727,11 +782,15 @@
             }
             nC += nPersist;
         }
-        const int next = c->keysCur ^ 1;
+        c->lastKeyLen = hc.nContactsRaw;
+        const bool keysSorted = keysAhead && hc.nContactsRaw <= keyBound && (!segmented || grid_for(segMax) <= compactBlocks);
         uint64_t* rawKeys = c->keysRaw.as<uint64_t>();
         if (segmented) {
             c->lastSegMax = segMax;
-            if (grid_for(segMax) > compactBlocks)
+            if (keysAhead && !keysSorted)
+                hipLaunchKernelGGL(k_compact_keys, dim3(std::max(1u, grid_for(segMax)), DEME_KEY_SEGS), dim3(256), 0, st, c->keysRaw.as<uint64_t>(),
+                                   ar.segCap, blk, 0u, c->keysSorted[next].as<uint64_t>(), (const uint2*)nullptr, 0u);
+            else if (grid_for(segMax) > compactBlocks)
                 hipLaunchKernelGGL(k_compact_keys, dim3((unsigned)grid_for(segMax) - compactBlocks, DEME_KEY_SEGS), dim3(256), 0, st,
                                    c->keysRaw.as<uint64_t>(), ar.segCap, blk, compactBlocks, c->keysSorted[next].as<uint64_t>(),
                                    (const uint2*)nullptr, 0u);
@@ -740,17 +799,16 @@
         }
         if (nPersist)
             HIPCK(hipMemcpyAsync(rawKeys + hc.nContactsRaw, c->persistKeys.p, nPersist * 8, hipMemcpyDeviceToDevice, st));
-        if (nC) {
-            const unsigned bitsA = bits_for(c->dp.nSpheres, 31);
+        if (nC && !keysSorted) {
             if (int rc = ensure(c, c->keysMid, (size_t)c->cntCap * 8))
                 return rc;
             uint64_t* mid = c->keysMid.as<uint64_t>();
             if (int rc = with_temp(c, c->sortTmp, [&](void* tmp, size_t& bytes) {
                     return deme_radix_sort<DemeRadixCfg<8>, false>(tmp, bytes, rawKeys, mid, nullptr, nullptr, (size_t)nC, (size_t)c->cntCap, 31,
-                                                                   33 + bitsA, DEME_SORT_OWN_FROM_KEYS64, st);
+                                                                   33 + bitsA, c->ownFromKeys, st);
                 }))
                 return rc;
-            hipLaunchKernelGGL(k_segment_rank_sort, dim3(grid_for(nC)), dim3(256), 0, st, (uint32_t)nC, mid,
+            hipLaunchKernelGGL(k_segment_rank_sort, dim3(grid_for(nC)), dim3(256), 0, st, (uint32_t)nC, (const uint32_t*)nullptr, mid,
                                c->keysSorted[next].as<uint64_t>());
             if (nPersist) {
                 unsigned long long* cnt = &blk->c.nContactsRaw;
@@ -788,7 +846,7 @@
         HIPCK(hipMemsetAsync(L.blockMode.p, 0, L.blockMode.bytes, st));
     }
     if (nC)
-        hipLaunchKernelGGL(k_run_starts, dim3(grid_for(nC)), dim3(256), 0, st, (uint32_t)nC, L.ownerB[1].as<uint32_t>(),
+        hipLaunchKernelGGL(k_run_starts, dim3(grid_for(nC)), dim3(256), 0, st, (uint32_t)nC, (const uint32_t*)nullptr, L.ownerB[1].as<uint32_t>(),
                            c->nOwners, L.bStart.as<uint32_t>());
     else
         HIPCK(hipMemsetAsync(L.bStart.p, 0, ((size_t)c->nOwners + 1) * 4, st));
@@ -862,7 +920,7 @@
                 }))
                 return rc;
         }
-        hipLaunchKernelGGL(k_run_starts, dim3(grid_for(nC)), dim3(256), 0, st, (uint32_t)nC, L.ownerA.as<uint32_t>(), c->nOwners,
+        hipLaunchKernelGGL(k_run_starts, dim3(grid_for(nC)), dim3(256), 0, st, (uint32_t)nC, (const uint32_t*)nullptr, L.ownerA.as<uint32_t>(), c->nOwners,
                            L.aStart.as<uint32_t>());
     } else {
         HIPCK(hipMemsetAsync(L.aStart.p, 0, ((size_t)c->nOwners + 1) * 4, st));
@@ -872,32 +930,51 @@
     RangeCounters hr{};
     if (tileEligible) {
         hipLaunchKernelGGL(k_scan_small, dim3(1), dim3(DEME_SCAN_T), 0, st, L.tileRem.as<uint32_t>(), L.tileBase.as<uint32_t>(), nTiles + 1,
-                           &L.rangeCtr.as<RangeCounters>()->nRemote);
+                           &L.rangeCtr.as<RangeCounters>()->nRemote, (unsigned int*)nullptr, 0ull);
         hipLaunchKernelGGL(k_tile_build, dim3(nTiles), dim3(256), 0, st, c->dp, c->nOwners, L.info.as<uint4>(),
                            L.ownerB[0].as<uint32_t>(), L.aStart.as<uint32_t>(), ow, L.tileBase.as<uint32_t>(), L.tInfo.as<uint2>(),
                            L.hList.as<uint32_t>(), L.hCount.as<uint32_t>(),
                            c->hasGhosts ? L.tileMode.as<uint32_t>() : (uint32_t*)nullptr, L.lOff.as<uint16_t>(),
                            L.lPos.as<uint16_t>(), L.lCount.as<uint32_t>(), L.rankC.as<uint32_t>(), L.remKey[0].as<uint32_t>(),
-                           L.remVal.as<uint32_t>(), L.tileOrg.as<int64_t>(), L.rangeCtr.as<RangeCounters>(), nTiles,
+                           L.tileOrg.as<int64_t>(), L.rangeCtr.as<RangeCounters>(), nTiles,
                            L.tileBig.as<uint32_t>(), L.bigList.as<uint32_t>(), c->recContact.as<uint32_t>());
         hipLaunchKernelGGL(k_tile_stats, dim3((nTiles + 1023u) / 1024u), dim3(256), 0, st, nTiles, L.hCount.as<uint32_t>(),
                            L.lCount.as<uint32_t>(), L.rangeCtr.as<RangeCounters>());
         uint32_t nR = 0;
+        const unsigned obits = bits_for(c->nOwners, 32);
+        const size_t recBound = ahead_bound(c->lastRecLen, std::min<size_t>((size_t)nC, c->cntCap));
+        const bool recsAhead = sort_goes_ahead(c, c->lastRecLen, c->ownFromRecs, recBound);
+        if (recsAhead) {
+            size_t bytes = 0;
+            HIPCK((deme_sort::radix_sort<uint32_t, true>(nullptr, bytes, nullptr, nullptr, nullptr, nullptr, recBound, (size_t)c->cntCap, 0, obits, st)));
+            if (int rc = ensure(c, c->sortTmp, bytes))
+                return rc;
+        }
         HIPCK(hipMemcpyAsync(pin_at<RangeCounters>(c, 128), L.rangeCtr.p, sizeof(hr), hipMemcpyDeviceToHost, st));
-        HIPCK(sync_readback(c, st, true));
+        HIPCK(mark_readback(c, st));
+        if (recsAhead) {
+            const uint32_t* nDev = &L.rangeCtr.as<RangeCounters>()->nRecSort;
+            size_t bytes = c->sortTmp.bytes;
+            HIPCK((deme_sort::radix_sort<uint32_t, true>(c->sortTmp.p, bytes, L.remKey[0].as<uint32_t>(), L.remKey[1].as<uint32_t>(), nullptr,
+                                                         L.rIdx.as<uint32_t>(), recBound, (size_t)c->cntCap, 0, obits, st, nDev)));
+            hipLaunchKernelGGL(k_run_starts, dim3(grid_for(recBound)), dim3(256), 0, st, (uint32_t)recBound, nDev, L.remKey[1].as<uint32_t>(),
+                               c->nOwners, L.rStart.as<uint32_t>());
+        }
+        HIPCK(sync_readback(c, true));
         hr = *pin_at<RangeCounters>(c, 128);
         nR = (uint32_t)hr.nRemote + hr.nExtra;
+        c->lastRecLen = nR;
         L.nBigTiles = hr.nBig;
-        const unsigned obits = bits_for(c->nOwners, 32);
-        if (nR) {
+        if (recsAhead && nR <= recBound) {
+        } else if (nR) {
             if (int rc = with_temp(c, c->sortTmp, [&](void* tmp, size_t& bytes) {
                     return deme_radix_sort<DemeRadixCfg<10>, true>(tmp, bytes, L.remKey[0].as<uint32_t>(), L.remKey[1].as<uint32_t>(),
-                                                                   L.remVal.as<uint32_t>(), L.rIdx.as<uint32_t>(), (size_t)nR, (size_t)c->cntCap, 0, obits,
-                                                                   DEME_SORT_OWN_FROM_RECORDS, st);
+                                                                   (const uint32_t*)nullptr, L.rIdx.as<uint32_t>(), (size_t)nR, (size_t)c->cntCap, 0,
+                                                                   obits, c->ownFromRecs, st);
                 }))
                 return rc;
-            hipLaunchKernelGGL(k_run_starts, dim3(grid_for(nR)), dim3(256), 0, st, nR, L.remKey[1].as<uint32_t>(), c->nOwners,
-                               L.rStart.as<uint32_t>());
+            hipLaunchKernelGGL(k_run_starts, dim3(grid_for(nR)), dim3(256), 0, st, nR, (const uint32_t*)nullptr, L.remKey[1].as<uint32_t>(),
+                               c->nOwners, L.rStart.as<uint32_t>());
         } else {
             HIPCK(hipMemsetAsync(L.rStart.p, 0, ((size_t)c->nOwners + 1) * 4, st));
         }
@@ -1428,6 +1505,15 @@
         c->spinSync = atoi(e);
     if (const char* e = getenv("DEME_KEY_SEG_MIN"))
         c->keySegMin = (size_t)std::max(0ll, atoll(e));
+    c->ownFromInc = DEME_SORT_OWN_FROM_INCIDENCES, c->ownFromKeys = DEME_SORT_OWN_FROM_KEYS64, c->ownFromRecs = DEME_SORT_OWN_FROM_RECORDS;
+    if (const char* e = getenv("DEME_SORT_OWN_FROM"))
+        c->ownFromInc = c->ownFromKeys = c->ownFromRecs = (size_t)std::max(0ll, atoll(e));
+    if (const char* e = getenv("DEME_SORT_AHEAD"))
+        c->sortAhead = atoi(e);
+    if (hipEventCreateWithFlags(&c->evReadback, hipEventDisableTiming) != hipSuccess) {
+        deme_ctx_destroy(c);
+        return DEME_ERR_HIP;
+    }
     *out = c;
     return DEME_OK;
 }
@@ -1457,6 +1543,8 @@
     }
     if (c->pin)
         hipHostFree(c->pin);
+    if (c->evReadback)
+        hipEventDestroy(c->evReadback);
     for (ContactList& l : c->list)
         for (DevBuf* b : l.buffers())
             if (b->p)
@@ -4536,7 +4624,7 @@
         if (int rc = with_temp(c, c->tlTmp, [&](void* tmp, size_t& bytes) {
                 return deme_radix_sort<DemeRadixCfg<8>, true>(tmp, bytes, c->tlTri[0].as<uint32_t>(), c->tlTri[1].as<uint32_t>(),
                                                               c->tlRow[0].as<uint32_t>(), c->tlRow[1].as<uint32_t>(), n, n, 0, bits,
-                                                              DEME_SORT_OWN_FROM_RECORDS, c->stream);
+                                                              c->ownFromRecs, c->stream);
             }))
             return rc;
     }
@@ -4723,9 +4811,57 @@
         ok = ok && hipMemcpy(valsOut, vOut, n * 4, hipMemcpyDeviceToHost) == hipSuccess;
     return ok ? DEME_OK : DEME_ERR_HIP;
 }
+template <bool HAS_V, typename K>
+int sort_host_arrays_devlen(int device, const K* keys, const uint32_t* vals, size_t bound, uint32_t len, unsigned beginBit, unsigned endBit,
+                            K* keysOut, uint32_t* valsOut) {
+    if (endBit < beginBit || endBit > 8 * sizeof(K) || (bound && (!keys || !keysOut || (HAS_V && !valsOut))))
+        return DEME_ERR_INVALID;
+    if (DEME_SORT_ROCPRIM || bound > deme_sort::MAX_N)
+        return DEME_ERR_INVALID;
+    if (!bound)
+        return DEME_OK;
+    if (hipSetDevice(device) != hipSuccess)
+        return DEME_ERR_HIP;
+    SortScratch s;
+    K *dIn = s.room<K>(bound), *dOut = s.room<K>(bound);
+    uint32_t *vIn = HAS_V && vals ? s.room<uint32_t>(bound) : nullptr, *vOut = HAS_V ? s.room<uint32_t>(bound) : nullptr;
+    uint32_t* dLen = s.room<uint32_t>(1);
+    if (!dIn || !dOut || !dLen || (HAS_V && !vOut) || (HAS_V && vals && !vIn))
+        return DEME_ERR_HIP;
+    size_t bytes = 0;
+    if (deme_sort::radix_sort<K, HAS_V>(nullptr, bytes, dIn, dOut, vIn, vOut, bound, bound, beginBit, endBit, nullptr, dLen) != hipSuccess)
+        return DEME_ERR_HIP;
+    void* tmp = s.room<char>(bytes);
+    if (!tmp)
+        return DEME_ERR_HIP;
+    bool ok = hipMemcpy(dIn, keys, bound * sizeof(K), hipMemcpyHostToDevice) == hipSuccess;
+    ok = ok && hipMemcpy(dOut, keysOut, bound * sizeof(K), hipMemcpyHostToDevice) == hipSuccess;
+    ok = ok && hipMemcpy(dLen, &len, 4, hipMemcpyHostToDevice) == hipSuccess;
+    if (HAS_V) {
+        if (vals)
+            ok = ok && hipMemcpy(vIn, vals, bound * 4, hipMemcpyHostToDevice) == hipSuccess;
+        ok = ok && hipMemcpy(vOut, valsOut, bound * 4, hipMemcpyHostToDevice) == hipSuccess;
+    }
+    ok = ok && deme_sort::radix_sort<K, HAS_V>(tmp, bytes, dIn, dOut, vIn, vOut, bound, bound, beginBit, endBit, nullptr, dLen) == hipSuccess;
+    ok = ok && hipDeviceSynchronize() == hipSuccess;
+    ok = ok && hipMemcpy(keysOut, dOut, bound * sizeof(K), hipMemcpyDeviceToHost) == hipSuccess;
+    if (HAS_V)
+        ok = ok && hipMemcpy(valsOut, vOut, bound * 4, hipMemcpyDeviceToHost) == hipSuccess;
+    return ok ? DEME_OK : DEME_ERR_HIP;
+}
 }
 
 unsigned deme_sort_tile_keys(void) { return deme_sort::TILE; }
+
+int deme_sort_pairs_u32_devlen(int device, const uint32_t* keys, const uint32_t* vals, size_t bound, uint32_t len, unsigned beginBit,
+                               unsigned endBit, uint32_t* keysOut, uint32_t* valsOut) {
+    return sort_host_arrays_devlen<true>(device, keys, vals, bound, len, beginBit, endBit, keysOut, valsOut);
+}
+
+int deme_sort_keys_u64_devlen(int device, const uint64_t* keys, size_t bound, uint32_t len, unsigned beginBit, unsigned endBit,
+                              uint64_t* keysOut) {
+    return sort_host_arrays_devlen<false>(device, keys, (const uint32_t*)nullptr, bound, len, beginBit, endBit, keysOut, (uint32_t*)nullptr);
+}
 
 int deme_sort_pairs_u32(int device, const uint32_t* keys, const uint32_t* vals, size_t n, unsigned beginBit, unsigned endBit, int forceOwn,
                         uint32_t* keysOut, uint32_t* valsOut) {
diff --git a/dem-engine_amd/csrc/deme_kernels.h b/dem-engine_amd/csrc/deme_kernels.h
--- a/dem-engine_amd/csrc/deme_kernels.h
+++ b/dem-engine_amd/csrc/deme_kernels.h
@@ -5,6 +5,9 @@
 namespace deme_dev {
 
 #define DEME_NULL_BINID_DEV 0xFFFFFFFFu
+__device__ inline uint32_t list_length(uint32_t n, const uint32_t* __restrict__ nDev) {
+    return nDev ? min(*nDev, n) : n;
+}
 #define DEME_ST_VELOCITY 1u
 #define DEME_ST_NONFINITE 2u
 #define DEME_ST_INCIDENCE 4u
@@ -26,6 +29,8 @@
     DetectCounters c;
     unsigned long long segCount[DEME_KEY_SEGS];
     unsigned long long segCtr[DEME_KEY_SEGS * DEME_KEY_SEG_STRIDE];
+    unsigned int nIncSort;
+    unsigned int nKeySort;
 };
 struct DetectHead {
     DetectCounters c;
@@ -55,7 +60,8 @@
     if (threadIdx.x < 64) {
         static_assert(DEME_KEY_SEGS == 64, "one lane per segment");
         const unsigned long long raw = blk->segCtr[threadIdx.x * DEME_KEY_SEG_STRIDE];
-        if (stats && seg == 0 && blockIdx.x == 0)
+        const bool head = stats && seg == 0 && blockIdx.x == 0;
+        if (head)
             blk->segCount[threadIdx.x] = raw;
         const unsigned long long cnt = min(raw, (unsigned long long)segCap);
         unsigned long long inc = cnt;
@@ -66,6 +72,8 @@
         }
         if (threadIdx.x == seg)
             sStart = inc - cnt, sCount = cnt;
+        if (head && threadIdx.x == 63)
+            blk->nKeySort = (unsigned int)min(inc, 0xFFFFFFFFull);
     }
     __syncthreads();
     const uint64_t i = ((uint64_t)xOff + blockIdx.x) * blockDim.x + threadIdx.x;
@@ -217,7 +225,8 @@
 
 #define DEME_SCAN_T 1024u
 #define DEME_SCAN_IPT 4u
-__global__ __launch_bounds__(DEME_SCAN_T) void k_scan_small(const uint32_t* in, uint32_t* out, uint32_t n, unsigned long long* totalOut) {
+__global__ __launch_bounds__(DEME_SCAN_T) void k_scan_small(const uint32_t* in, uint32_t* out, uint32_t n, unsigned long long* totalOut,
+                                                            unsigned int* lenOut, unsigned long long lenCap) {
     __shared__ unsigned long long sWave[DEME_SCAN_T / 64];
     __shared__ unsigned long long sCarry;
     const uint32_t lane = threadIdx.x & 63u, w = threadIdx.x >> 6;
@@ -259,8 +268,11 @@
             sCarry += total;
         __syncthreads();
     }
-    if (threadIdx.x == 0)
+    if (threadIdx.x == 0) {
         *totalOut = sCarry;
+        if (lenOut)
+            *lenOut = (unsigned int)min(sCarry, min(lenCap, 0xFFFFFFFFull));
+    }
 }
 
 __global__ __launch_bounds__(256) void k_fill_incidence(const DevParams p, const uint4* __restrict__ binLo,
@@ -705,8 +717,13 @@
 __global__ __launch_bounds__(256) void k_bin_stats_final(const uint2* __restrict__ perBlock, uint32_t nBlocks, DetectCounters* ctr) {
     bin_stats_block(perBlock, nBlocks, blockIdx.x, ctr);
 }
-
-__global__ __launch_bounds__(256) void k_segment_rank_sort(uint32_t n, const uint64_t* __restrict__ in, uint64_t* __restrict__ out) {
+__global__ void k_key_length(DetectBlock* blk, unsigned long long cap) {
+    blk->nKeySort = (unsigned int)min(min(blk->c.nContactsRaw, cap), 0xFFFFFFFFull);
+}
+
+__global__ __launch_bounds__(256) void k_segment_rank_sort(uint32_t n, const uint32_t* __restrict__ nDev, const uint64_t* __restrict__ in,
+                                                           uint64_t* __restrict__ out) {
+    n = list_length(n, nDev);
     const uint32_t i = blockIdx.x * blockDim.x + threadIdx.x;
     if (i >= n)
         return;
@@ -1145,12 +1162,19 @@
     unsigned int nBigIn;
     unsigned int tileMaxHaloIn;
     unsigned long long nRemote;
-    unsigned int pad[2];
+    unsigned int nRecSort;
+    unsigned int pad;
 };
 
-__global__ __launch_bounds__(256) void k_run_starts(uint32_t n, const uint32_t* __restrict__ owner, uint32_t nOwners,
-                                                    uint32_t* __restrict__ start) {
+__global__ __launch_bounds__(256) void k_run_starts(uint32_t n, const uint32_t* __restrict__ nDev, const uint32_t* __restrict__ owner,
+                                                    uint32_t nOwners, uint32_t* __restrict__ start) {
+    n = list_length(n, nDev);
     const uint32_t i = blockIdx.x * blockDim.x + threadIdx.x;
+    if (n == 0) {
+        for (uint32_t o = i; o <= nOwners; o += gridDim.x * blockDim.x)
+            start[o] = 0u;
+        return;
+    }
     if (i >= n)
         return;
     const uint32_t cur = owner[i];
diff --git a/dem-engine_amd/csrc/deme_sort.h b/dem-engine_amd/csrc/deme_sort.h
--- a/dem-engine_amd/csrc/deme_sort.h
+++ b/dem-engine_amd/csrc/deme_sort.h
@@ -29,12 +29,22 @@
     return (unsigned)(k >> shift) & mask;
 }
 
+__device__ inline uint32_t length_of(uint32_t nBound, const uint32_t* __restrict__ nDev) {
+    return nDev ? min(*nDev, nBound) : nBound;
+}
+
 template <typename K>
-__global__ __launch_bounds__(THREADS) void k_count(const K* __restrict__ keys, uint32_t n, uint32_t nTiles, unsigned shift, unsigned nbits,
-                                                   uint32_t* __restrict__ table) {
+__global__ __launch_bounds__(THREADS) void k_count(const K* __restrict__ keys, uint32_t nBound, const uint32_t* __restrict__ nDev, uint32_t nTiles,
+                                                   unsigned shift, unsigned nbits, uint32_t* __restrict__ table) {
     constexpr unsigned COPIES = 4;
     __shared__ uint32_t hist[COPIES * RADIX];
     const unsigned tid = threadIdx.x, tile = blockIdx.x, mask = (1u << nbits) - 1u;
+    const uint32_t n = length_of(nBound, nDev);
+    if (tile * TILE >= n) {
+        if (tid <= mask)
+            table[(size_t)tid * nTiles + tile] = 0u;
+        return;
+    }
     for (unsigned d = tid; d < COPIES * RADIX; d += THREADS)
         hist[d] = 0;
     __syncthreads();
@@ -86,16 +96,20 @@
 }
 
 template <typename K, bool HAS_V>
-__global__ __launch_bounds__(THREADS) void k_scatter(const K* __restrict__ keys, const uint32_t* __restrict__ vals, uint32_t n, uint32_t nTiles,
-                                                     unsigned shift, unsigned nbits, const uint32_t* __restrict__ table,
-                                                     const uint32_t* __restrict__ totals, K* __restrict__ keysOut, uint32_t* __restrict__ valsOut) {
+__global__ __launch_bounds__(THREADS) void k_scatter(const K* __restrict__ keys, const uint32_t* __restrict__ vals, uint32_t nBound,
+                                                     const uint32_t* __restrict__ nDev, uint32_t nTiles, unsigned shift, unsigned nbits,
+                                                     const uint32_t* __restrict__ table, const uint32_t* __restrict__ totals,
+                                                     K* __restrict__ keysOut, uint32_t* __restrict__ valsOut) {
     __shared__ typename BlockScan::storage_type scanSt;
     __shared__ K sKeys[TILE];
     __shared__ uint32_t sVals[HAS_V ? TILE : 1];
     __shared__ uint32_t wcnt[WAVES * RADIX];
     __shared__ uint32_t gbase[RADIX];
     const unsigned tid = threadIdx.x, lane = tid % WAVE, w = tid / WAVE, tile = blockIdx.x, mask = (1u << nbits) - 1u;
-    const uint32_t tile0 = tile * TILE, nValid = n - tile0 < TILE ? n - tile0 : TILE;
+    const uint32_t n = length_of(nBound, nDev), tile0 = tile * TILE;
+    if (tile0 >= n)
+        return;
+    const uint32_t nValid = n - tile0 < TILE ? n - tile0 : TILE;
     for (unsigned d = tid; d < WAVES * RADIX; d += THREADS)
         wcnt[d] = 0;
     K k[KPT];
@@ -105,7 +119,7 @@
         const uint32_t at = w * (WAVE * KPT) + i * WAVE + lane;
         k[i] = at < nValid ? keys[tile0 + at] : ~K(0);
         if (HAS_V)
-            v[i] = at < nValid ? vals[tile0 + at] : 0u;
+            v[i] = at < nValid ? (vals ? vals[tile0 + at] : tile0 + at) : 0u;
     }
     __syncthreads();
     uint32_t* wc = wcnt + w * RADIX;
@@ -167,12 +181,18 @@
     }
 }
 
+__global__ __launch_bounds__(256) void k_iota(uint32_t n, uint32_t* __restrict__ out) {
+    const uint32_t i = blockIdx.x * blockDim.x + threadIdx.x;
+    if (i < n)
+        out[i] = i;
+}
+
 inline size_t align256(size_t b) { return (b + 255) & ~(size_t)255; }
 inline unsigned passes_for(unsigned beginBit, unsigned endBit) { return (endBit - beginBit + RB - 1) / RB; }
 
 template <typename K, bool HAS_V>
 hipError_t radix_sort(void* tmp, size_t& bytes, const K* keysIn, K* keysOut, const uint32_t* valsIn, uint32_t* valsOut, size_t n, size_t cap,
-                      unsigned beginBit, unsigned endBit, hipStream_t st) {
+                      unsigned beginBit, unsigned endBit, hipStream_t st, const uint32_t* nDev = nullptr) {
     const size_t room = n > cap ? n : cap, tilesRoom = (room + TILE - 1) / TILE;
     const size_t tableB = align256((tilesRoom + 1) * RADIX * 4), keysB = align256(room * sizeof(K)), valsB = HAS_V ? align256(room * 4) : 0;
     if (!tmp) {
@@ -186,8 +206,12 @@
     const unsigned passes = passes_for(beginBit, endBit);
     if (!passes) {
         hipError_t e = hipMemcpyAsync(keysOut, keysIn, n * sizeof(K), hipMemcpyDeviceToDevice, st);
-        if (e == hipSuccess && HAS_V)
+        if (e == hipSuccess && HAS_V && valsIn)
             e = hipMemcpyAsync(valsOut, valsIn, n * 4, hipMemcpyDeviceToDevice, st);
+        if (e == hipSuccess && HAS_V && !valsIn) {
+            hipLaunchKernelGGL(k_iota, dim3((unsigned)((n + 255) / 256)), dim3(256), 0, st, (uint32_t)n, valsOut);
+            e = hipGetLastError();
+        }
         return e;
     }
     uint32_t* table = reinterpret_cast<uint32_t*>(tmp);
@@ -202,10 +226,10 @@
         const bool toOut = (passes - 1 - p) % 2 == 0;
         K* kDst = toOut ? keysOut : keysAlt;
         uint32_t* vDst = toOut ? valsOut : valsAlt;
-        hipLaunchKernelGGL(k_count<K>, dim3(nTiles), dim3(THREADS), 0, st, kSrc, (uint32_t)n, nTiles, shift, nbits, table);
+        hipLaunchKernelGGL(k_count<K>, dim3(nTiles), dim3(THREADS), 0, st, kSrc, (uint32_t)n, nDev, nTiles, shift, nbits, table);
         hipLaunchKernelGGL(k_scan_rows, dim3(1u << nbits), dim3(SCAN_THREADS), 0, st, table, nTiles, totals);
-        hipLaunchKernelGGL((k_scatter<K, HAS_V>), dim3(nTiles), dim3(THREADS), 0, st, kSrc, vSrc, (uint32_t)n, nTiles, shift, nbits, table,
-                           totals, kDst, vDst);
+        hipLaunchKernelGGL((k_scatter<K, HAS_V>), dim3(nTiles), dim3(THREADS), 0, st, kSrc, vSrc, (uint32_t)n, nDev, nTiles, shift, nbits,
+                           table, totals, kDst, vDst);
         kSrc = kDst, vSrc = vDst;
     }
     return hipGetLastError();
diff --git a/dem-engine_amd/csrc/deme_tile.h b/dem-engine_amd/csrc/deme_tile.h
--- a/dem-engine_amd/csrc/deme_tile.h
+++ b/dem-engine_amd/csrc/deme_tile.h
@@ -753,7 +753,7 @@
                                                     uint32_t* __restrict__ tileMode, uint16_t* __restrict__ lOff,
                                                     uint16_t* __restrict__ lPos, uint32_t* __restrict__ lCount,
                                                     uint32_t* __restrict__ rankC, uint32_t* __restrict__ remKey,
-                                                    uint32_t* __restrict__ remVal, int64_t* __restrict__ org, RangeCounters* rc,
+                                                    int64_t* __restrict__ org, RangeCounters* rc,
                                                     uint32_t nTiles, uint32_t* __restrict__ tileBig, uint32_t* __restrict__ bigList,
                                                     uint32_t* __restrict__ recContact) {
     __shared__ uint32_t table[DEME_TILE_HASH];
@@ -861,7 +861,7 @@
                 const unsigned long long below = (1ull << lane) - 1ull;
                 const uint32_t r = remote ? runR + beforeR + (uint32_t)__popcll(mr & below) : runL + beforeL + (uint32_t)__popcll(ml & below);
                 rankC[c] = r;
-                remKey[r] = ob, remVal[r] = r, recContact[r] = c;
+                remKey[r] = ob, recContact[r] = c;
             }
             runR += totR, runL += totL;
             __syncthreads();
@@ -938,7 +938,7 @@
         if (c < c1) {
             rankC[c] = r;
             if (remote)
-                remKey[r] = ob, remVal[r] = r, recContact[r] = c;
+                remKey[r] = ob, recContact[r] = c;
         }
         run += total;
         __syncthreads();
@@ -980,6 +980,8 @@
         mh[threadIdx.x >> 6] = a, ml[threadIdx.x >> 6] = b, sh[threadIdx.x >> 6] = sum;
     __syncthreads();
     if (threadIdx.x == 0) {
+        if (blockIdx.x == 0)
+            rc->nRecSort = (unsigned int)rc->nRemote + rc->nExtra;
         atomicAdd(&rc->tileHaloSum, sh[0] + sh[1] + sh[2] + sh[3]);
         atomicMax(&rc->tileMaxHalo, max(max(mh[0], mh[1]), max(mh[2], mh[3])));
         atomicMax(&rc->tileMaxList, max(max(ml[0], ml[1]), max(ml[2], ml[3])));
diff --git a/include/deme_hip.h b/include/deme_hip.h
--- a/include/deme_hip.h
+++ b/include/deme_hip.h
@@ -184,6 +184,10 @@
                         uint32_t* keysOut, uint32_t* valsOut);
 int deme_sort_keys_u64(int device, const uint64_t* keys, size_t n, unsigned beginBit, unsigned endBit, int forceOwn, uint64_t* keysOut);
 unsigned deme_sort_tile_keys(void);
+int deme_sort_pairs_u32_devlen(int device, const uint32_t* keys, const uint32_t* vals, size_t bound, uint32_t len, unsigned beginBit,
+                               unsigned endBit, uint32_t* keysOut, uint32_t* valsOut);
+int deme_sort_keys_u64_devlen(int device, const uint64_t* keys, size_t bound, uint32_t len, unsigned beginBit, unsigned endBit,
+                              uint64_t* keysOut);
 int deme_download_sphere_geometry(deme_ctx* ctx, double* X, double* Y, double* Z, float* R, size_t cap);
 
 int deme_change_owner_sizes(deme_ctx* ctx, const uint32_t* ownerIds, const float* factors, size_t n);
```

Measured after the change: 6.518 billion (median of 6 runs). No clear change (+0.2%).
